# awaelchli/torch-optical-flow

Hardware: AMD Instinct MI355X
Metric: image-pairs/sec + corr-lookup HBM GB/s, RAFT 12-iter @ Sintel 1024×436 (higher is better)
Workload: dtype corr + convs split-fp16 (22-bit operands: fp16 hi + lo, 3 f16 MFMA per product, fp32 accumulate); lookup fp32; 1 GPU; raft-12iter-sintel-436x1024; pairs_per_gpu=8, global_batch=8, iters=12, padded=440x1024, parallelism=pairs sharded over 1 GPU(s), conv_benchmark=True, update_impl=split, hip_graph=True, steps_in_flight=1, full=False

## Files before the change

include/oflow.h:

```cpp
#ifndef OFLOW_H_
#define OFLOW_H_

#ifdef __cplusplus
extern "C" {
#endif

#define OFLOW_ABI_VERSION 3

#define OFLOW_OK 0
#define OFLOW_E_NULL (-1)
#define OFLOW_E_SHAPE (-2)
#define OFLOW_E_LEVELS (-3)
#define OFLOW_E_TINY (-4)
#define OFLOW_E_RADIUS (-5)
#define OFLOW_E_MODE (-6)
#define OFLOW_E_ALIGN (-7)

#define OFLOW_MAX_LEVELS 8
#define OFLOW_MAX_RADIUS 7

#define OFLOW_INTERP_BILINEAR 0
#define OFLOW_INTERP_NEAREST 1
#define OFLOW_INTERP_BICUBIC 2
#define OFLOW_PAD_ZEROS 0
#define OFLOW_PAD_BORDER 1
#define OFLOW_PAD_REFLECTION 2

#define OFLOW_IN_S32 0
#define OFLOW_IN_F32_NORM 1
#define OFLOW_IN_F32 2
#define OFLOW_IN_IMG7S2 3
#define OFLOW_IN_FLOW7 4
#define OFLOW_EPI_FLOW_HEAD 3

int oflow_abi_version(void);
const char* oflow_status_string(int status);

int oflow_corr_pyramid_dims(int H, int W, int num_levels, int* level_h, int* level_w);

int oflow_corr_pyramid_f32(const float* d_fmap1, const float* d_fmap2, int B, int C, int H, int W,
                           int num_levels, float* const* d_levels, void* stream);

int oflow_corr_lookup_f32(const float* const* d_levels, const int* level_h, const int* level_w,
                          int num_levels, const float* d_coords, int B, int H, int W, int radius,
                          float* d_out, void* stream);

long long oflow_corr_tiled_level_floats(int H_l, int W_l);
int oflow_corr_pyramid_tiled_f32(const float* d_fmap1, const float* d_fmap2, int B, int C, int H, int W,
                                 int num_levels, float* const* d_levels, void* stream);
int oflow_corr_pyramid_tiled_s32(const void* d_fmap1_s32, const void* d_fmap2_s32, int B, int C, int H, int W,
                                 int num_levels, float* const* d_levels, void* stream);
int oflow_corr_lookup_tiled_f32(const float* const* d_levels, const int* level_h, const int* level_w,
                                int num_levels, const float* d_coords, int B, int H, int W, int radius,
                                float* d_out, void* stream);
int oflow_corr_untile_f32(const float* d_tiled, float* d_out, long long Q, int H_l, int W_l, void* stream);

int oflow_grid_warp_f32(const float* d_frame, const float* d_flow, int B, int C, int H, int W, int mode,
                        int padding_mode, int align_corners, float* d_out, void* stream);

int oflow_grid_sample_f32(const float* d_input, const float* d_grid, int B, int C, int H, int W, int Ho, int Wo,
                          int mode, int padding_mode, int align_corners, float* d_out, void* stream);

int oflow_corr_otf_prepare_f16(const float* d_fmap1, const float* d_fmap2, int B, int C, int H, int W,
                               int num_levels, void* d_f1h, void* const* d_f2h, float* d_scratch, void* stream);
int oflow_corr_lookup_otf_f16(const void* d_f1h, const void* const* d_f2h, const int* level_h, const int* level_w,
                              int num_levels, const float* d_coords, int B, int C, int H, int W, int radius,
                              float* d_out, void* stream);

int oflow_corr_lookup_otf_backward_f32(const float* d_grad_out, const void* d_f1h, const void* const* d_f2h,
                                       const int* level_h, const int* level_w, int num_levels, const float* d_coords,
                                       int B, int C, int H, int W, int radius, float* d_grad_fmap1,
                                       float* d_grad_fmap2, float* d_scratch, void* stream);

int oflow_bias_act_f32(const float* d_x, long long sx, const float* d_bias, float* d_y0, long long sy0, float* d_y1,
                       long long sy1, int B, int C, int P, int activation, float scale, void* stream);
int oflow_gru_reset_f32(const float* d_zr, long long szr, const float* d_br, const float* d_h, long long sh,
                        float* d_rh, long long srh, int B, int CH, int P, void* stream);
int oflow_gru_blend_f32(const float* d_zr, long long szr, const float* d_bz, const float* d_q, long long sq,
                        const float* d_bq, float* d_h, long long sh, int B, int CH, int P, void* stream);

int oflow_pack_s32_f32(const float* d_x, long long x_batch_stride, int C, int B, int H, int W, int activation,
                       int dst_channel, void* d_y0, long long y0_pixel_stride, void* d_y1, long long y1_pixel_stride,
                       float* d_nhwc, int nhwc_pixel_stride, void* stream);
int oflow_flow_prep_s32(const float* d_coords, int B, int H, int W, void* d_patches, void* d_flow0,
                        long long flow0_pixel_stride, void* d_flow1, long long flow1_pixel_stride, void* stream);

typedef struct oflow_conv_s32_desc {
  unsigned int struct_size;
  int in_format, in_groups;
  const void* d_x;
  long long x_pixel_stride;
  const float *d_in_scale, *d_in_shift;
  const void *d_wpack, *d_wfrag;
  const float *d_wscale, *d_bias;
  int n_pad, N;
  int B, H, W, kh, kw, block_n;
  int epilogue, activation;
  float out_scale;
  void *d_y0, *d_y1;
  long long y0_pixel_stride, y1_pixel_stride;
  float* d_f32;
  long long f32_batch_stride, f32_channel_stride;
  int f32_accumulate;
  float *d_gru_h, *d_gru_z;
  int gru_channels;
  float *d_nhwc, *d_stats;
  const void* d_res;
  long long res_pixel_stride;
  int nhwc_pixel_stride, res_activation, s2d;
  const float* d_addend;
  long long addend_pixel_stride;
  const float* d_fh_weights;
  float* d_fh_partial;
  int fh_slabs;
} oflow_conv_s32_desc;
int oflow_conv_s32(const oflow_conv_s32_desc* desc, void* stream);

int oflow_flow_head_col2im_f32(const float* d_y, const float* d_bias, int B, int H, int W, float* d_coords, void* stream);
int oflow_flow_head_finish_f32(const float* d_partial, int slabs, const float* d_bias, int B, int H, int W,
                               float* d_coords, void* d_flow0, long long flow0_pixel_stride, void* d_flow1,
                               long long flow1_pixel_stride, void* stream);

int oflow_normalize_images_f32(const float* d_x0, const float* d_x1, long long n, float* d_y0, float* d_y1, void* stream);

int oflow_replicate_pad_f32(const float* const* d_src, float* const* d_dst, int count, long long planes, int H, int W,
                            int top, int bottom, int left, int right, void* stream);

int oflow_set_range_flag(unsigned int* d_flag);

int oflow_range_flag_exchange(unsigned int* d_flag, unsigned int* d_out, void* stream);

int oflow_timing_event_create(void** ev);
int oflow_timing_event_destroy(void* ev);
int oflow_timing_event_record(void* ev, void* stream, int external);
int oflow_timing_event_elapsed_ms(void* start, void* end, float* ms);

int oflow_flow_head2_s32(const void* d_x, long long x_pixel_stride, int in_groups, const float* d_weight,
                         const float* d_bias, int B, int H, int W, float* d_coords, void* stream);
int oflow_flow_head2_tiled_s32(const void* d_x, long long x_pixel_stride, int in_groups, const float* d_wr,
                               const float* d_bias, int B, int H, int W, float* d_coords, void* stream);
int oflow_corr_lookup_tiled_nhwc_f32(const float* const* d_levels, const int* level_h, const int* level_w, int num_levels,
                                     const float* d_coords, int B, int H, int W, int radius, float* d_out, int row_floats,
                                     void* stream);
int oflow_corr_lookup_convc1_s32(const float* const* d_levels, const int* level_h, const int* level_w, int num_levels,
                                 const float* d_coords, int B, int H, int W, int radius, const void* d_wpack,
                                 const float* d_wscale, const float* d_bias, void* d_y, long long y_pixel_stride,
                                 void* stream);

int oflow_stem_patches_s32(const float* d_img, int B, int C, int H, int W, void* d_out, int out_groups, void* stream);
int oflow_norm_stats_finalize(const float* d_partials, int B, int tiles, int n_pad, int C, double eps, float* d_alpha,
                              float* d_beta, void* stream);
int oflow_norm_apply_s32(const float* d_x, int C, int B, int H, int W, const float* d_alpha, const float* d_beta,
                         int activation, int res_mode, const void* d_res, long long res_pixel_stride, const float* d_x2,
                         const float* d_alpha2, const float* d_beta2, int res_activation, int s2d, void* d_y,
                         long long y_pixel_stride, void* stream);

int oflow_convex_upsample_f32(const float* d_flow, const float* d_mask, int B, int H, int W, float* d_out, void* stream);
int oflow_convex_upsample_backward_f32(const float* d_grad_out, const float* d_flow, const float* d_mask, int B, int H,
                                       int W, float* d_grad_flow, float* d_grad_mask, float* d_scratch, void* stream);

int oflow_conv2d_backward_input_f32(const float* d_grad_out, const float* d_weight, int B, int Cout, int Cin, int H, int W,
                                    int kh, int kw, float* d_grad_input, void* stream);
int oflow_conv2d_backward_weight_slab_pixels(void);
long long oflow_conv2d_backward_weight_workspace_floats(int B, int Cout, int Cin, int H, int W, int kh, int kw);
int oflow_conv2d_backward_weight_f32(const float* d_grad_out, const float* d_x, int B, int Cout, int Cin, int H, int W,
                                     int kh, int kw, float* d_grad_weight, float* d_grad_bias, float* d_workspace,
                                     void* stream);

int oflow_conv2d_strided_backward_input_f32(const float* d_grad_out, const float* d_weight, int B, int Cout, int Cin, int H,
                                            int W, int kh, int kw, int stride, float* d_grad_input, void* stream);
long long oflow_conv2d_strided_backward_weight_workspace_floats(int B, int Cout, int Cin, int H, int W, int kh, int kw,
                                                                int stride);
int oflow_conv2d_strided_backward_weight_f32(const float* d_grad_out, const float* d_x, int B, int Cout, int Cin, int H,
                                             int W, int kh, int kw, int stride, float* d_grad_weight, float* d_grad_bias,
                                             float* d_workspace, void* stream);
int oflow_conv2d_strided_backward_weight_generic_f32(const float* d_grad_out, const float* d_x, int B, int Cout, int Cin,
                                                     int H, int W, int kh, int kw, int stride, float* d_grad_weight,
                                                     float* d_grad_bias, float* d_workspace, void* stream);

int oflow_instance_norm_backward_f32(const float* d_grad_out, const float* d_x, int planes, int HW, double eps, int relu,
                                     float* d_grad_input, void* stream);
long long oflow_frozen_batch_norm_backward_workspace_floats(int B, int C, int HW);
int oflow_frozen_batch_norm_backward_f32(const float* d_grad_out, const float* d_x, const float* d_weight, const float* d_bias,
                                         const float* d_running_mean, const float* d_running_var, int B, int C, int HW,
                                         double eps, int relu, float* d_grad_input, float* d_grad_weight, float* d_grad_bias,
                                         float* d_workspace, void* stream);

int oflow_batch_norm_chunk_elements(void);
long long oflow_batch_norm_workspace_floats(int B, int C, int HW);
int oflow_batch_norm_forward_f32(const float* d_x, const float* d_weight, const float* d_bias, int B, int C, int HW,
                                 double eps, int relu, float* d_y, float* d_mean, float* d_var, float* d_workspace,
                                 void* stream);
int oflow_batch_norm_backward_f32(const float* d_grad_out, const float* d_x, const float* d_weight, const float* d_bias,
                                  const float* d_mean, const float* d_var, int B, int C, int HW, double eps, int relu,
                                  float* d_grad_input, float* d_grad_weight, float* d_grad_bias, float* d_workspace,
                                  void* stream);

int oflow_corr_lookup_backward_f32(const float* d_grad_out, const float* d_coords, int B, int H, int W, int radius,
                                   float* const* d_grad_levels, const int* level_h, const int* level_w, int num_levels,
                                   void* stream);
int oflow_corr_pyramid_grad_combine_f32(float* const* d_grad_levels, const int* level_h, const int* level_w,
                                        int num_levels, long long Q, void* stream);
int oflow_corr_fmap_grad_f32(const float* d_fmap1, const float* d_fmap2, const float* d_g0, int B, int C, int N,
                             float scale, float* d_grad_f1, float* d_grad_f2, void* stream);

int oflow_grid_warp_backward_f32(const float* d_grad_out, const float* d_frame, const float* d_flow, int B, int C, int H,
                                 int W, int mode, int padding_mode, int align_corners, float* d_grad_frame,
                                 float* d_grad_flow, void* stream);
int oflow_grid_sample_backward_f32(const float* d_grad_out, const float* d_input, const float* d_grid, int B, int C,
                                   int H, int W, int Ho, int Wo, int mode, int padding_mode, int align_corners,
                                   float* d_grad_input, float* d_grad_grid, void* stream);

#define OFLOW_FLOW_STATS_CHUNKS 128
#define OFLOW_FLOW2RGB_BAKER 0
#define OFLOW_FLOW2RGB_HSV 1
#define OFLOW_FLOW2RGB_MEISTER 2
int oflow_flow_stats_f32(const float* d_flow, int B, int H, int W, int clip, float clip_lo, float clip_hi,
                         int invert_y, float* d_partials, void* stream);
int oflow_flow2rgb_f32(const float* d_flow, int B, int H, int W, int method, int clip, float clip_lo, float clip_hi,
                       int invert_y, int have_denom, float denom, const float* d_partials, float* d_rgb, void* stream);
int oflow_flow_pack_f32(const float* d_flow, int B, int H, int W, int channels, int flip_rows, float* d_out,
                        void* stream);

#define OFLOW_FLOW_METRICS_PARTIALS 1024
#define OFLOW_MAX_PREDS 32
#define OFLOW_VALID_NONE 0
#define OFLOW_VALID_F32 1
#define OFLOW_VALID_U8 2
int oflow_flow_error_stats_f32(const float* d_pred, long long pred_sb, long long pred_sc, long long pred_sh,
                               const float* d_target, long long target_sb, long long target_sc, long long target_sh,
                               const void* d_valid, int valid_kind, long long valid_sb, long long valid_sh, int B, int H,
                               int W, float abs_threshold, float rel_threshold, float max_flow, float* d_epe_map,
                               double* d_workspace, double* d_accum, void* stream);
int oflow_sequence_loss_f32(const float* const* d_preds, int n_preds, const float* weights, const float* d_flow_gt,
                            const void* d_valid, int valid_kind, int B, int H, int W, float max_flow,
                            double* d_workspace, float* d_loss, double* d_stats, void* stream);
int oflow_sequence_loss_backward_f32(const float* d_grad_out, const float* const* d_preds, float* const* d_grads,
                                     int n_preds, const float* weights, const float* d_flow_gt, const void* d_valid,
                                     int valid_kind, int B, int H, int W, float max_flow, void* stream);

int oflow_forward_interpolate_f32(const float* d_flow, int B, int H, int W, float* d_out, void* stream);

int oflow_fb_consistency_f32(const float* d_fw, const float* d_bw, int B, int H, int W, float alpha, float beta,
                             unsigned char* d_mask_fw, unsigned char* d_mask_bw, float* d_err_fw, float* d_err_bw,
                             void* stream);

#define OFLOW_SPLAT_SUM 0
#define OFLOW_SPLAT_AVG 1
#define OFLOW_SPLAT_LINEAR 2
#define OFLOW_SPLAT_SOFT 3
#define OFLOW_SPLAT_EPS 1e-7
#define OFLOW_SPLAT_MIN_FRAC_BITS 38
#define OFLOW_SPLAT_MAX_PIXELS (1 << 22)
int oflow_splat_frac_bits(int H, int W);
long long oflow_splat_workspace_bytes(int B, int C, int H, int W);
int oflow_splat_f32(const float* d_frame, const float* d_flow, const float* d_metric, int B, int C, int H, int W,
                    int mode, float* d_out, float* d_weight, void* d_workspace, void* stream);
int oflow_splat_backward_f32(const float* d_grad_out, const float* d_frame, const float* d_flow, const float* d_metric,
                             const float* d_out, const float* d_weight, int B, int C, int H, int W, int mode,
                             float* d_grad_frame, float* d_grad_flow, float* d_grad_metric, void* d_workspace,
                             void* stream);

long long oflow_census_loss_workspace_bytes(int B, int H, int W);
int oflow_census_loss_f32(const float* d_frame0, const float* d_frame1, const void* d_mask, int mask_kind, int B,
                          int C, int H, int W, int patch, float image_range, float* d_s_map, double* d_workspace,
                          float* d_loss, double* d_sum_m, void* stream);
int oflow_census_loss_backward_f32(const float* d_grad_loss, const float* d_frame0, const float* d_frame1,
                                   const void* d_mask, int mask_kind, const float* d_s_map, const double* d_sum_m,
                                   int B, int C, int H, int W, int patch, float image_range, float* d_grad_frame0,
                                   float* d_grad_frame1, void* stream);
// ... 40 lines not shown
```

torch-optical-flow_amd/csrc/conv_s32.hip:

```cpp
#include "oflow_internal.h"

namespace oflow {
namespace {

typedef _Float16 half8 __attribute__((ext_vector_type(8)));
typedef float f32x16 __attribute__((ext_vector_type(16)));
typedef unsigned int u32x4 __attribute__((ext_vector_type(4)));

constexpr int kTY = 4, kTX = 32;

constexpr int kAinGroups = 4;


struct ConvArgs {
  const uint8_t* x;
  long long xps;
  int kg;
  const uint8_t* w;
  int npad;
  const float* wsc;
  const float* bias;
  int N;
  int B, H, W, tiles_x, tiles_y;
  int act;
  float oscale;
  uint8_t* y0;
  long long y0ps;
  uint8_t* y1;
  long long y1ps;
  float* f;
  long long fbs, fcs;
  int faccum;
  float* h;
  float* z;
  int gch;
  const float* add;
  long long addps;
  float* fn;
  int fnps;
  float* stats;
  const uint8_t* res;
  long long resps;
  int res_act;
  int s2d;
  const float* ia;
  const float* ib;
  int ain;
  int cin;
  int wbytes;
  const uint8_t* wf;
  int exp_flags;
  const float* fhw;
  float* fhy;
};
constexpr int kEpiFlowHead = OFLOW_EPI_FLOW_HEAD;
constexpr int kInS32 = OFLOW_IN_S32, kInF32Norm = OFLOW_IN_F32_NORM, kInF32 = OFLOW_IN_F32, kInImg = OFLOW_IN_IMG7S2,
              kInFlow = OFLOW_IN_FLOW7;
constexpr int kImgC = 3, kImgK = 7, kImgRows = (kTY - 1) * 2 + kImgK, kImgCols = (kTX - 1) * 2 + kImgK;
constexpr int kImgHalf = (kImgCols + 1) / 2, kImgPitch = 2 * kImgHalf, kImgPlane = kImgRows * kImgPitch;

__device__ __forceinline__ float sigmoid_hw(float v) {
  return __builtin_amdgcn_rcpf(1.0f + __builtin_amdgcn_exp2f(v * -1.4426950408889634f));
}
__device__ __forceinline__ float tanh_hw(float v) {
  return 1.0f - 2.0f * __builtin_amdgcn_rcpf(__builtin_amdgcn_exp2f(v * 2.8853900817779268f) + 1.0f);
}

__device__ __forceinline__ float act_fn(float v, int act) {
  if (act == 1) return v < 0.f ? 0.f : v;
  if (act == 2) return 1.0f / (1.0f + expf(-v));
  if (act == 3) return tanhf(v);
  return v;
}

__device__ __forceinline__ void split8(const float* v, half8& hi, half8& lo) { split_vec(v, hi, lo); }

__device__ __forceinline__ void store_s32(uint8_t* y, long long ps, long long P, int n, int N, const float* v, float& gm) {
  uint8_t* line = y + P * ps + (long long)(n >> 5) * 128 + ((n & 31) >> 3) * 16;
  if (n + 8 <= N) {
    half8 hi, lo;
    split8(v, hi, lo);
    gm = fmaxf(gm, fmaxf(fmaxf(fmaxf(fabsf(v[0]), fabsf(v[1])), fmaxf(fabsf(v[2]), fabsf(v[3]))),
                         fmaxf(fmaxf(fabsf(v[4]), fabsf(v[5])), fmaxf(fabsf(v[6]), fabsf(v[7])))));
    *reinterpret_cast<half8*>(line) = hi;
    *reinterpret_cast<half8*>(line + 64) = lo;
  } else {
    _Float16* hp = reinterpret_cast<_Float16*>(line);
    _Float16* lp = reinterpret_cast<_Float16*>(line + 64);
#pragma unroll
    for (int j = 0; j < 8; ++j) {
      if (n + j < N) {
        gm = fmaxf(gm, fabsf(v[j]));
        _Float16 h_, l_;
        split_f16(v[j], h_, l_);
        hp[j] = h_;
        lp[j] = l_;
      }
    }
  }
}

typedef __attribute__((address_space(4))) const float cfloat;
template <int T0, int T1>
__device__ __forceinline__ void flow_head_partials(const float* tp, cfloat* w, float* yp, long long plane, bool in) {
  constexpr int NO = 2 * (T1 - T0);
  float acc[2][NO];
#pragma unroll
  for (int j = 0; j < NO; ++j) acc[0][j] = acc[1][j] = 0.f;
  float wn[2][NO];
#pragma unroll
  for (int e = 0; e < 2; ++e)
#pragma unroll
    for (int j = 0; j < NO; ++j) wn[e][j] = w[e * 18 + 2 * T0 + j];
  float2 tn = *reinterpret_cast<const float2*>(tp);
#pragma unroll
  for (int e = 0; e < 2; ++e)
#pragma unroll
    for (int j = 0; j < NO; ++j) asm volatile("" : "+s"(wn[e][j]));
  asm volatile("" : "+v"(tn.x), "+v"(tn.y));
#pragma unroll 2
  for (int c0 = 0; c0 < 64; c0 += 2) {
    float wc[2][NO];
#pragma unroll
    for (int e = 0; e < 2; ++e)
#pragma unroll
      for (int j = 0; j < NO; ++j) wc[e][j] = wn[e][j];
    const float2 t = tn;
    const int c1 = c0 + 2 < 64 ? c0 + 2 : c0;
#pragma unroll
    for (int e = 0; e < 2; ++e)
#pragma unroll
      for (int j = 0; j < NO; ++j) wn[e][j] = w[(c1 + e) * 18 + 2 * T0 + j];
    tn = *reinterpret_cast<const float2*>(tp + c1);
    __builtin_amdgcn_sched_barrier(0);
#pragma unroll
    for (int j = 0; j < NO; ++j) {
      acc[0][j] = fmaf(t.x, wc[0][j], acc[0][j]);
      acc[1][j] = fmaf(t.y, wc[1][j], acc[1][j]);
    }
    __builtin_amdgcn_sched_barrier(0);
#pragma unroll
    for (int e = 0; e < 2; ++e)
#pragma unroll
      for (int j = 0; j < NO; ++j) asm volatile("" : "+s"(wn[e][j]));
    asm volatile("" : "+v"(tn.x), "+v"(tn.y));
  }
  if (in) {
#pragma unroll
    for (int j = 0; j < NO; ++j) yp[(2 * T0 + j) * plane] = acc[0][j] + acc[1][j];
  }
}

template <int KH, int KW, int BN, int WM, int WN, int EPI, int TY = kTY, int AIN = kInS32, bool BREG = false, int BD = 1>
__global__ __launch_bounds__(64 * WM * WN, WM * WN == 8 ? 1 : 2) void conv_s32_kernel(ConvArgs a) {
  constexpr int NTH = 64 * WM * WN;
  constexpr int T = KH * KW;
  constexpr int BM = TY * kTX;
  constexpr int PH = KH / 2, PW = KW / 2;
  constexpr int HY = TY + KH - 1, HX = kTX + KW - 1, NPIX = HY * HX;
  constexpr int AITEMS = NPIX * 8, APER = (AITEMS + NTH - 1) / NTH;
  constexpr int BITEMS = BN * 8, BPER = (BITEMS + NTH - 1) / NTH;
  constexpr int MT = TY / WM;
  constexpr int NT = BN / WN / 32;
  static_assert((WM * WN == 4 || WM * WN == 8) && MT >= 1 && NT >= 1, "bad wave grid");
  static_assert(NTH % 8 == 0, "an A item's 16-B chunk is tid & 7");
  constexpr bool WIN = AIN == kInImg || AIN == kInFlow;
  constexpr int WC = AIN == kInFlow ? 2 : kImgC, WS = AIN == kInFlow ? 1 : 2;
  constexpr int WROWS = (kTY - 1) * WS + kImgK, WCOLS = (kTX - 1) * WS + kImgK;
  constexpr int WHALF = WS == 2 ? (WCOLS + 1) / 2 : WCOLS, WPITCH = WS == 2 ? 2 * WHALF : WCOLS;
  constexpr int WPLANE = WROWS * WPITCH;
  constexpr int WKPAD = AIN == kInFlow ? 128 : 160;
  constexpr int WAPER = WIN ? BM * 4 / NTH : 1;
  static_assert(!WIN || (BM * 4) % NTH == 0, "window items");
  static_assert(AIN != kInImg || (WHALF == kImgHalf && WPITCH == kImgPitch && WPLANE == kImgPlane), "stem window");
  constexpr bool ADB = (T == 1) && !WIN;
  constexpr int RSA = 144, RSB = 144;
  constexpr int A_BYTES = NPIX * RSA, B_BYTES = BN * RSB;
  static_assert(!BREG || (T > 1 && (WM == 1 || WM == 2 || WM == 4) && BN == 32 * WN && AIN == kInS32),
                "register-direct B: T > 1, WM x WN waves of one 32-channel tile each");
  constexpr int MAIN_BYTES = (ADB ? 2 : 1) * A_BYTES + (BREG ? 0 : 2 * B_BYTES);
  constexpr int TS = BN + 4;
  constexpr int EPI_BYTES = BM * TS * 4;
  constexpr int LDS_BYTES = MAIN_BYTES > EPI_BYTES ? MAIN_BYTES : EPI_BYTES;
  constexpr int kImgZero = WC * WPLANE;
  constexpr int IMG_FLOATS = (kImgZero + 1 + 3) & ~3;
  constexpr int AFF_BYTES = AIN == kInF32Norm ? kAinGroups * 32 * 8
                            : WIN ? IMG_FLOATS * 4 + WKPAD * 4
                            : 0;
  static_assert(!WIN || (T == 1 && TY == kTY), "window input: 1x1 geometry over the patch channels, 4-row tiles");
  __shared__ __attribute__((aligned(16))) uint8_t smem[LDS_BYTES + AFF_BYTES];
  __shared__ float2 sSB[BN];
  __shared__ float3 sStat[EPI == 0 ? WM * BN : 1];
  float2* sAff = reinterpret_cast<float2*>(smem + LDS_BYTES);
  float* sImg = reinterpret_cast<float*>(smem + LDS_BYTES);
  int* sKoff = reinterpret_cast<int*>(smem + LDS_BYTES + (WIN ? IMG_FLOATS * 4 : 0));
  uint8_t* sA = smem;
  uint8_t* sB = smem + (ADB ? 2 : 1) * A_BYTES;

  const int tid = threadIdx.x, lane = tid & 63, wave = tid >> 6;
  const int wm = wave / WN, wn = wave % WN;
  const int r = lane & 31, hh = lane >> 5;

  int tile = blockIdx.x;
  const int cblk = blockIdx.y;
  const int tx0 = (tile % a.tiles_x) * kTX;
  tile /= a.tiles_x;
  const int ty0 = (tile % a.tiles_y) * TY;
  const int b = tile / a.tiles_y;
  const int n0 = cblk * BN;
  const long long pix0 = (long long)b * a.H * a.W;

  u32x4 ra[APER];
  const __amdgpu_buffer_rsrc_t rsA = __builtin_amdgcn_make_buffer_rsrc(
      const_cast<uint8_t*>(a.x + pix0 * a.xps), (short)0, (int)((long long)a.H * a.W * a.xps), 0x00020000);
  const __amdgpu_buffer_rsrc_t rsB =
      __builtin_amdgcn_make_buffer_rsrc(const_cast<uint8_t*>(a.w), (short)0, a.wbytes, 0x00020000);
  auto a_off = [&](int s_, int& col) {
    int t_ = tid;
    asm volatile("" : "+v"(t_));
    const int item = (AITEMS % NTH == 0) ? t_ + s_ * NTH : min(t_ + s_ * NTH, AITEMS - 1);
    const int p = item >> 3, c = item & 7;
    const int gy = ty0 - PH + p / HX, gx = tx0 - PW + p % HX;
    const int cy = min(max(gy, 0), a.H - 1), cx = min(max(gx, 0), a.W - 1);
    col = c * 16;
    return (cy * a.W + cx) * (int)a.xps + (AIN == kInF32 ? 0 : c * 16);
  };
  unsigned aok = 0u;
#pragma unroll
  for (int s_ = 0; s_ < APER; ++s_) {
    const int item = (AITEMS % NTH == 0) ? tid + s_ * NTH : min(tid + s_ * NTH, AITEMS - 1);
    const int p = item >> 3;
    const int gy = ty0 - PH + p / HX, gx = tx0 - PW + p % HX;
    const bool ok = static_cast<unsigned>(gy) < static_cast<unsigned>(a.H) && static_cast<unsigned>(gx) < static_cast<unsigned>(a.W);
    aok |= (ok ? 1u : 0u) << s_;
  }
  int boff[BPER];
#pragma unroll
  for (int s_ = 0; s_ < BPER; ++s_) boff[s_] = (n0 + (tid + s_ * NTH) / 8) * 128 + ((tid + s_ * NTH) & 7) * 16;
#define OFLOW_LOAD_A(RA, G)                                                                                          \
  if constexpr (!WIN) _Pragma("unroll") for (int s_ = 0; s_ < APER; ++s_) {                                          \
    int col_;                                                                                                        \
    const int off_ = a_off(s_, col_);                                                                                \
    if constexpr (AIN == kInF32)     \
      RA[s_] = __builtin_amdgcn_raw_buffer_load_b128(rsA, off_ + min((G) * 128 + col_, a.cin * 4 - 16), 0, 0);       \
    else                                                                                                             \
      RA[s_] = __builtin_amdgcn_raw_buffer_load_b128(rsA, off_, (G) * 128, 0);                                       \
  }
#define OFLOW_WRITE_A(RA, BUF, G)                                                                                    \
  float amx_ = 0.f;                                                                                                  \
  float2 af4_[4];                                                                                                    \
  if constexpr (AIN == kInF32Norm) _Pragma("unroll") for (int e_ = 0; e_ < 4; ++e_)                                  \
    af4_[e_] = sAff[(G) * 32 + 4 * (tid & 7) + e_];                                                                  \
  if constexpr (WIN) {                                                                                               \
                                                                                                        \
    _Pragma("unroll") for (int s_ = 0; s_ < WAPER; ++s_) {                                                           \
      const int item = tid + s_ * NTH;                                                                               \
      const int p = item % BM, cp = item / BM;                                                                       \
      const int pb_ = WS * (p >> 5) * WPITCH + (p & 31);                                                             \
      const int4 k0_ = *reinterpret_cast<const int4*>(sKoff + (G) * 32 + 8 * cp);                                    \
      const int4 k1_ = *reinterpret_cast<const int4*>(sKoff + (G) * 32 + 8 * cp + 4);                                \
      const int kov_[8] = {k0_.x, k0_.y, k0_.z, k0_.w, k1_.x, k1_.y, k1_.z, k1_.w};                                  \
      float v8_[8];                                                                                                  \
      _Pragma("unroll") for (int e_ = 0; e_ < 8; ++e_) {                                                             \
        v8_[e_] = sImg[kov_[e_] < 0 ? kImgZero : pb_ + kov_[e_]];                                                    \
        amx_ = fmaxf(amx_, fabsf(v8_[e_]));                                                                          \
      }                                                                                                              \
      half8 h8_, l8_;                                                                                                \
      split_vec(v8_, h8_, l8_);                                                                                      \
      uint8_t* rw_ = sA + (BUF) * A_BYTES + p * RSA;                                                                 \
      *reinterpret_cast<half8*>(rw_ + (cp << 4)) = h8_;                                                              \
      *reinterpret_cast<half8*>(rw_ + ((4 + cp) << 4)) = l8_;                                                        \
    }                                                                                                                \
  } else                                                                                                             \
  _Pragma("unroll") for (int s_ = 0; s_ < APER; ++s_) {                                                              \
    const int item = tid + s_ * NTH;                                                                                 \
                                                     \
    const int p = item >> 3, c = item & 7;                                                                           \
    if (AITEMS % NTH == 0 || item < AITEMS) {                                                                        \
      if constexpr (AIN != kInS32) {                                                                                 \
                   \
        typedef _Float16 half4_ __attribute__((ext_vector_type(4)));                                                 \
        half4_ h4 = {0, 0, 0, 0}, l4 = {0, 0, 0, 0};                                                                 \
        if (((aok >> s_) & 1u) && (AIN != kInF32 || (G) * 32 + 4 * c < a.cin)) {                                     \
          const float* fv = reinterpret_cast<const float*>(&RA[s_]);                                                 \
          float mx_ = 0.f, v4_[4];                                                                                   \
          _Pragma("unroll") for (int e_ = 0; e_ < 4; ++e_) {                                                         \
            float v_ = fv[e_];                                                                                       \
            if constexpr (AIN == kInF32Norm) {                                                                       \
              const float2 af = af4_[e_];                                                                            \
              v_ = v_ * af.x + af.y;                                                                                 \
              v_ = v_ < 0.f ? 0.f : v_;                                                                              \
            }                                                                                                        \
            mx_ = fmaxf(mx_, fabsf(v_));                                                                             \
            v4_[e_] = v_;                                                                                            \
          }                                                                                                          \
          split_vec(v4_, h4, l4);                                                                                    \
          amx_ = fmaxf(amx_, mx_);                                                                                   \
        }                                                                                                            \
        uint8_t* rw_ = sA + (BUF) * A_BYTES + p * RSA + (c & 1) * 8;                                                 \
        *reinterpret_cast<half4_*>(rw_ + ((c >> 1) << 4)) = h4;                                                      \
        *reinterpret_cast<half4_*>(rw_ + ((4 + (c >> 1)) << 4)) = l4;                                                \
      } else {                                                                                                       \
        *reinterpret_cast<u32x4*>(sA + (BUF) * A_BYTES + p * RSA + (c << 4)) =                                       \
            ((aok >> s_) & 1u) ? RA[s_] : u32x4{0u, 0u, 0u, 0u};                                                     \
      }                                                                                                              \
    }                                                                                                                \
  }                                                                                                                  \
  if constexpr (AIN != kInS32) range_guard(amx_);
#define OFLOW_LOAD_B(RB, STEP)                                                                                       \
  _Pragma("unroll") for (int s_ = 0; s_ < BPER; ++s_) {                                                              \
    const int item = tid + s_ * NTH;                                                                                 \
    if (BITEMS % NTH == 0 || item < BITEMS)                                                                          \
      RB[s_] = __builtin_amdgcn_raw_buffer_load_b128(rsB, boff[s_], (STEP) * a.npad * 128, 0);                       \
  }
#define OFLOW_WRITE_B(RB, BUF)                                                                                       \
  _Pragma("unroll") for (int s_ = 0; s_ < BPER; ++s_) {                                                              \
    const int item = tid + s_ * NTH;                                                                                 \
    const int n = item >> 3, c = item & 7;                                                                           \
    if (BITEMS % NTH == 0 || item < BITEMS)                                                                          \
      *reinterpret_cast<u32x4*>(sB + (BUF) * B_BYTES + n * RSB + (c << 4)) = RB[s_];                                 \
  }
#define OFLOW_READ_OPS(AH, AL, BH, BL, I, S_)                                                                        \
  {                                                                                                                  \
    const int ii_ = (I);                                                                                             \
    const int t_ = ii_ % T, ky_ = t_ / KW, kx_ = t_ - ky_ * KW;                                                      \
    const uint8_t* bufA_ = sA + (ADB ? (ii_ & 1) * A_BYTES : 0);                                                     \
    const uint8_t* bufB_ = sB + (ii_ & 1) * B_BYTES;                                                                 \
    const int chi_ = 2 * (S_) + hh, clo_ = 4 + 2 * (S_) + hh;                                                        \
    _Pragma("unroll") for (int mt_ = 0; mt_ < MT; ++mt_) {                                                           \
      const int p_ = (wm * MT + mt_ + ky_) * HX + r + kx_;                                                           \
      const uint8_t* row_ = bufA_ + p_ * RSA;                                                                        \
      AH[mt_] = *reinterpret_cast<const half8*>(row_ + (chi_ << 4));                                                 \
      AL[mt_] = *reinterpret_cast<const half8*>(row_ + (clo_ << 4));                                                 \
    }                                                                                                                \
    _Pragma("unroll") for (int nt_ = 0; nt_ < NT; ++nt_) {                                                           \
      const int n_ = wn * (BN / WN) + nt_ * 32 + r;                                                                  \
      const uint8_t* row_ = bufB_ + n_ * RSB;                                                                        \
      BH[nt_] = *reinterpret_cast<const half8*>(row_ + (chi_ << 4));                                                 \
      BL[nt_] = *reinterpret_cast<const half8*>(row_ + (clo_ << 4));                                                 \
    }                                                                                                                \
  }
#define OFLOW_MFMAS(AH, AL, BH, BL)                                                                                  \
  _Pragma("unroll") for (int mt = 0; mt < MT; ++mt)                                                                  \
    _Pragma("unroll") for (int nt = 0; nt < NT; ++nt) {                                                              \
      acc[mt][nt] = __builtin_amdgcn_mfma_f32_32x32x16_f16(AH[mt], BL[nt], acc[mt][nt], 0, 0, 0);                    \
      acc[mt][nt] = __builtin_amdgcn_mfma_f32_32x32x16_f16(AL[mt], BH[nt], acc[mt][nt], 0, 0, 0);                    \
      acc[mt][nt] = __builtin_amdgcn_mfma_f32_32x32x16_f16(AH[mt], BH[nt], acc[mt][nt], 0, 0, 0);                    \
    }

  f32x16 acc[MT][NT];
#pragma unroll
  for (int i = 0; i < MT; ++i)
#pragma unroll
    for (int j = 0; j < NT; ++j)
#pragma unroll
      for (int e = 0; e < 16; ++e) acc[i][j][e] = 0.f;

  const int S = a.kg * T;
  for (int c = tid; c < BN; c += NTH) {
    const int n = min(n0 + c, a.N - 1);
    sSB[c] = make_float2(a.wsc[n], a.bias ? a.bias[n] : 0.f);
  }
  if constexpr (AIN == kInF32Norm) {
    for (int e = tid; e < a.kg * 32; e += NTH)
      sAff[e] = make_float2(a.ia[(long long)b * a.kg * 32 + e], a.ib[(long long)b * a.kg * 32 + e]);
    __syncthreads();
  }
  if constexpr (AIN == kInImg) {
    const float* img = reinterpret_cast<const float*>(a.x) + (long long)b * kImgC * (2 * a.H) * (2 * a.W);
    const int iy0 = 2 * ty0 - kImgK / 2, ix0 = 2 * tx0 - kImgK / 2;
    constexpr int IMG_N = kImgC * kImgRows * kImgCols, IMG_PER = (IMG_N + NTH - 1) / NTH;
    float iv[IMG_PER];
    int io[IMG_PER];
#pragma unroll
    for (int s_ = 0; s_ < IMG_PER; ++s_) {
      const int e = min(tid + s_ * NTH, IMG_N - 1);
      const int ch = e / (kImgRows * kImgCols), rem = e - ch * (kImgRows * kImgCols);
      const int ry = rem / kImgCols, rx = rem - ry * kImgCols;
      const int iy = iy0 + ry, ix = ix0 + rx;
      const bool in = static_cast<unsigned>(iy) < static_cast<unsigned>(2 * a.H) && static_cast<unsigned>(ix) < static_cast<unsigned>(2 * a.W);
      const int cy = min(max(iy, 0), 2 * a.H - 1), cx = min(max(ix, 0), 2 * a.W - 1);
      const float v = img[((long long)ch * (2 * a.H) + cy) * (2 * a.W) + cx];
      iv[s_] = in ? v : 0.f;
      io[s_] = ch * kImgPlane + ry * kImgPitch + (rx & 1) * kImgHalf + (rx >> 1);
    }
#pragma unroll
    for (int s_ = 0; s_ < IMG_PER; ++s_)
      if (tid + s_ * NTH < IMG_N) sImg[io[s_]] = iv[s_];
  }
  if constexpr (AIN == kInFlow) {
    const float* co = reinterpret_cast<const float*>(a.x) + (long long)b * 2 * a.H * a.W;
    const int iy0 = ty0 - kImgK / 2, ix0 = tx0 - kImgK / 2;
    constexpr int FL_N = 2 * WROWS * WCOLS, FL_PER = (FL_N + NTH - 1) / NTH;
    float iv[FL_PER];
    int io[FL_PER];
#pragma unroll
    for (int s_ = 0; s_ < FL_PER; ++s_) {
      const int e = min(tid + s_ * NTH, FL_N - 1);
      const int ch = e / (WROWS * WCOLS), rem = e - ch * (WROWS * WCOLS);
      const int ry = rem / WCOLS, rx = rem - ry * WCOLS;
      const int iy = iy0 + ry, ix = ix0 + rx;
      const bool in = static_cast<unsigned>(iy) < static_cast<unsigned>(a.H) && static_cast<unsigned>(ix) < static_cast<unsigned>(a.W);
      const int cy = min(max(iy, 0), a.H - 1), cx = min(max(ix, 0), a.W - 1);
      const float v = co[((long long)ch * a.H + cy) * a.W + cx] - static_cast<float>(ch == 0 ? ix : iy);
      iv[s_] = in ? v : 0.f;
      io[s_] = ch * WPLANE + ry * WPITCH + rx;
    }
#pragma unroll
    for (int s_ = 0; s_ < FL_PER; ++s_)
      if (tid + s_ * NTH < FL_N) sImg[io[s_]] = iv[s_];
  }
  if constexpr (WIN) {
    for (int k = tid; k < WKPAD; k += NTH) {
      const int t = k / WC, ch = k - t * WC;
      const int ky = t / kImgK, kx = t - ky * kImgK;
      sKoff[k] = t < kImgK * kImgK
                     ? ch * WPLANE + ky * WPITCH + (WS == 2 ? (kx & 1) * WHALF + (kx >> 1) : kx)
                     : -1;
    }
    if (tid == 0) sImg[kImgZero] = 0.f;
    __syncthreads();
  }
  if constexpr (BREG) {
  const __amdgpu_buffer_rsrc_t rsW =
      __builtin_amdgcn_make_buffer_rsrc(const_cast<uint8_t*>(a.wf), (short)0, a.wbytes, 0x00020000);
  const int wlane = ((n0 >> 5) + wn) * 4096 + lane * 16;
  const int wstep = a.npad * 128;
  constexpr int RING = 2;
  u32x4 bq[RING][4];
  auto load_b = [&](u32x4 (&d)[4], int step) {
#pragma unroll
    for (int e = 0; e < 4; ++e) d[e] = __builtin_amdgcn_raw_buffer_load_b128(rsW, wlane + e * 1024, step * wstep, 0);
  };
#define OFLOW_READ_A(AH, AL, I, S_)                                                                                  \
  {                                                                                                                  \
    const int ii_ = (I);                                                                                             \
    const int t_ = ii_ % T, ky_ = t_ / KW, kx_ = t_ - ky_ * KW;                                                      \
    const int chi_ = 2 * (S_) + hh, clo_ = 4 + 2 * (S_) + hh;                                                        \
    _Pragma("unroll") for (int mt_ = 0; mt_ < MT; ++mt_) {                                                           \
      const int p_ = (wm * MT + mt_ + ky_) * HX + r + kx_;                                                           \
      const uint8_t* row_ = sA + p_ * RSA;                                                                           \
      AH[mt_] = *reinterpret_cast<const half8*>(row_ + (chi_ << 4));                                                 \
      AL[mt_] = *reinterpret_cast<const half8*>(row_ + (clo_ << 4));                                                 \
    }                                                                                                                \
  }
#define OFLOW_MFMAS_R(AH, AL, BC, S_)                                                                                \
  _Pragma("unroll") for (int mt = 0; mt < MT; ++mt) {                                                                \
    const half8 bh_ = __builtin_bit_cast(half8, BC[2 * (S_)]), bl_ = __builtin_bit_cast(half8, BC[2 * (S_) + 1]);    \
    acc[mt][0] = __builtin_amdgcn_mfma_f32_32x32x16_f16(AH[mt], bl_, acc[mt][0], 0, 0, 0);                           \
    acc[mt][0] = __builtin_amdgcn_mfma_f32_32x32x16_f16(AL[mt], bh_, acc[mt][0], 0, 0, 0);                           \
    acc[mt][0] = __builtin_amdgcn_mfma_f32_32x32x16_f16(AH[mt], bh_, acc[mt][0], 0, 0, 0);                           \
  }
#pragma unroll
  for (int q = 0; q < RING; ++q) load_b(bq[q], q < S ? q : S - 1);
  OFLOW_LOAD_A(ra, 0);
  OFLOW_WRITE_A(ra, 0, 0);
  OFLOW_LOAD_A(ra, a.kg > 1 ? 1 : 0);
  __syncthreads();
  constexpr int GPB = (T % RING == 0) ? 1 : RING;
  constexpr bool VSLIDE = KW == 1 && KH > 1 && WM == 1 && !(EPI == 0 && KH == 5);
  if constexpr (VSLIDE) {
    constexpr int NR = MT + KH - 1;
    half8 V[NR][2][2];
    auto rd = [&](int hr, int sub) {
      const uint8_t* row_ = sA + (hr * HX + r) * RSA;
      V[hr][sub][0] = *reinterpret_cast<const half8*>(row_ + ((2 * sub + hh) << 4));
      V[hr][sub][1] = *reinterpret_cast<const half8*>(row_ + ((4 + 2 * sub + hh) << 4));
    };
    auto mf = [&](int ky, int sub, u32x4 (&bc)[4]) {
      const half8 bh_ = __builtin_bit_cast(half8, bc[2 * sub]), bl_ = __builtin_bit_cast(half8, bc[2 * sub + 1]);
#pragma unroll
      for (int mt = 0; mt < MT; ++mt) {
        acc[mt][0] = __builtin_amdgcn_mfma_f32_32x32x16_f16(V[mt + ky][sub][0], bl_, acc[mt][0], 0, 0, 0);
        acc[mt][0] = __builtin_amdgcn_mfma_f32_32x32x16_f16(V[mt + ky][sub][1], bh_, acc[mt][0], 0, 0, 0);
        acc[mt][0] = __builtin_amdgcn_mfma_f32_32x32x16_f16(V[mt + ky][sub][0], bh_, acc[mt][0], 0, 0, 0);
      }
    };
#pragma unroll
    for (int m = 0; m < MT; ++m) rd(m, 0);
    for (int g0 = 0; g0 < a.kg; g0 += GPB) {
#pragma unroll
      for (int j = 0; j < GPB * T; ++j) {
        const int gg = g0 + j / T, t = j % T;
        if (GPB > 1 && j > 0 && t == 0 && gg >= a.kg) break;
        const int i_ = gg * T + t;
        u32x4 (&bc)[4] = bq[j % RING];
        if (t == 0) {
#pragma unroll
          for (int m = 0; m < MT; ++m) rd(m, 1);
        } else {
          rd(t + MT - 1, 1);
        }
        mf(t, 0, bc);
        if (t == T - 1) {
          __syncthreads();
          OFLOW_WRITE_A(ra, 0, gg + 1 < a.kg ? gg + 1 : gg);
          const int g2 = gg + 2 < a.kg ? gg + 2 : a.kg - 1;
          OFLOW_LOAD_A(ra, g2);
          __syncthreads();
#pragma unroll
          for (int m = 0; m < MT; ++m) rd(m, 0);
        } else {
          rd(t + MT, 0);
        }
        mf(t, 1, bc);
        load_b(bc, i_ + RING < S ? i_ + RING : S - 1);
      }
    }
  } else {
  half8 xah[MT], xal[MT], yah[MT], yal[MT];
  OFLOW_READ_A(xah, xal, 0, 0);
  for (int g0 = 0; g0 < a.kg; g0 += GPB) {
#pragma unroll
    for (int j = 0; j < GPB * T; ++j) {
      const int gg = g0 + j / T, t = j % T;
      if (GPB > 1 && j > 0 && t == 0 && gg >= a.kg) break;
      const int i_ = gg * T + t;
      u32x4 (&bc)[4] = bq[j % RING];
      OFLOW_READ_A(yah, yal, i_, 1);
      OFLOW_MFMAS_R(xah, xal, bc, 0);
      if (t == T - 1) {
        __syncthreads();
        OFLOW_WRITE_A(ra, 0, gg + 1 < a.kg ? gg + 1 : gg);
        const int g2 = gg + 2 < a.kg ? gg + 2 : a.kg - 1;
        OFLOW_LOAD_A(ra, g2);
        __syncthreads();
      }
      OFLOW_READ_A(xah, xal, i_ + 1, 0);
      OFLOW_MFMAS_R(yah, yal, bc, 1);
      load_b(bc, i_ + RING < S ? i_ + RING : S - 1);
    }
  }
  }
#undef OFLOW_READ_A
#undef OFLOW_MFMAS_R
  } else {
  u32x4 rbr[BD][BPER];
  u32x4 rar[ADB ? BD : 1][APER];
  OFLOW_LOAD_B(rbr[0], 0);
  OFLOW_LOAD_A(rar[0], 0);
  OFLOW_WRITE_A(rar[0], 0, 0);
// ... 7 lines not shown
  if constexpr (!ADB) { OFLOW_LOAD_A(rar[0], a.kg > 1 ? 1 : 0); }
  __syncthreads();
  half8 xah[MT], xal[MT], xbh[NT], xbl[NT];
  half8 yah[MT], yal[MT], ybh[NT], ybl[NT];
  OFLOW_READ_OPS(xah, xal, xbh, xbl, 0, 0);

  constexpr int GPB2 = (BD > 1 && (T % BD) != 0) ? BD : 1;
  for (int g0 = 0; g0 < a.kg; g0 += GPB2) {
#pragma unroll
    for (int j = 0; j < GPB2 * T; ++j) {
      const int g = g0 + j / T, t = j % T;
      if (GPB2 > 1 && j > 0 && t == 0 && g >= a.kg) break;
      const int i_ = g * T + t;
      u32x4 (&rb)[BPER] = rbr[(j + 1) % BD];
      OFLOW_WRITE_B(rb, (i_ + 1) & 1);
      if constexpr (ADB) { OFLOW_WRITE_A(rar[(j + 1) % BD], (i_ + 1) & 1, i_ + 1 < S ? i_ + 1 : S - 1); }
      {
        const int i2 = i_ + 1 + BD < S ? i_ + 1 + BD : S - 1;
        OFLOW_LOAD_B(rb, i2);
        if constexpr (ADB) { OFLOW_LOAD_A(rar[(j + 1) % BD], i2); }
      }
      OFLOW_READ_OPS(yah, yal, ybh, ybl, i_, 1);
      OFLOW_MFMAS(xah, xal, xbh, xbl);
      if constexpr (!ADB) {
        if (t == T - 1) {
          __syncthreads();
          OFLOW_WRITE_A(rar[0], 0, g + 1 < a.kg ? g + 1 : g);
          const int g2 = g + 2 < a.kg ? g + 2 : a.kg - 1;
          OFLOW_LOAD_A(rar[0], g2);
        }
      }
      __syncthreads();
      OFLOW_READ_OPS(xah, xal, xbh, xbl, i_ + 1, 0);
      OFLOW_MFMAS(yah, yal, ybh, ybl);
    }
  }
  }
#undef OFLOW_MFMAS
#undef OFLOW_READ_OPS
#undef OFLOW_LOAD_A
#undef OFLOW_WRITE_A
#undef OFLOW_LOAD_B
#undef OFLOW_WRITE_B

  constexpr int C8 = BN / 8;
  constexpr int KIT = (BM * C8 + NTH - 1) / NTH;
  constexpr bool GRU = EPI == 1 || EPI == 2;
  const bool has_add = GRU && a.add != nullptr;
  u32x4 ad[GRU ? KIT : 1][2];
  if (has_add) {
#pragma unroll
    for (int k = 0; k < (GRU ? KIT : 0); ++k) {
      const int item = tid + k * NTH;
      const int pl = item / C8, n = n0 + (item - pl * C8) * 8;
      const int y = ty0 + pl / kTX, x = tx0 + (pl % kTX);
      if (item >= BM * C8 || n >= a.N || y >= a.H || x >= a.W) continue;
      const u32x4* ap = reinterpret_cast<const u32x4*>(a.add + (pix0 + (long long)y * a.W + x) * a.addps + n);
      ad[k][0] = ap[0];
      ad[k][1] = ap[1];
    }
  }
  __syncthreads();
  float* sT = reinterpret_cast<float*>(smem);
#pragma unroll
  for (int mt = 0; mt < MT; ++mt)
#pragma unroll
    for (int nt = 0; nt < NT; ++nt) {
      const int nl = wn * (BN / WN) + nt * 32 + r;
      const int pbase = (wm * MT + mt) * kTX;
      if constexpr (EPI == kEpiFlowHead) {
        const float2 sb = sSB[nl];
#pragma unroll
        for (int e = 0; e < 16; ++e) {
          const int m = (e & 3) + 8 * (e >> 2) + 4 * hh;
          const float v = fmaf(acc[mt][nt][e], sb.x, sb.y);
          sT[(pbase + m) * TS + nl] = v < 0.f ? 0.f : v;
        }
      } else {
#pragma unroll
      for (int e = 0; e < 16; ++e) {
        const int m = (e & 3) + 8 * (e >> 2) + 4 * hh;
        sT[(pbase + m) * TS + nl] = acc[mt][nt][e];
      }
      }
    }
  if constexpr (EPI == 0 && TY >= kTY) {
    if (a.stats != nullptr) {
#pragma unroll
      for (int nt = 0; nt < NT; ++nt) {
        const int nl = wn * (BN / WN) + nt * 32 + r;
        const float2 sb = sSB[nl];
        float cnt = 0.f, sum = 0.f, q = 0.f;
        const bool full = ty0 + TY <= a.H && tx0 + kTX <= a.W;
        if (full) {
#pragma unroll
          for (int mt = 0; mt < MT; ++mt)
#pragma unroll
            for (int e = 0; e < 16; ++e) sum += acc[mt][nt][e] * sb.x + sb.y;
          cnt = 16.f * MT;
        } else {
#pragma unroll
          for (int mt = 0; mt < MT; ++mt) {
            const bool yok = ty0 + wm * MT + mt < a.H;
#pragma unroll
            for (int e = 0; e < 16; ++e) {
              const bool ok = yok && tx0 + (e & 3) + 8 * (e >> 2) + 4 * hh < a.W;
              sum += ok ? acc[mt][nt][e] * sb.x + sb.y : 0.f;
              cnt += ok ? 1.f : 0.f;
            }
          }
        }
        const float mean = cnt > 0.f ? sum / cnt : 0.f;
        if (full) {
#pragma unroll
          for (int mt = 0; mt < MT; ++mt)
#pragma unroll
            for (int e = 0; e < 16; ++e) {
              const float d = (acc[mt][nt][e] * sb.x + sb.y) - mean;
              float dd = d * d;
              asm volatile("" : "+v"(dd));
              q += dd;
            }
        } else {
#pragma unroll
          for (int mt = 0; mt < MT; ++mt) {
            const bool yok = ty0 + wm * MT + mt < a.H;
#pragma unroll
            for (int e = 0; e < 16; ++e) {
              const bool ok = yok && tx0 + (e & 3) + 8 * (e >> 2) + 4 * hh < a.W;
              const float d = (acc[mt][nt][e] * sb.x + sb.y) - mean;
              q += ok ? d * d : 0.f;
            }
          }
        }
        const float nb = __shfl_xor(cnt, 32), mb = __shfl_xor(mean, 32), qb = __shfl_xor(q, 32);
        const float n0_ = hh ? nb : cnt, m0_ = hh ? mb : mean, q0_ = hh ? qb : q;
        const float n1_ = hh ? cnt : nb, m1_ = hh ? mean : mb, q1_ = hh ? q : qb;
        const float nn = n0_ + n1_;
        float M = m0_, Q = q0_;
        if (n1_ > 0.f) {
          if (n0_ > 0.f) {
            const float d = m1_ - m0_;
            M = m0_ + d * (n1_ / nn);
            Q = q0_ + q1_ + d * d * (n0_ * n1_ / nn);
          } else {
            M = m1_;
            Q = q1_;
          }
        }
        if (hh == 0) sStat[wm * BN + nl] = make_float3(nn, M, Q);
      }
    }
  }
  __syncthreads();
  if constexpr (EPI == kEpiFlowHead) {
    constexpr int NSLAB = BN / 64, NPART = NTH / 64 / (2 * NSLAB);
    static_assert(BM == 128 && BN % 64 == 0 && NTH == 256 && (NPART == 1 || NPART == 2), "flow-head epilogue: 4 x 32 tiles, 4 waves");
    const int wv = __builtin_amdgcn_readfirstlane(wave);
    const int sl = (wv >> 1) % NSLAB, part = (wv >> 1) / NSLAB;
    const int pl = (wv & 1) * 64 + lane;
    const int y = ty0 + pl / kTX, x = tx0 + (pl % kTX);
    const bool in = y < a.H && x < a.W;
    const int slab = (n0 >> 6) + sl;
    const long long plane = (long long)a.H * a.W;
    cfloat* w2 = (cfloat*)(a.fhw) + slab * (64 * 18);
    float* yp = a.fhy + ((long long)slab * a.B + b) * 18 * plane + (long long)y * a.W + x;
    const float* tp = sT + pl * TS + sl * 64;
    if constexpr (NPART == 1) {
      flow_head_partials<0, 9>(tp, w2, yp, plane, in);
    } else {
      if (part == 0)
        flow_head_partials<0, 5>(tp, w2, yp, plane, in);
      else
        flow_head_partials<5, 9>(tp, w2, yp, plane, in);
    }
    return;
  }
  if (has_add) {
    constexpr bool FIXED_OCT_ADD = NTH % C8 == 0;
    float2 sba[8];
    if constexpr (FIXED_OCT_ADD) {
#pragma unroll
      for (int j = 0; j < 8; ++j) sba[j] = sSB[(tid % C8) * 8 + j];
    }
#pragma unroll
    for (int k = 0; k < (GRU ? KIT : 0); ++k) {
      const int item = tid + k * NTH;
      const int pl = item / C8, nl = (item - pl * C8) * 8, n = n0 + nl;
      const int y = ty0 + pl / kTX, x = tx0 + (pl % kTX);
      if (item >= BM * C8 || n >= a.N || y >= a.H || x >= a.W) continue;
      const float* av = reinterpret_cast<const float*>(&ad[k][0]);
      float4* tp4 = reinterpret_cast<float4*>(&sT[pl * TS + nl]);
      const float4 t0 = tp4[0], t1 = tp4[1];
      float t[8] = {t0.x, t0.y, t0.z, t0.w, t1.x, t1.y, t1.z, t1.w};
#pragma unroll
      for (int j = 0; j < 8; ++j) {
        const float2 sb = FIXED_OCT_ADD ? sba[j] : sSB[nl + j];
        t[j] = (t[j] * sb.x + sb.y) + av[j];
      }
      tp4[0] = make_float4(t[0], t[1], t[2], t[3]);
      tp4[1] = make_float4(t[4], t[5], t[6], t[7]);
    }
  }

  if (a.f != nullptr) {
    for (int item = tid; item < BM * BN; item += NTH) {
      const int nl = item / BM, pl = item - nl * BM;
      const int n = n0 + nl;
      const int y = ty0 + pl / kTX, x = tx0 + (pl % kTX);
      if (n < a.N && y < a.H && x < a.W) {
        const float2 sb = sSB[nl];
        float v = sT[pl * TS + nl] * sb.x + sb.y;
        v = act_fn(v, a.act) * a.oscale;
        float* d = a.f + b * a.fbs + n * a.fcs + (long long)y * a.W + x;
        if (a.faccum)
          *d = *d + v;
        else
          *d = v;
      }
    }
  }
  if constexpr (EPI == 0) {
    if (a.stats != nullptr) {
      if constexpr (TY >= kTY) {
        constexpr int NSUB = TY / kTY, WPS = kTY / MT;
        if (tid < BN * NSUB) {
          const int c = tid % BN, sub = tid / BN, n = n0 + c;
          float N0 = 0.f, M0 = 0.f, Q0 = 0.f;
#pragma unroll
          for (int j = 0; j < WPS; ++j) {
            const float3 t = sStat[(sub * WPS + j) * BN + c];
            const float nn = N0 + t.x;
            if (t.x > 0.f) {
              if (N0 > 0.f) {
                const float d = t.y - M0;
                M0 = M0 + d * (t.x / nn);
                Q0 = Q0 + t.z + d * d * (N0 * t.x / nn);
              } else {
                M0 = t.y;
                Q0 = t.z;
              }
              N0 = nn;
            }
          }
          if (n < a.N && ty0 + sub * kTY < a.H) {
            const int tiles4_y = (a.H + kTY - 1) / kTY;
            const int tile_in_img = (ty0 / kTY + sub) * a.tiles_x + tx0 / kTX;
            float* st = a.stats + (((long long)b * a.tiles_x * tiles4_y + tile_in_img) * a.npad + n) * 3;
            st[0] = N0;
            st[1] = M0;
            st[2] = Q0;
          }
        }
      }
    }
    if (a.y0 == nullptr && a.fn == nullptr) return;
  }

  u32x4 pre[EPI == 0 ? 1 : KIT][EPI == 2 ? 4 : 2];
#pragma unroll
  for (int k = 0; k < (EPI == 0 ? 0 : KIT); ++k) {
    const int item = tid + k * NTH;
    const int pl = item / C8, nl = (item - pl * C8) * 8, n = n0 + nl;
    const int y = ty0 + pl / kTX, x = tx0 + (pl % kTX);
    if (item >= BM * C8 || n >= a.N || y >= a.H || x >= a.W) continue;
    const long long P = pix0 + (long long)y * a.W + x;
    if constexpr (EPI == 1) {
      if (n >= a.gch) {
        const u32x4* hp = reinterpret_cast<const u32x4*>(a.h + P * a.gch + (n - a.gch));
        pre[k][0] = hp[0];
        pre[k][1] = hp[1];
      }
    } else if constexpr (EPI == 2) {
      const u32x4* hp = reinterpret_cast<const u32x4*>(a.h + P * a.gch + n);
      const u32x4* zp = reinterpret_cast<const u32x4*>(a.z + P * a.gch + n);
      pre[k][0] = hp[0];
      pre[k][1] = hp[1];
      pre[k][2] = zp[0];
      pre[k][3] = zp[1];
    }
  }
  const bool hwx = (a.exp_flags & 256) == 0;
  constexpr int UNR = EPI == 0 ? 1 : KIT;
  float gmx = 0.f;
  constexpr bool FIXED_OCT = NTH % C8 == 0;
  float2 sbv[8];
  if constexpr (FIXED_OCT) {
#pragma unroll
    for (int j = 0; j < 8; ++j) sbv[j] = sSB[(tid % C8) * 8 + j];
  }
#pragma unroll UNR
  for (int k = 0; k < KIT; ++k) {
    const int item = tid + k * NTH;
    const int pl = item / C8, c8 = item - pl * C8;
    const int nl = c8 * 8, n = n0 + nl;
    const int y = ty0 + pl / kTX, x = tx0 + (pl % kTX);
    if (item >= BM * C8 || n >= a.N || y >= a.H || x >= a.W) continue;
    const long long P = pix0 + (long long)y * a.W + x;
    const float* pf = reinterpret_cast<const float*>(&pre[EPI == 0 ? 0 : k][0]);
    const float4 t0 = *reinterpret_cast<const float4*>(&sT[pl * TS + nl]);
    const float4 t1 = *reinterpret_cast<const float4*>(&sT[pl * TS + nl + 4]);
    float v[8] = {t0.x, t0.y, t0.z, t0.w, t1.x, t1.y, t1.z, t1.w};
    if (!has_add) {
#pragma unroll
      for (int j = 0; j < 8; ++j) {
        const float2 sb = FIXED_OCT ? sbv[j] : sSB[nl + j];
        v[j] = v[j] * sb.x + sb.y;
      }
    }
    if constexpr (EPI == 0) {
#pragma unroll
      for (int j = 0; j < 8; ++j) v[j] = act_fn(v[j], a.act) * a.oscale;
      if (a.res) {
        const uint8_t* rl = a.res + P * a.resps + (long long)(n >> 5) * 128 + ((n & 31) >> 3) * 16;
        const half8 rh = *reinterpret_cast<const half8*>(rl), rlo = *reinterpret_cast<const half8*>(rl + 64);
#pragma unroll
        for (int j = 0; j < 8; ++j) {
          v[j] = v[j] + (static_cast<float>(rh[j]) + static_cast<float>(rlo[j]));
          if (a.res_act) v[j] = act_fn(v[j], a.res_act);
        }
      }
      if (a.fn) {
        float* fp = a.fn + P * a.fnps + n;
        if (n + 8 <= a.N) {
          *reinterpret_cast<float4*>(fp) = make_float4(v[0], v[1], v[2], v[3]);
          *reinterpret_cast<float4*>(fp + 4) = make_float4(v[4], v[5], v[6], v[7]);
        } else {
#pragma unroll
          for (int j = 0; j < 8; ++j)
            if (n + j < a.N) fp[j] = v[j];
        }
      }
      if (a.y0) {
        long long Pd = P;
        int nd = n;
        if (a.s2d) {
          const int W2 = a.W >> 1, H2 = a.H >> 1;
          Pd = ((long long)b * H2 + (y >> 1)) * W2 + (x >> 1);
          nd = n + ((y & 1) * 2 + (x & 1)) * a.N;
        }
        store_s32(a.y0, a.y0ps, Pd, nd, a.s2d ? 4 * a.N : a.N, v, gmx);
        if (a.y1) store_s32(a.y1, a.y1ps, Pd, nd, a.s2d ? 4 * a.N : a.N, v, gmx);
      }
    } else if constexpr (EPI == 1) {
      if (n < a.gch) {
        float4* zp = reinterpret_cast<float4*>(a.z + P * a.gch + n);
        float zv[8];
#pragma unroll
        for (int j = 0; j < 8; ++j) zv[j] = hwx ? sigmoid_hw(v[j]) : 1.0f / (1.0f + expf(-v[j]));
        zp[0] = make_float4(zv[0], zv[1], zv[2], zv[3]);
        zp[1] = make_float4(zv[4], zv[5], zv[6], zv[7]);
      } else {
        float rh[8];
#pragma unroll
        for (int j = 0; j < 8; ++j) rh[j] = (hwx ? sigmoid_hw(v[j]) : 1.0f / (1.0f + expf(-v[j]))) * pf[j];
        store_s32(a.y0, a.y0ps, P, n - a.gch, a.gch, rh, gmx);
      }
    } else {
      float* hp = a.h + P * a.gch + n;
      float hn[8];
#pragma unroll
      for (int j = 0; j < 8; ++j) {
        const float q = hwx ? tanh_hw(v[j]) : tanhf(v[j]);
        const float z = pf[8 + j];
        hn[j] = (1.0f - z) * pf[j] + z * q;
      }
#pragma unroll
      for (int j = 0; j < 8; ++j) hp[j] = hn[j];
      store_s32(a.y0, a.y0ps, P, n, a.N, hn, gmx);
    }
  }
  range_guard(gmx);
}

inline dim3 conv_grid(const ConvArgs& a, int bn) {
  const int ntiles = a.tiles_x * a.tiles_y * a.B;
  return dim3(ntiles, a.npad / bn);
}

long long g_last_conv_leaf = 0;
template <int KH, int KW, int BN, int WM, int WN, int EPI, int TY, int AIN, bool BREG, int BD>
void record_leaf() {
  static_assert(KH < 16 && KW < 16 && BN < 256 && WM < 16 && WN < 16 && EPI < 16 && TY < 16 && AIN < 16 && BD < 16, "leaf fields");
  g_last_conv_leaf = (long long)KH | (long long)KW << 4 | (long long)BN << 8 | (long long)WM << 16 | (long long)WN << 20 |
                     (long long)EPI << 24 | (long long)TY << 28 | (long long)AIN << 32 | (long long)(BREG ? 1 : 0) << 36 |
                     (long long)BD << 40;
}

template <int KH, int KW, int BN, int WM, int WN, int EPI, int TY, int AIN>
void launch_staged(const ConvArgs& a, dim3 grid, hipStream_t s) {
  record_leaf<KH, KW, BN, WM, WN, EPI, TY, AIN, false, 2>();
  hipLaunchKernelGGL((conv_s32_kernel<KH, KW, BN, WM, WN, EPI, TY, AIN, false, 2>), grid, dim3(64 * WM * WN), 0, s, a);
}

template <int KH, int KW, int BN, int WM, int WN, int EPI, int TY = kTY, bool BREG = false>
int launch_conv(const ConvArgs& a0, hipStream_t s) {
  ConvArgs a = a0;
  if constexpr (BREG) {
    a.tiles_y = (a.H + TY - 1) / TY;
    dim3 grid = conv_grid(a, BN);
    record_leaf<KH, KW, BN, WM, WN, EPI, TY, kInS32, true, 1>();
    hipLaunchKernelGGL((conv_s32_kernel<KH, KW, BN, WM, WN, EPI, TY, kInS32, true>), grid, dim3(64 * WM * WN), 0, s, a);
    return launch_status();
  } else {
  a.tiles_y = (a.H + TY - 1) / TY;
  dim3 grid = conv_grid(a, BN);
  if constexpr (KH == 3 && KW == 3 && EPI == 0) {
    if (a.ain == kInF32Norm) {
      launch_staged<KH, KW, BN, WM, WN, EPI, TY, kInF32Norm>(a, grid, s);
      return launch_status();
    }
  }
  if constexpr (KH == 1 && KW == 1 && EPI == 0 && BN == 64 && TY == kTY) {
    if (a.ain == kInImg) {
      launch_staged<KH, KW, BN, WM, WN, EPI, TY, kInImg>(a, grid, s);
      return launch_status();
    }
  }
  if constexpr (KH == 1 && KW == 1 && EPI == 0 && BN == 128 && TY == kTY) {
    if (a.ain == kInFlow) {
      launch_staged<KH, KW, BN, WM, WN, EPI, TY, kInFlow>(a, grid, s);
      return launch_status();
    }
  }
  if constexpr (KH == 1 && KW == 1 && EPI == 0 && BN == 128) {
    if (a.ain == kInF32) {
      launch_staged<KH, KW, BN, WM, WN, EPI, TY, kInF32>(a, grid, s);
      return launch_status();
    }
  }
  if (a.ain != kInS32) return OFLOW_E_MODE;
  launch_staged<KH, KW, BN, WM, WN, EPI, TY, kInS32>(a, grid, s);
  return launch_status();
  }
}

int g_small_grid_px = 16384;
int g_stats_8row = 1;
int g_conv_exp_flags = 0;
int g_bn64_8row = 0;
inline bool small_grid(const ConvArgs& a, int bn) {
  return (long long)a.B * a.H * a.W < g_small_grid_px && a.stats == nullptr && a.ain == kInS32 && a.npad % 64 == 0 &&
         bn >= 64;
}

inline bool use_breg(const ConvArgs& a, int bn, int taps) {
  return a.wf != nullptr && (bn == 128 || bn == 64 || bn == 32) && taps > 1 && a.ain == kInS32 && a.stats == nullptr &&
         !small_grid(a, bn);
}

template <int KH, int KW, int EPI>
int launch_bn(const ConvArgs& a, int bn, hipStream_t s) {
  if (small_grid(a, bn)) return launch_conv<KH, KW, 64, 2, 2, EPI, 2>(a, s);
  if constexpr (KH * KW > 1 && KH * KW != 4)
    if (use_breg(a, bn, KH * KW)) {
      if (bn == 128) return launch_conv<KH, KW, 128, 1, 4, EPI, kTY, true>(a, s);
      if constexpr (KH == 3 && KW == 3) {
        if (bn == 64) return launch_conv<KH, KW, 64, 2, 2, EPI, kTY, true>(a, s);
        return launch_conv<KH, KW, 32, 4, 1, EPI, kTY, true>(a, s);
      }
    }
  switch (bn) {
    case 128: return launch_conv<KH, KW, 128, 2, 2, EPI>(a, s);
    case 96: return launch_conv<KH, KW, 96, 4, 1, EPI>(a, s);
    case 64:
      if constexpr (KH * KW > 1)
        if (a.stats == nullptr ? g_bn64_8row != 0 : g_stats_8row != 0) return launch_conv<KH, KW, 64, 4, 1, EPI, 8>(a, s);
      return launch_conv<KH, KW, 64, 2, 2, EPI>(a, s);
    case 32: return launch_conv<KH, KW, 32, 4, 1, EPI>(a, s);
    default: return OFLOW_E_SHAPE;
  }
}

int dispatch_conv(const ConvArgs& a, int kh, int kw, int block_n, int epilogue, hipStream_t s) {
  const int key = kh * 16 + kw;
  switch (epilogue) {
    case 0:
      switch (key) {
        case 0x11: return launch_bn<1, 1, 0>(a, block_n, s);
        case 0x22: return launch_bn<2, 2, 0>(a, block_n, s);
        case 0x33: return launch_bn<3, 3, 0>(a, block_n, s);
        case 0x15: return launch_bn<1, 5, 0>(a, block_n, s);
        case 0x51: return launch_bn<5, 1, 0>(a, block_n, s);
        default: return OFLOW_E_SHAPE;
      }
    case 1:
      if (block_n != 128) return OFLOW_E_SHAPE;
      if (small_grid(a, block_n)) {
        if (key == 0x15) return launch_conv<1, 5, 64, 2, 2, 1, 2>(a, s);
        if (key == 0x51) return launch_conv<5, 1, 64, 2, 2, 1, 2>(a, s);
      }
      if (use_breg(a, block_n, kh * kw)) {
        if (key == 0x15) return launch_conv<1, 5, 128, 1, 4, 1, kTY, true>(a, s);
        if (key == 0x51) return launch_conv<5, 1, 128, 1, 4, 1, kTY, true>(a, s);
      }
      if (key == 0x15) return launch_conv<1, 5, 128, 2, 2, 1>(a, s);
      if (key == 0x51) return launch_conv<5, 1, 128, 2, 2, 1>(a, s);
      return OFLOW_E_SHAPE;
    case kEpiFlowHead:
      if (key != 0x33) return OFLOW_E_SHAPE;
      if (block_n == 64) return launch_conv<3, 3, 64, 2, 2, kEpiFlowHead>(a, s);
      if (block_n == 128) return a.wf != nullptr ? launch_conv<3, 3, 128, 1, 4, kEpiFlowHead, kTY, true>(a, s) : OFLOW_E_MODE;
      return OFLOW_E_SHAPE;
    default:
      if (block_n != 128) return OFLOW_E_SHAPE;
      if (small_grid(a, block_n)) {
        if (key == 0x15) return launch_conv<1, 5, 64, 2, 2, 2, 2>(a, s);
        if (key == 0x51) return launch_conv<5, 1, 64, 2, 2, 2, 2>(a, s);
      }
      if (use_breg(a, block_n, kh * kw)) {
        if (key == 0x15) return launch_conv<1, 5, 128, 1, 4, 2, kTY, true>(a, s);
        if (key == 0x51) return launch_conv<5, 1, 128, 1, 4, 2, kTY, true>(a, s);
      }
      if (key == 0x15) return launch_conv<1, 5, 128, 2, 2, 2>(a, s);
      if (key == 0x51) return launch_conv<5, 1, 128, 2, 2, 2>(a, s);
      return OFLOW_E_SHAPE;
  }
}

int conv_args_from_desc(const oflow_conv_s32_desc& d, ConvArgs& a) {
  const bool fh = d.epilogue == kEpiFlowHead;
  if (fh) {
    if (!d.d_fh_weights || !d.d_fh_partial) return OFLOW_E_NULL;
    if (d.N != 256 || d.n_pad != 256 || d.fh_slabs != d.N / 64 || d.kh != 3 || d.kw != 3 ||
        (d.block_n != 64 && d.block_n != 128))
      return OFLOW_E_SHAPE;
    if (d.in_format != kInS32 || d.activation != 1 || d.out_scale != 1.0f || d.d_y0 || d.d_y1 || d.d_f32 || d.d_gru_h ||
        d.d_gru_z || d.d_nhwc || d.d_stats || d.d_res || d.s2d || d.d_addend)
      return OFLOW_E_MODE;
    if ((d.x_pixel_stride & 127) || ((uintptr_t)d.d_fh_weights & 3) || ((uintptr_t)d.d_fh_partial & 3)) return OFLOW_E_ALIGN;
  }
  const bool gru = d.epilogue == 1 || d.epilogue == 2;
  if (!d.d_x || !d.d_wpack || !d.d_wscale) return OFLOW_E_NULL;
  if (d.B <= 0 || d.H <= 0 || d.W <= 0 || d.N <= 0 || d.in_groups <= 0 || d.n_pad < d.N || d.n_pad % d.block_n)
    return OFLOW_E_SHAPE;
  if (d.activation < 0 || d.activation > 3 ||
      (!fh && (d.res_activation < 0 || d.res_activation > 3 || d.epilogue < 0 || d.epilogue > 2)))
    return OFLOW_E_MODE;
  if ((d.x_pixel_stride & 15) || ((uintptr_t)d.d_x & 15) || ((uintptr_t)d.d_wpack & 15)) return OFLOW_E_ALIGN;
  if (d.epilogue == 0 && !d.d_y0 && !d.d_f32 && !d.d_nhwc && !d.d_stats) return OFLOW_E_NULL;
  if (gru && (!d.d_y0 || !d.d_gru_h || !d.d_gru_z || d.gru_channels <= 0 || d.gru_channels % 8)) return OFLOW_E_NULL;
  if (gru && (((uintptr_t)d.d_gru_h & 15) || ((uintptr_t)d.d_gru_z & 15))) return OFLOW_E_ALIGN;
  if (d.epilogue == 1 && d.N != 2 * d.gru_channels) return OFLOW_E_SHAPE;
  if (d.epilogue == 2 && d.N != d.gru_channels) return OFLOW_E_SHAPE;
  if (gru && (d.d_nhwc || d.d_stats || d.d_res || d.s2d)) return OFLOW_E_MODE;
  if (d.s2d && ((d.H | d.W) & 1 || d.N % 8)) return OFLOW_E_SHAPE;
  if (d.d_nhwc && (d.nhwc_pixel_stride < d.N || ((uintptr_t)d.d_nhwc & 15) || (d.nhwc_pixel_stride & 3))) return OFLOW_E_ALIGN;
  if ((d.d_y0 && ((d.y0_pixel_stride & 127) || ((uintptr_t)d.d_y0 & 15))) ||
      (d.d_y1 && ((d.y1_pixel_stride & 127) || ((uintptr_t)d.d_y1 & 15))) ||
      (d.d_res && ((d.res_pixel_stride & 127) || ((uintptr_t)d.d_res & 15))))
    return OFLOW_E_ALIGN;
  a = ConvArgs{};
  a.x = static_cast<const uint8_t*>(d.d_x);
  a.xps = d.x_pixel_stride;
  a.kg = d.in_groups;
  a.w = static_cast<const uint8_t*>(d.d_wpack);
  a.npad = d.n_pad;
  a.wsc = d.d_wscale;
  a.bias = d.d_bias;
  a.N = d.N;
  a.B = d.B;
  a.H = d.H;
  a.W = d.W;
  a.tiles_x = (d.W + kTX - 1) / kTX;
  a.tiles_y = (d.H + kTY - 1) / kTY;
  a.act = d.activation;
  a.oscale = d.out_scale;
  a.cin = d.in_groups * 32;
  a.exp_flags = g_conv_exp_flags;
  a.y0 = static_cast<uint8_t*>(d.d_y0);
  a.y0ps = d.y0_pixel_stride;
  a.y1 = static_cast<uint8_t*>(d.d_y1);
  a.y1ps = d.y1_pixel_stride;
  a.f = d.d_f32;
  a.fbs = d.f32_batch_stride;
  a.fcs = d.f32_channel_stride;
  a.faccum = d.f32_accumulate;
  a.h = d.d_gru_h;
  a.z = d.d_gru_z;
  a.gch = d.gru_channels;
  a.fn = d.d_nhwc;
  a.fnps = d.nhwc_pixel_stride;
  a.stats = d.d_stats;
  a.res = static_cast<const uint8_t*>(d.d_res);
  a.resps = d.res_pixel_stride;
  a.res_act = d.res_activation;
  a.s2d = d.s2d;
  const long long wbytes = (long long)d.in_groups * d.kh * d.kw * d.n_pad * 128;
  if (wbytes >= (1ll << 31) || (long long)d.H * d.W * d.x_pixel_stride >= (1ll << 31)) return OFLOW_E_SHAPE;
  a.wbytes = static_cast<int>(wbytes);
  if (d.d_wfrag) {
    if ((uintptr_t)d.d_wfrag & 15) return OFLOW_E_ALIGN;
    if (d.n_pad % 32) return OFLOW_E_SHAPE;
    a.wf = static_cast<const uint8_t*>(d.d_wfrag);
  }
  if (fh) {
    a.fhw = d.d_fh_weights;
    a.fhy = d.d_fh_partial;
    return OFLOW_OK;
  }
  if (d.in_format < kInS32 || d.in_format > kInFlow) return OFLOW_E_MODE;
  a.ain = d.in_format;
  if (d.in_format == kInFlow) {
    if (d.kh != 1 || d.kw != 1 || d.epilogue != 0 || d.block_n != 128 || d.in_groups != (kImgK * kImgK * 2 + 31) / 32)
      return OFLOW_E_MODE;
    if ((long long)2 * d.B * d.H * d.W >= (1ll << 31) || d.d_addend) return OFLOW_E_SHAPE;
    return OFLOW_OK;
  }
  if (d.in_format == kInImg) {
    if (d.kh != 1 || d.kw != 1 || d.epilogue != 0 || d.block_n != 64 || d.in_groups != (kImgK * kImgK * kImgC + 31) / 32)
      return OFLOW_E_MODE;
    if ((long long)kImgC * 4 * d.H * d.W >= (1ll << 31)) return OFLOW_E_SHAPE;
    if (d.d_addend) return OFLOW_E_MODE;
    return OFLOW_OK;
  }
  if (d.in_format != kInF32 && (d.x_pixel_stride & 127)) return OFLOW_E_ALIGN;
  if (d.in_format == kInF32Norm && d.x_pixel_stride != (long long)d.in_groups * 128) return OFLOW_E_SHAPE;
  if (d.in_format == kInF32) {
    const long long cin = d.x_pixel_stride / 4;
    if ((d.x_pixel_stride & 15) || cin > (long long)d.in_groups * 32 || cin <= (long long)(d.in_groups - 1) * 32)
      return OFLOW_E_SHAPE;
    a.cin = static_cast<int>(cin);
  }
  if (d.in_format == kInF32Norm) {
    if (!d.d_in_scale || !d.d_in_shift) return OFLOW_E_NULL;
    if (d.kh != 3 || d.kw != 3 || d.epilogue != 0 || d.in_groups > kAinGroups) return OFLOW_E_MODE;
    a.ia = d.d_in_scale;
    a.ib = d.d_in_shift;
  } else if (d.in_format == kInF32) {
    if (d.kh != 1 || d.kw != 1 || d.epilogue != 0 || d.block_n != 128) return OFLOW_E_MODE;
  }
  if (d.d_addend) {
    if (d.epilogue == 0) return OFLOW_E_MODE;
    if (d.N % 8) return OFLOW_E_SHAPE;
    if (((uintptr_t)d.d_addend & 15) || (d.addend_pixel_stride & 3) || d.addend_pixel_stride < d.N) return OFLOW_E_ALIGN;
    a.add = d.d_addend;
    a.addps = d.addend_pixel_stride;
  }
  return OFLOW_OK;
}

}
OFLOW_RANGE_FLAG_SETTER(conv)
}

using namespace oflow;

extern "C" int oflow_conv_s32(const oflow_conv_s32_desc* desc, void* stream) {
  if (!desc) return OFLOW_E_NULL;
  if (desc->struct_size != sizeof(oflow_conv_s32_desc)) return OFLOW_E_MODE;
  ConvArgs a;
  const int st = conv_args_from_desc(*desc, a);
  if (st != OFLOW_OK) return st;
  return dispatch_conv(a, desc->kh, desc->kw, desc->block_n, desc->epilogue, static_cast<hipStream_t>(stream));
}

extern "C" void oflow_exp_set_small_grid_px(int pixels) { oflow::g_small_grid_px = pixels; }
extern "C" void oflow_exp_set_stats_8row(int on) { oflow::g_stats_8row = on; }
extern "C" void oflow_exp_set_conv_flags(int flags) { oflow::g_conv_exp_flags = flags; }
extern "C" void oflow_exp_set_bn64_8row(int on) { oflow::g_bn64_8row = on; }
extern "C" long long oflow_exp_last_conv_leaf(void) { return oflow::g_last_conv_leaf; }
```

torch-optical-flow_amd/csrc/upsample.hip:

```cpp
#include "oflow_internal.h"

namespace oflow {
namespace {

constexpr int kUX = 32;

__global__ __launch_bounds__(256) void convex_upsample_kernel(const float* __restrict__ flow,
                                                              const float* __restrict__ mask, int H, int W,
                                                              float* __restrict__ out) {
  __shared__ float sM[9][8][kUX + 1];
  __shared__ float sF[2][3][kUX + 2];
  const int tid = threadIdx.x;
  const int xb = blockIdx.x, y = blockIdx.y, n = blockIdx.z;
  const int x0 = xb * kUX;
  const long long HW = (long long)H * W;
  const float* fl = flow + (long long)n * 2 * HW;
  const float* mk = mask + (long long)n * 576 * HW + (long long)y * W;
  for (int e = tid; e < 2 * 3 * (kUX + 2); e += 256) {
    const int c = e / (3 * (kUX + 2)), rem = e - c * 3 * (kUX + 2);
    const int dy = rem / (kUX + 2), dx = rem - dy * (kUX + 2);
    const int yy = y + dy - 1, xx = x0 + dx - 1;
    float v = 0.f;
    if (yy >= 0 && yy < H && xx >= 0 && xx < W) v = 8.0f * fl[c * HW + (long long)yy * W + xx];
    sF[c][dy][dx] = v;
  }
  const int xo = tid >> 3, j = tid & 7;
  const bool live = x0 + xo < W;
  for (int i = 0; i < 8; ++i) {
    __syncthreads();
    for (int e = tid; e < 9 * 8 * kUX; e += 256) {
      const int row = e / kUX, xl = e - row * kUX;
      const int k = row >> 3, jj = row & 7;
      float v = 0.f;
      if (x0 + xl < W) v = mk[(long long)(k * 64 + i * 8 + jj) * HW + x0 + xl];
      sM[k][jj][xl] = v;
    }
    __syncthreads();
    if (live) {
      float m[9];
      float mx = sM[0][j][xo];
#pragma unroll
      for (int k = 0; k < 9; ++k) {
        m[k] = sM[k][j][xo];
        mx = fmaxf(mx, m[k]);
      }
      float s = 0.f;
#pragma unroll
      for (int k = 0; k < 9; ++k) {
        m[k] = expf(m[k] - mx);
        s += m[k];
      }
      float o0 = 0.f, o1 = 0.f;
#pragma unroll
      for (int k = 0; k < 9; ++k) {
        const float w = m[k] / s;
        const int dy = k / 3, dx = k % 3;
        o0 += w * sF[0][dy][xo + dx];
        o1 += w * sF[1][dy][xo + dx];
      }
      const long long W8 = 8LL * W, H8W8 = 64LL * HW;
      float* op = out + (long long)n * 2 * H8W8 + (long long)(8 * y + i) * W8 + 8LL * (x0 + xo) + j;
      op[0] = o0;
      op[H8W8] = o1;
    }
  }
}

}
}

using namespace oflow;

extern "C" int oflow_convex_upsample_f32(const float* d_flow, const float* d_mask, int B, int H, int W, float* d_out,
                                         void* stream) {
  if (!d_flow || !d_mask || !d_out) return OFLOW_E_NULL;
  if (B <= 0 || H <= 0 || W <= 0 || B > 65535 || H > 65535) return OFLOW_E_SHAPE;
  dim3 grid((W + kUX - 1) / kUX, H, B);
  hipLaunchKernelGGL(convex_upsample_kernel, grid, dim3(256), 0, static_cast<hipStream_t>(stream), d_flow, d_mask, H,
                     W, d_out);
  return launch_status();
}
```

torch-optical-flow_amd/methods/raft/model/extractor.py:

```python
from __future__ import annotations

import os

from typing import Optional, List, Sequence, Tuple, Union

import torch
import torch.nn as nn
from torch import Tensor

from optical_flow import _native

from .update import CONV_BLOCKS, parse_block_overrides


def _norm_layer(norm_fn: str, planes: int, groups: int) -> nn.Module:
    if norm_fn == "group":
        return nn.GroupNorm(num_groups=groups, num_channels=planes)
    if norm_fn == "batch":
        return nn.BatchNorm2d(planes)
    if norm_fn == "instance":
        return nn.InstanceNorm2d(planes)
    if norm_fn == "none":
        return nn.Sequential()
    raise ValueError(f"unknown norm_fn {norm_fn!r}")
# ... 124 lines not shown
                    nn.init.constant_(m.weight, 1)
                if m.bias is not None:
                    nn.init.constant_(m.bias, 0)

    def _make_layer(self, dim: int, stride: int = 1) -> nn.Module:
        blocks = (ResidualBlock(self.in_planes, dim, self.norm_fn, stride=stride), ResidualBlock(dim, dim, self.norm_fn, 1))
        self.in_planes = dim
        return nn.Sequential(*blocks)

    def forward(self, x: Union[Tensor, Sequence[Tensor]]) -> Union[Tensor, Tuple[Tensor, ...]]:
        is_list = isinstance(x, (tuple, list))
        if is_list:
            batch_dim = x[0].shape[0]
            x = torch.cat(list(x), dim=0)
        impl = self.encoder_backward_impl
        if impl not in ENCODER_BACKWARD_IMPLS:
            raise ValueError(f"encoder_backward_impl must be 'aten' or 'native', got {impl!r}")
        bn = self.batch_norm_impl
        if bn not in BATCH_NORM_IMPLS:
            raise ValueError(f"batch_norm_impl must be 'aten' or 'native', got {bn!r}")
        for layer in (self.layer1, self.layer2, self.layer3):
            for blk in layer:
                blk.encoder_backward_impl, blk.batch_norm_impl = impl, bn
        if impl != "aten" or bn != "aten":
            x = enc_norm_act(self.norm1, enc_conv(self.conv1, x, impl), True, impl, bn)
        else:
            x = self.relu1(self.norm1(self.conv1(x)))
        x = self.layer3(self.layer2(self.layer1(x)))
        x = enc_conv(self.conv2, x, impl)
        if self.training and self.dropout is not None:
            x = self.dropout(x)
        if is_list:
            return torch.split(x, [batch_dim, batch_dim], dim=0)
        return x




def _s2d_weight(w: Tensor) -> Tensor:
    n, c = w.shape[:2]
    out = torch.zeros((n, 4, c, 2, 2), device=w.device, dtype=w.dtype)
    for kyp in range(2):
        for a in range(2):
            ky = 2 * kyp + a - 1
            if not 0 <= ky <= 2:
                continue
            for kxp in range(2):
                for b in range(2):
                    kx = 2 * kxp + b - 1
                    if 0 <= kx <= 2:
                        out[:, a * 2 + b, :, kyp, kxp] = w[:, :, ky, kx]
    return out.reshape(n, 4 * c, 2, 2)


def _fold_bn(conv: nn.Conv2d, bn: nn.Module):
    w = conv.weight.detach().double()
    b = conv.bias.detach().double() if conv.bias is not None else torch.zeros(w.shape[0], device=w.device, dtype=w.dtype)
    alpha = bn.weight.detach().double() / torch.sqrt(bn.running_var.detach().double() + bn.eps)
    beta = bn.bias.detach().double() - bn.running_mean.detach().double() * alpha
    return (w * alpha.view(-1, 1, 1, 1)).float(), (b * alpha + beta).float()


_ENC_BN_OVERRIDE = {int(k): v for k, v in
                    parse_block_overrides("OFLOW_ENC_BN", {str(b) for b in CONV_BLOCKS}).items()}


class SplitEncoder:

    def __init__(self, enc: BasicEncoder) -> None:
        if enc.norm_fn not in ("instance", "batch"):
            raise RuntimeError(f"SplitEncoder: norm_fn {enc.norm_fn!r} not supported")
        if enc.norm_fn == "batch" and enc.training:
            raise RuntimeError("SplitEncoder: batch norm needs eval mode (running statistics)")
        self.enc = enc
        self.inorm = enc.norm_fn == "instance"
        from .update import cached_pack, tensor_key

        key = tuple(tensor_key(q) for q in enc.parameters()) + tuple(tensor_key(q) for q in enc.buffers())
        self.w = cached_pack(enc, key, lambda: self._pack(enc))

    def _cw(self, conv: nn.Conv2d, norm, **kw):
        if self.inorm or norm is None:
            w, b = conv.weight, conv.bias
        else:
            w, b = _fold_bn(conv, norm)
        if kw.pop("s2d", False):
            w = _s2d_weight(w.detach().float())
        n = w.shape[0]
        return _native.ConvWeights(w, b, ((n + 31) // 32) * 32, **kw)

    def _pack(self, enc: BasicEncoder):
        W = {"stem": self._cw(enc.conv1, enc.norm1, patches=True)}
        for li, layer in enumerate((enc.layer1, enc.layer2, enc.layer3)):
            for bi, blk in enumerate(layer):
                s2 = blk.downsample is not None
                W[f"{li}.{bi}.conv1"] = self._cw(blk.conv1, blk.norm1, s2d=s2)
                W[f"{li}.{bi}.conv2"] = self._cw(blk.conv2, blk.norm2)
                if s2:
                    W[f"{li}.{bi}.down"] = self._cw(blk.downsample[0], blk.downsample[1])
        W["head"] = _native.ConvWeights(enc.conv2.weight, enc.conv2.bias, ((enc.conv2.out_channels + 31) // 32) * 32)
        return W

    @staticmethod
    def _bn(n: int) -> int:
        bn = {64: 64, 96: 96, 128: 128}.get(n, 128 if n % 128 == 0 else 64 if n % 64 == 0 else 32)
        return _ENC_BN_OVERRIDE.get(bn, bn)

    def _conv_norm(self, x, cw, shape, act, out=None, res=None, s2d=False, raw_only=False):
        b, h, w = shape
        bn = self._bn(cw.n)
        V = _native.S32Slice
        dev = x.device
        if self.inorm:
            raw = torch.empty((b * h * w, cw.n), device=dev, dtype=torch.float32)
            tiles = _native.conv_tiles(h, w)
            part = torch.empty((b, tiles, cw.n_pad, 3), device=dev, dtype=torch.float32)
            _native.conv_s32(x, cw, bn, nhwc=raw, stats=part)
            alpha, beta = _native.norm_stats(part, b, tiles, cw.n_pad, cw.n, 1e-5)
            if raw_only:
                return raw, alpha, beta
            if out is None:
                out = _native.s32_empty(b, h // 2 if s2d else h, w // 2 if s2d else w, (cw.n * (4 if s2d else 1) + 31) // 32, dev)
            if isinstance(res, _native.NhwcNormIn):
                _native.norm_apply(raw, (b, cw.n, h, w), alpha, beta, act, V(out), res_raw=(res.raw, res.scale, res.shift),
                                   res_act="relu", s2d=s2d, res_raw_relu=True)
            elif isinstance(res, tuple):
                _native.norm_apply(raw, (b, cw.n, h, w), alpha, beta, act, V(out), res_raw=res, res_act="relu", s2d=s2d)
            else:
                _native.norm_apply(raw, (b, cw.n, h, w), alpha, beta, act, V(out), res=res, res_act="relu" if res is not None else "none", s2d=s2d)
            return out
        if raw_only:
            out = _native.s32_empty(b, h, w, (cw.n + 31) // 32, dev)
            _native.conv_s32(x, cw, bn, y0=V(out))
            return out
        if out is None:
            out = _native.s32_empty(b, h // 2 if s2d else h, w // 2 if s2d else w, (cw.n * (4 if s2d else 1) + 31) // 32, dev)
        _native.conv_s32(x, cw, bn, act=act, y0=V(out), res=res, res_act="relu" if res is not None else "none", s2d=s2d)
        return out

    def _conv1(self, x, cw, shape):
        if self.inorm:
            raw, alpha, beta = self._conv_norm(x, cw, shape, "relu", raw_only=True)
            return _native.NhwcNormIn(raw, *shape, alpha, beta)
        return _native.S32Slice(self._conv_norm(x, cw, shape, "relu"))

    def stem_patches(self, x: Tensor) -> Tensor:
        x = x.float().contiguous()
        n, _, hh, ww = x.shape
        patches = _native.s32_empty(n, hh // 2, ww // 2, self.w["stem"].kg, x.device)
        _native.stem_patches(x, patches)
        return patches

    def __call__(self, x: Union[Tensor, Sequence[Tensor]], patches: Optional[Tensor] = None,
                 split_out: bool = False, stem_from_image: bool = False) -> Union[Tensor, Tuple[Tensor, ...]]:
        is_list = isinstance(x, (tuple, list))
        if is_list:
            batch_dim = x[0].shape[0]
            n, _, hh, ww = x[0].shape
            n *= len(x)
            if patches is None or tuple(patches.shape[:4]) != (n, hh // 2, ww // 2, self.w["stem"].kg):
                x = torch.cat(list(x), dim=0)
        if not isinstance(x, (tuple, list)):
            x = x.float().contiguous()
            n, _, hh, ww = x.shape
            dev = x.device
        else:
            dev = x[0].device
        if hh % 8 or ww % 8:
            raise RuntimeError("SplitEncoder: H and W must be multiples of 8")
        V = _native.S32Slice
        h, w = hh // 2, ww // 2
        if stem_from_image:
            if isinstance(x, (tuple, list)):
                x = torch.cat([t.float() for t in x], dim=0)
            stem_in = _native.ImgIn(x.float().contiguous())
            self.patches = None
        else:
            if patches is None or tuple(patches.shape[:4]) != (n, h, w, self.w["stem"].kg):
                patches = _native.s32_empty(n, h, w, self.w["stem"].kg, dev)
                _native.stem_patches(x, patches)
            self.patches = patches
            stem_in = V(patches)
        cur = (self._conv1(stem_in, self.w["stem"], (n, h, w)) if self.inorm
               else self._conv_norm(stem_in, self.w["stem"], (n, h, w), "relu"))
        layers = (self.enc.layer1, self.enc.layer2, self.enc.layer3)
        for li, layer in enumerate(layers):
            for bi, blk in enumerate(layer):
                last_of_stage = bi == len(layer) - 1
                out_s2d = last_of_stage and li + 1 < len(layers)
                pre = f"{li}.{bi}."
                if blk.downsample is None:
                    x_in = cur if isinstance(cur, _native.NhwcNormIn) else V(cur)
                    t = self._conv1(x_in, self.w[pre + "conv1"], (n, h, w))
                    cur = self._conv_norm(t, self.w[pre + "conv2"], (n, h, w), "relu", res=x_in, s2d=out_s2d)
                else:
                    h, w = h // 2, w // 2
                    t = self._conv1(V(cur), self.w[pre + "conv1"], (n, h, w))
                    cin = self.w[pre + "down"].kg
                    d = self._conv_norm(V(cur, 0, cin), self.w[pre + "down"], (n, h, w), "none", raw_only=True)
                    res = d if self.inorm else V(d)
                    cur = self._conv_norm(t, self.w[pre + "conv2"], (n, h, w), "relu", res=res, s2d=out_s2d)
                if out_s2d:
                    pass
        head = self.w["head"]
        if split_out:
            out = _native.s32_empty(n, h, w, (head.n + 31) // 32, dev)
            _native.conv_s32(V(cur), head, self._bn(head.n), y0=V(out))
        else:
            out = torch.empty((n, head.n, h, w), device=dev, dtype=torch.float32)
            _native.conv_s32(V(cur), head, self._bn(head.n), f32=out)
        if is_list:
            return torch.split(out, [batch_dim, batch_dim], dim=0)
        return out
```

torch-optical-flow_amd/methods/raft/model/raft.py:

```python
from __future__ import annotations

import os
from typing import Any, Dict, List, Optional, Tuple, Union

import torch
import torch.nn as nn
import torch.nn.functional as F
from torch import Tensor

from optical_flow import _native
from optical_flow.metrics import AverageEndPointError, OutlierRatio

from .corr import AlternateCorrBlock, CorrBlock
from .extractor import BasicEncoder, SplitEncoder
from .update import BasicUpdateBlock, FusedUpdate, SplitUpdate, _side_stream, capture_active
from .utils import InputPadder, coords_grid, upflow8

NATIVE_NORMALIZE = True
EARLY_LANE_INIT = True


class HParams(dict):

    def __getattr__(self, key: str) -> Any:
        try:
            return self[key]
        except KeyError as e:
            raise AttributeError(key) from e


def strip_module(state_dict: Dict[str, Tensor]) -> Dict[str, Tensor]:
    return {(k[7:] if k.startswith("module.") else k): v for k, v in state_dict.items()}


def _drop_weight_cache(module: nn.Module, _incompatible) -> None:
    module.__dict__.pop("_split_weights", None)


class RAFT(nn.Module):
    def __init__(
        self,
        hidden_dim: int = 128,
        context_dim: int = 128,
        corr_levels: int = 4,
        corr_radius: int = 4,
        iters: int = 12,
        iters_val: int = 24,
        gamma: float = 0.8,
        dropout: float = 0.0,
        lr: float = 0.00002,
        wdecay: float = 0.00005,
        epsilon: float = 1e-8,
        alternate_corr: bool = False,
    ) -> None:
        super().__init__()
        self.hparams = HParams(
            hidden_dim=hidden_dim,
            context_dim=context_dim,
            corr_levels=corr_levels,
            corr_radius=corr_radius,
            iters=iters,
            iters_val=iters_val,
            gamma=gamma,
            dropout=dropout,
            lr=lr,
            wdecay=wdecay,
            epsilon=epsilon,
            alternate_corr=alternate_corr,
        )
        self.fnet = BasicEncoder(output_dim=256, norm_fn="instance", dropout=dropout)
        self.cnet = BasicEncoder(output_dim=hidden_dim + context_dim, norm_fn="batch", dropout=dropout)
        self.update_block = BasicUpdateBlock(corr_levels=corr_levels, corr_radius=corr_radius, hidden_dim=hidden_dim)
        self.epe_train = AverageEndPointError()
        self.epe_val = AverageEndPointError()
        self.f1_val = OutlierRatio(abs_threshold=3.0, rel_threshold=0.05)
        self.last_train_metrics: Dict[str, float] = {}
        self.update_impl = "split"
        self.fused_update = True
        self.encoder_impl = "split"
        self.upsample_impl = "native"
        self.conv_backward_impl = "aten"
        self.encoder_backward_impl = "aten"
        self.batch_norm_impl = "aten"
        self.encoder_streams = True
        self.fnet_streams = True
        self.pair_lanes = 2
        self.pair_lookup = "joined"
        self.lookup_fusion = True
        self.split_corr = True
        self.stem_from_image = True
        self.range_guard = "deferred"
        self._range_pending = []
        self.last_range_snapshot = None
        for m in (self.fnet, self.cnet, self.update_block):
            m.register_load_state_dict_post_hook(_drop_weight_cache)

    def invalidate_weight_caches(self) -> None:
        for m in (self.fnet, self.cnet, self.update_block):
            _drop_weight_cache(m, None)

    @classmethod
    def load_from_checkpoint(cls, checkpoint_path: Union[str, os.PathLike], map_location=None, **kwargs) -> "RAFT":
        ckpt = torch.load(checkpoint_path, map_location=map_location or "cpu", weights_only=True)
        hp = {}
        if isinstance(ckpt, dict) and "state_dict" in ckpt:
            hp = dict(ckpt.get("hyper_parameters", {}) or {})
            sd = ckpt["state_dict"]
        else:
            sd = ckpt
        hp.update(kwargs)
        model = cls(**{k: v for k, v in hp.items() if k in cls.__init__.__code__.co_varnames})
        sd = {k: v for k, v in strip_module(sd).items() if not k.startswith(("epe_", "f1_"))}
        model.load_state_dict(sd)
        return model

    def freeze_bn(self) -> None:
        for m in self.modules():
            if isinstance(m, nn.BatchNorm2d):
                m.eval()

    def training_step(self, batch: Tuple[Tensor, Tensor, Tensor, Tensor], batch_idx: int = 0) -> Tensor:
        img0, img1, flow, valid = batch
        flow_predictions = self(img0, img1, iters=self.hparams.iters)
        loss, metrics = sequence_loss(flow_predictions, flow, valid, gamma=self.hparams.gamma)
        self.epe_train.update(flow_predictions[-1].detach(), flow, valid)
        self.last_train_metrics = metrics
        return loss

    def unsupervised_step(self, batch: Tuple[Tensor, Tensor], batch_idx: int = 0, w_census: float = 1.0,
                          w_smooth: float = 1.0, smooth_order: int = 1, w_ssim: float = 0.0,
                          w_charbonnier: float = 0.0, ssim_window: int = 3, ssim_sigma: Optional[float] = None) -> Tensor:
        from optical_flow import fb_consistency

        img0, img1 = batch
        preds_fw, preds_bw = self.forward_bidirectional(img0, img1, iters=self.hparams.iters)
        with torch.no_grad():
            occ_fw, occ_bw = fb_consistency(preds_fw[-1], preds_bw[-1], both=True)
        kw = dict(gamma=self.hparams.gamma, w_census=w_census, w_smooth=w_smooth, smooth_order=smooth_order,
                  w_ssim=w_ssim, w_charbonnier=w_charbonnier, ssim_window=ssim_window, ssim_sigma=ssim_sigma)
        return (unsupervised_sequence_loss(preds_fw, img0, img1, mask=~occ_fw, **kw)
                + unsupervised_sequence_loss(preds_bw, img1, img0, mask=~occ_bw, **kw))

    def validation_step(self, batch: Tuple[Tensor, Tensor, Tensor, Tensor], batch_idx: int = 0, stage: str = "sintel") -> None:
        img0, img1, flow_gt, valid = batch
        padder = InputPadder(img0.shape, mode=stage)
        img0, img1 = padder.pad(img0, img1)
        _, flow_pr = self(img0, img1, iters=self.hparams.iters_val, test_mode=True)
        flow_pr = padder.unpad(flow_pr)
        self.epe_val.update(flow_pr, flow_gt, valid)
        self.f1_val.update(flow_pr, flow_gt, valid)

    @staticmethod
    def initialize_flow(img: Tensor) -> Tuple[Tensor, Tensor]:
        n, _, h, w = img.shape
        coords0 = coords_grid(n, h // 8, w // 8, device=img.device)
        return coords0, coords0.clone()

    @staticmethod
    def upsample_flow(flow: Tensor, mask: Tensor, impl: str = "native") -> Tensor:
        if impl not in ("native", "aten"):
            raise ValueError(f"upsample_impl must be 'native' or 'aten', got {impl!r}")
        grad = torch.is_grad_enabled() and (flow.requires_grad or mask.requires_grad)
        if flow.is_cuda and (not grad or impl == "native"):
            return _native.convex_upsample(flow, mask)
        n, _, h, w = flow.shape
        mask = torch.softmax(mask.view(n, 1, 9, 8, 8, h, w), dim=2)
        up_flow = F.unfold(8 * flow, [3, 3], padding=1).view(n, 2, 9, 1, 1, h, w)
        up_flow = torch.sum(mask * up_flow, dim=2).permute(0, 1, 4, 2, 5, 3)
        return up_flow.reshape(n, 2, 8 * h, 8 * w)

    def _lane_cuts(self, b: int):
        n = min(self.pair_lanes, b)
        edges = [(b * i) // n for i in range(n + 1)]
        return list(zip(edges[:-1], edges[1:]))

    def _lane_runners(self, cnet_out: Tensor, hdim: int, lanes, on=None) -> list:
        runners = []
        for i, ((b0, b1), st) in enumerate(zip(self._lane_cuts(cnet_out.shape[0]), lanes)):
            with torch.cuda.stream(on if on is not None else st):
                slot = 0 if i == 0 else 200 + i
                runners.append(SplitUpdate(self.update_block, cnet_out[b0:b1], hdim, side_slot=slot, fuse_c1=self.lookup_fusion,
                                           flow_head_pixels=cnet_out.shape[0] * cnet_out.shape[2] * cnet_out.shape[3],
                                           side_owner=st))
        return runners

    def _lanes_for(self, dev, b: int):
        main = torch.cuda.current_stream(dev)
        return [main] + [_side_stream(dev, 100 + i) for i in range(1, min(self.pair_lanes, b))]

    def _split_update_lanes(self, corr_fn, cnet_out: Tensor, coords0: Tensor, coords1: Tensor, iters: int, hdim: int,
                            test_mode: bool, runners=None) -> List[Tensor]:
        b = cnet_out.shape[0]
        dev = cnet_out.device
        cuts = self._lane_cuts(b)
        main = torch.cuda.current_stream(dev)
        lanes = self._lanes_for(dev, b)
        SplitUpdate._weights(self.update_block)
        init_main = getattr(self, "lane_init_on_main", False) or runners is not None
        if not init_main:
            for st in lanes[1:]:
                st.wait_stream(main)
        if runners is None:
            runners = self._lane_runners(cnet_out, hdim, lanes, on=main if init_main else None)
        if init_main:
            for st in lanes[1:]:
                st.wait_stream(main)
        joined = self.pair_lookup == "joined" and not runners[0].fusable(corr_fn)
        hw = cnet_out.shape[2] * cnet_out.shape[3]
        if joined:
            rows = torch.empty((b * hw, runners[0].corr_ch), device=dev, dtype=torch.float32)
            h, w = cnet_out.shape[2:]
            ins = [_native.F32In(rows[b0 * hw : b1 * hw], b1 - b0, h, w) for b0, b1 in cuts]
        else:
            parts = [corr_fn.batch_slice(b0, b1) for b0, b1 in cuts]
        outs = []
        for itr in range(iters):
            last = itr == iters - 1
            need = not test_mode or last
            mask = torch.empty((b, 576, *cnet_out.shape[2:]), device=dev, dtype=torch.float32) if need else None
            if joined:
                for st in lanes[1:]:
                    main.wait_stream(st)
                corr_fn.lookup_nhwc(coords1, rows)
            if joined or need:
                for st in lanes[1:]:
                    st.wait_stream(main)
            for i, ((b0, b1), st) in enumerate(zip(cuts, lanes)):
                with torch.cuda.stream(st):
                    c1 = coords1[b0:b1]
                    corr_in = ins[i] if joined else runners[i].lookup(parts[i], c1)
                    runners[i].update(corr_in, c1, need, mask_out=mask[b0:b1] if need else None)
            if need:
                for st in lanes[1:]:
                    main.wait_stream(st)
                outs.append(self.upsample_flow(coords1 - coords0, mask))
        for st in lanes[1:]:
            main.wait_stream(st)
        return outs

    def check_range(self, device=None) -> None:
        pend, self._range_pending = self._range_pending, []
        bad = False
        for snap in pend:
            bad |= snap.overflowed()
        if bad:
            raise RuntimeError(f"RAFT forward: in an earlier forward {_native.RANGE_ERROR}")
        if device is not None:
            _native.range_flag_raise_if_set(device, all_streams=True)

    def forward(
        self,
        image0: Tensor,
        image1: Tensor,
        iters: int = 12,
        flow_init: Optional[Tensor] = None,
        upsample: bool = True,
        test_mode: bool = False,
    ) -> Union[Tensor, Tuple[Tensor, Tensor], List[Tensor]]:
        return self._guarded(image0, lambda: self._forward(image0, image1, iters, flow_init, test_mode))

    def forward_bidirectional(
        self,
        image0: Tensor,
        image1: Tensor,
        iters: int = 12,
        flow_init: Optional[Tuple[Optional[Tensor], Optional[Tensor]]] = None,
        test_mode: bool = False,
    ):
        n = image0.shape[0]
        init = None
        if flow_init is not None:
            if not isinstance(flow_init, (tuple, list)) or len(flow_init) != 2:
                raise TypeError("forward_bidirectional: flow_init must be None or a pair (init_fw, init_bw), either of "
                                "which may be None")
            init_fw, init_bw = flow_init
            if init_fw is not None or init_bw is not None:
                ref = init_fw if init_fw is not None else init_bw
                init = torch.cat([torch.zeros_like(ref) if t is None else t for t in (init_fw, init_bw)], dim=0)
        if self.fnet.training and self.fnet.dropout is not None:
            stacked0, stacked1 = torch.cat([image0, image1], dim=0), torch.cat([image1, image0], dim=0)
            out = self._guarded(image0, lambda: self._forward(stacked0, stacked1, iters, init, test_mode))
        else:
            out = self._guarded(image0, lambda: self._forward(image0, image1, iters, init, test_mode, both=True))
        if test_mode:
            low, up = out
            return (low[:n], up[:n]), (low[n:], up[n:])
        return [p[:n] for p in out], [p[n:] for p in out]

    def _guarded(self, image0: Tensor, run):
        guard = self.range_guard in ("sync", "deferred") and image0.is_cuda and not torch.is_grad_enabled()
        capturing = image0.is_cuda and capture_active(image0.device)
        if guard and not capturing:
            self._range_before(image0.device)
        out = run()
        if guard and not capturing:
            self._range_after(image0.device)
        return out

    def _range_before(self, dev) -> None:
        _native.range_flag(dev)
        if self.range_guard != "deferred":
            return
        bad = False
        while self._range_pending and self._range_pending[0].done():
            bad |= self._range_pending.pop(0).overflowed()
        if bad:
            raise RuntimeError(f"RAFT forward: in an earlier forward {_native.RANGE_ERROR}")

    def _range_after(self, dev) -> None:
        snap = _native.RangeSnapshot(torch.device(dev)).take()
        self.last_range_snapshot = snap
        if self.range_guard == "sync":
            if snap.overflowed():
                raise RuntimeError(f"RAFT forward: {_native.RANGE_ERROR}")
        else:
            self._range_pending.append(snap)

    def _encode(self, image0: Tensor, image1: Tensor, hdim: int, both: bool):
        if (NATIVE_NORMALIZE and image0.is_cuda and image1.is_cuda and image0.dtype == image1.dtype == torch.float32
                and image0.shape == image1.shape
                and not (torch.is_grad_enabled() and (image0.requires_grad or image1.requires_grad))):
            image0, image1 = _native.normalize_images(image0, image1)
        else:
            image0 = (2 * (image0 / 255.0) - 1.0).contiguous()
            image1 = (2 * (image1 / 255.0) - 1.0).contiguous()
        first = torch.cat([image0, image1], dim=0) if both else image0

        def sides(a, b):
            return (torch.cat([a, b], dim=0), torch.cat([b, a], dim=0)) if both else (a, b)

        split_enc = (
            image0.is_cuda
            and not torch.is_grad_enabled()
            and self.encoder_impl == "split"
            and (not self.fnet.training or self.fnet.dropout is None)
        )
        fnet = SplitEncoder(self.fnet) if split_enc else self.fnet
        cnet = SplitEncoder(self.cnet) if split_enc and not self.cnet.training else self.cnet
        block = AlternateCorrBlock if self.hparams.get("alternate_corr", False) else CorrBlock
        pre_runners = None
        if split_enc and isinstance(cnet, SplitEncoder):
            main = torch.cuda.current_stream(image0.device)
            side = _side_stream(image0.device) if self.encoder_streams else None
            ni = image0.shape[0]
            nb = first.shape[0]
            side2 = (_side_stream(image0.device, 1) if side is not None and self.fnet_streams
                     and block is CorrBlock and self.split_corr else None)
            sfi = self.stem_from_image
            patches = None if sfi or not both else fnet.stem_patches(first)
            if side2 is not None:
                side2.wait_stream(main)
                with torch.cuda.stream(side2):
                    f2s = fnet(image1, patches=None if patches is None else patches[ni:], split_out=True,
                               stem_from_image=sfi)
                if not both:
                    patches = None if sfi else fnet.stem_patches(image0)
            elif not both:
                patches = None if sfi else fnet.stem_patches(torch.cat([image0, image1], dim=0))
            cpatches = None if patches is None else patches[:nb]
            early = (EARLY_LANE_INIT and side is not None and self.fused_update and self.update_impl == "split"
                     and self.pair_lanes > 1 and nb > 1 and block is CorrBlock and self.split_corr)
            lanes = self._lanes_for(image0.device, nb) if early else None
            if side is not None:
                side.wait_stream(main)
                with torch.cuda.stream(side):
                    cnet_out = cnet(first, patches=cpatches, stem_from_image=sfi)
                    if early:
                        SplitUpdate._weights(self.update_block)
                        pre_runners = self._lane_runners(cnet_out, hdim, lanes, on=side)
            if block is CorrBlock and self.split_corr:
                if side2 is not None:
                    f1s = fnet(image0, patches=patches[:ni] if both and patches is not None else patches, split_out=True,
                               stem_from_image=sfi)
                    main.wait_stream(side2)
                else:
                    f1s, f2s = fnet([image0, image1], patches=patches, split_out=True, stem_from_image=sfi)
                corr_fn = CorrBlock.from_split_features(*sides(f1s, f2s), radius=self.hparams.corr_radius)
            else:
                fmap1, fmap2 = fnet([image0, image1], patches=patches, stem_from_image=sfi)
                corr_fn = block(*sides(fmap1.float(), fmap2.float()), radius=self.hparams.corr_radius)
            if side is not None:
                main.wait_stream(side)
            else:
                cnet_out = cnet(first, patches=cpatches, stem_from_image=sfi)
        else:
            fmap1, fmap2 = fnet([image0, image1])
            corr_fn = block(*sides(fmap1.float(), fmap2.float()), radius=self.hparams.corr_radius)
            cnet_out = cnet(first)
        return corr_fn, cnet_out, pre_runners, first

    def _forward(self, image0: Tensor, image1: Tensor, iters: int, flow_init: Optional[Tensor], test_mode: bool,
                 both: bool = False):
        if self.conv_backward_impl not in ("aten", "native"):
            raise ValueError(f"conv_backward_impl must be 'aten' or 'native', got {self.conv_backward_impl!r}")
        if self.encoder_backward_impl not in ("aten", "native"):
            raise ValueError(f"encoder_backward_impl must be 'aten' or 'native', got {self.encoder_backward_impl!r}")
        if self.batch_norm_impl not in ("aten", "native"):
            raise ValueError(f"batch_norm_impl must be 'aten' or 'native', got {self.batch_norm_impl!r}")
        self.fnet.encoder_backward_impl = self.cnet.encoder_backward_impl = self.encoder_backward_impl
        self.fnet.batch_norm_impl = self.cnet.batch_norm_impl = self.batch_norm_impl
        hdim, cdim = self.hparams.hidden_dim, self.hparams.context_dim
        corr_fn, cnet_out, pre_runners, first = self._encode(image0, image1, hdim, both)
        coords0, coords1 = self.initialize_flow(first)
        if flow_init is not None:
            coords1 = coords1 + flow_init

        gpu_inference = cnet_out.is_cuda and not torch.is_grad_enabled() and self.fused_update
        impl = self.update_impl if gpu_inference else "module"
        flow_predictions = []
        flow_up = None
        if impl == "split" and self.pair_lanes > 1 and cnet_out.shape[0] > 1 and hasattr(corr_fn, "lookup_nhwc"):
            coords1 = coords1.contiguous()
            flow_predictions = self._split_update_lanes(corr_fn, cnet_out, coords0, coords1, iters, hdim, test_mode,
                                                        runners=pre_runners)
            if test_mode:
                return coords1 - coords0, flow_predictions[-1]
            return flow_predictions
        if impl == "split":
            runner = SplitUpdate(self.update_block, cnet_out, hdim, fuse_c1=self.lookup_fusion)
            coords1 = coords1.contiguous()
            for itr in range(iters):
                last = itr == iters - 1
                up_mask = runner.step(corr_fn, coords1, need_mask=not test_mode or last)
                if test_mode and not last:
                    continue
                flow_up = self.upsample_flow(coords1 - coords0, up_mask)
                flow_predictions.append(flow_up)
            if test_mode:
                return coords1 - coords0, flow_up
            return flow_predictions

        self.update_block.conv_backward_impl = self.conv_backward_impl
        net, inp = torch.split(cnet_out, [hdim, cdim], dim=1)
        net = torch.tanh(net)
        inp = torch.relu(inp)
        runner = FusedUpdate(self.update_block, net, inp) if impl == "fused" else None
        for itr in range(iters):
            coords1 = coords1.detach()
            corr = corr_fn(coords1)
            flow = coords1 - coords0
            last = itr == iters - 1
            if runner is not None:
                net, up_mask, delta_flow = runner.step(corr, flow, need_mask=not test_mode or last)
            else:
                net, up_mask, delta_flow = self.update_block(net, inp, corr, flow)
            coords1 = coords1 + delta_flow
            if test_mode and not last:
                continue
            if up_mask is None:
                flow_up = upflow8(coords1 - coords0)
            else:
                flow_up = self.upsample_flow(coords1 - coords0, up_mask, self.upsample_impl)
            flow_predictions.append(flow_up)

        if test_mode:
            return coords1 - coords0, flow_up
        return flow_predictions


def sequence_loss(
    flow_preds: List[Tensor],
    flow_gt: Tensor,
    valid: Tensor,
    gamma: float = 0.8,
    max_flow: float = 400.0,
) -> Tuple[Tensor, Dict[str, float]]:
    n = len(flow_preds)
    weights = [gamma ** (n - i - 1) for i in range(n)]
    if flow_gt.is_cuda:
        loss, stats = _native.ops().sequence_loss(list(flow_preds), flow_gt, valid, weights, float(max_flow))
        s = stats.cpu()
        px = (s[1:4] / s[0]).float().tolist()
        return loss, {"1px": px[0], "3px": px[1], "5px": px[2]}
    return sequence_loss_torch(flow_preds, flow_gt, valid, weights, max_flow)


def sequence_loss_torch(flow_preds, flow_gt: Tensor, valid: Tensor, weights, max_flow: float):
    mag = torch.sum(flow_gt**2, dim=1).sqrt()
    mask = (valid.reshape(mag.shape) >= 0.5) & (mag < max_flow)
    loss = 0.0
    for w, pred in zip(weights, flow_preds):
        loss = loss + w * (mask[:, None] * (pred - flow_gt).abs()).mean()
    epe = torch.sum((flow_preds[-1].detach() - flow_gt) ** 2, dim=1).sqrt()[mask]
    px = torch.stack([(epe < t).float().mean() for t in (1, 3, 5)]).tolist()
    return loss, {"1px": px[0], "3px": px[1], "5px": px[2]}


def unsupervised_sequence_loss(
    flow_preds: List[Tensor],
    image0: Tensor,
    image1: Tensor,
    mask: Optional[Tensor] = None,
    gamma: float = 0.8,
    w_census: float = 1.0,
    w_smooth: float = 1.0,
    smooth_order: int = 1,
    w_ssim: float = 0.0,
    w_charbonnier: float = 0.0,
    ssim_window: int = 3,
    ssim_sigma: Optional[float] = None,
) -> Tensor:
    from optical_flow import census_loss, charbonnier_loss, normalize, smoothness_loss, ssim_loss, warp, warp_grid

    n = len(flow_preds)
    loss = 0.0
    for i, flow in enumerate(flow_preds):
        if flow.is_cuda:
            warped = warp(image1, normalize(flow), align_corners=True)
        else:
            grid = warp_grid(normalize(flow).permute(0, 2, 3, 1))
            warped = F.grid_sample(image1, grid.to(image1.dtype), mode="bilinear", padding_mode="border", align_corners=True)
        term = w_census * census_loss(image0, warped, mask) + w_smooth * smoothness_loss(flow, image0, order=smooth_order)
        if w_ssim != 0:
            term = term + w_ssim * ssim_loss(image0, warped, mask, window=ssim_window, sigma=ssim_sigma)
        if w_charbonnier != 0:
            term = term + w_charbonnier * charbonnier_loss(image0, warped, mask)
        loss = loss + gamma ** (n - 1 - i) * term
    return loss
```

torch-optical-flow_amd/methods/raft/model/update.py:

```python
from __future__ import annotations

import contextlib
import os
import threading
from typing import Optional, Tuple

import torch
import torch.nn as nn
import torch.nn.functional as F
from torch import Tensor

from optical_flow import _native



CONV_BN = {"c2": 96, "f1": 128, "f2": 64, "mo": 128, "gru": 128, "fh1": 64}
CONV_BN_SIDE = dict(CONV_BN, c2=64, fh1=128)
CONV_BLOCKS = (32, 64, 96, 128)


def parse_block_overrides(var: str, keys) -> dict:
    spec = os.environ.get(var, "")
    out = {}
    for kv in filter(None, (s.strip() for s in spec.split(","))):
# ... 187 lines not shown
        if need_mask:
            m = _native.bias_act_(self._conv(net, blk.mask[0]), blk.mask[0].bias, "relu")
            mask = _native.bias_act_(self._conv(m, blk.mask[2]), blk.mask[2].bias, "none", scale=0.25)
        return net, mask, delta_flow


class FusedLookup:

    __slots__ = ("pyr", "coords", "radius")

    def __init__(self, pyr, coords: Tensor, radius: int) -> None:
        self.pyr, self.coords, self.radius = pyr, coords, radius


_SIDE_STREAMS = {}


def _side_stream(device: torch.device, slot: int = 0) -> "torch.cuda.Stream":
    dev = torch.device(device)
    owner = torch.cuda.current_stream(dev).stream_id
    key = (dev.index, owner, slot)
    if key not in _SIDE_STREAMS:
        _SIDE_STREAMS[key] = torch.cuda.Stream(device=device)
    return _SIDE_STREAMS[key]


_CAPTURE = threading.local()


@contextlib.contextmanager
def capturing(device: torch.device):
    depth = _CAPTURE.__dict__.setdefault("depth", {})
    idx = torch.device(device).index
    depth[idx] = depth.get(idx, 0) + 1
    try:
        yield
    finally:
        depth[idx] -= 1


def capture_active(device: Optional[torch.device] = None) -> bool:
    idx = torch.device(device).index if device is not None else torch.cuda.current_device()
    if _CAPTURE.__dict__.get("depth", {}).get(idx, 0) > 0:
        return True
    return torch.cuda.is_current_stream_capturing()


def _module_device(module: nn.Module) -> Optional[torch.device]:
    for p in module.parameters():
        return p.device
    return None


def cached_pack(module: nn.Module, key, build):
    dev = _module_device(module)
    on_gpu = dev is not None and dev.type == "cuda"
    cache = module.__dict__.get("_split_weights")
    if cache is not None and cache[0] == key:
        if cache[2] is not None and on_gpu and not capture_active(dev):
            torch.cuda.current_stream(dev).wait_event(cache[2])
        return cache[1]
    if on_gpu:
        with torch.cuda.device(dev):
            w = build()
            ev = torch.cuda.Event()
            ev.record(torch.cuda.current_stream(dev))
    else:
        w, ev = build(), None
    module.__dict__["_split_weights"] = (key, w, ev)
    return w


def tensor_key(q: Tensor):
    return (q.data_ptr(), -1 if q.is_inference() else q._version)


def _weights_key(block: nn.Module):
    return tuple(tensor_key(q) for q in block.parameters())


class SplitUpdate:

    def __init__(self, block: BasicUpdateBlock, cnet_out: Tensor, hdim: int, side_slot: int = 0,
                 fuse_c1: bool = True, flow_head_pixels: Optional[int] = None, side_owner=None) -> None:
        b, c, h, w = cnet_out.shape
        enc, gru = block.encoder, block.gru
        cdim = c - hdim
        if (hdim, cdim, enc.conv.out_channels, gru.convz1.in_channels) != (128, 128, 126, 384):
            raise RuntimeError("SplitUpdate: supports the RAFT (large) update block only")
        dev = cnet_out.device
        self.block, self.shape = block, (b, h, w)
        px = b * h * w if flow_head_pixels is None else int(flow_head_pixels)
        self.flow_head_fma = px < _native.FLOW_HEAD2_MAX_PIXELS
        self.f1_from_flow = px >= CONVF1_FROM_FLOW_MIN_PIXELS
        S = _native.s32_empty
        self.hx = S(b, h, w, 8, dev)
        self.rhx = S(b, h, w, 8, dev)
        levels, radius = block.corr_levels, block.corr_radius
        self.corr_ch = levels * (2 * radius + 1) ** 2
        self.corr_f32 = None
        self.c1 = S(b, h, w, 8, dev)
        self.cf = S(b, h, w, 8, dev)
        self.pm = None if self.f1_from_flow else S(b, h, w, 4, dev)
        self.f1 = S(b, h, w, 4, dev)
        self.fh = S(b, h, w, 8, dev)
        self.flow_head_mode = getattr(block, "flow_head_mode", FLOW_HEAD_MODE)
        self.fused_head = self.flow_head_mode == "fused" and not self.flow_head_fma
        self.fhy = _native.flow_head_partial_empty(b, h, w, dev) if self.fused_head else None
        self.flow_for = None
        self.hm = torch.empty((b * h * w, hdim), device=dev, dtype=torch.float32)
        self.z = torch.empty_like(self.hm)
        V = _native.S32Slice
        _native.pack_s32(cnet_out[:, :hdim], "tanh", V(self.hx, 0, 4), nhwc=self.hm)
        inp = S(b, h, w, 4, dev)
        _native.pack_s32(cnet_out[:, hdim:], "relu", V(inp))
        self.w = self._weights(block)
        self.gx = []
        for tag in ("1", "2"):
            gx = torch.empty((b * h * w, 3 * hdim), device=dev, dtype=torch.float32)
            _native.conv_s32(V(inp), self.w["inp" + tag], 128, nhwc=gx)
            self.gx.append(gx)
        self.fuse_c1 = fuse_c1 and "c1L" in self.w
        self.streams = getattr(block, "split_streams", True)
        self.side_stream = None
        if self.streams:
            if side_owner is None:
                self.side_stream = _side_stream(dev, side_slot)
            else:
                with torch.cuda.stream(side_owner):
                    self.side_stream = _side_stream(dev, side_slot)

    @staticmethod
    def _weights(block: BasicUpdateBlock):
        return cached_pack(block, _weights_key(block), lambda: SplitUpdate._pack(block))

    @staticmethod
    def _pack(block: BasicUpdateBlock):
        enc, gru, fh = block.encoder, block.gru, block.flow_head
        CW = _native.ConvWeights
        w = {
            "c1": CW(enc.convc1.weight, enc.convc1.bias, 256),
            "c2": CW(enc.convc2.weight, enc.convc2.bias, 192),
            "f1": CW(enc.convf1.weight, enc.convf1.bias, 128, patches=True),
            "f2": CW(enc.convf2.weight, enc.convf2.bias, 64),
            "mo": CW(enc.conv.weight, enc.conv.bias, 128),
            "fh1": CW(fh.conv1.weight, fh.conv1.bias, 256),
            "fh2": CW(fh.conv2.weight, fh.conv2.bias, 32),
            "fh2_bias": fh.conv2.bias.detach().float().contiguous(),
            "fh2_f32": (fh.conv2.weight.detach().float().contiguous(), fh.conv2.bias.detach().float().contiguous()),
            "fh2_tiled": (_native.flow_head2_tiled_weights(fh.conv2.weight), fh.conv2.bias.detach().float().contiguous()),
            "fh2_fused": _native.flow_head_fused_weights(fh.conv2.weight),
            "m1": CW(block.mask[0].weight, block.mask[0].bias, 256),
            "m2": CW(block.mask[2].weight, block.mask[2].bias, 576),
        }
        if block.corr_radius in (3, 4):
            w["c1L"] = _native.convc1_level_weights(enc.convc1, block.corr_levels, block.corr_radius)
        for tag in ("1", "2"):
            cz, cr, cq = (getattr(gru, f"conv{g}{tag}") for g in "zrq")
            hmf = lambda wt: torch.cat([wt[:, :128], wt[:, 256:]], dim=1)
            w["zr" + tag] = CW(hmf(torch.cat([cz.weight, cr.weight])), None, 256)
            w["q" + tag] = CW(hmf(cq.weight), None, 128)
            w["inp" + tag] = CW(torch.cat([cz.weight, cr.weight, cq.weight])[:, 128:256],
                                torch.cat([cz.bias, cr.bias, cq.bias]), 384)
        return w

    def step(self, corr_fn, coords1: Tensor, need_mask: bool, mask_out: Optional[Tensor] = None) -> Optional[Tensor]:
        return self.update(self.lookup(corr_fn, coords1), coords1, need_mask, mask_out)

    def lookup_rows(self, coords1: Tensor) -> Tensor:
        if self.corr_f32 is None:
            b, h, wd = self.shape
            self.corr_f32 = torch.empty((b * h * wd, self.corr_ch), device=coords1.device, dtype=torch.float32)
        return self.corr_f32

    def fusable(self, corr_fn) -> bool:
        return self.fuse_c1 and getattr(corr_fn, "_tiled", None) is not None and corr_fn.radius in (3, 4)

    def lookup(self, corr_fn, coords1: Tensor):
        if self.fusable(corr_fn):
            return FusedLookup(corr_fn._tiled, coords1, corr_fn.radius)
        b, h, wd = self.shape
        corr_fn.lookup_nhwc(coords1, self.lookup_rows(coords1))
        return _native.F32In(self.corr_f32, b, h, wd)

    def _convc1(self, corr_in) -> None:
        if isinstance(corr_in, FusedLookup):
            _native.corr_lookup_convc1(corr_in.pyr, corr_in.coords, corr_in.radius, self.w["c1L"], _native.S32Slice(self.c1))
        else:
            _native.conv_s32(corr_in, self.w["c1"], 128, "relu", y0=_native.S32Slice(self.c1))

    def update(self, corr_in, coords1: Tensor, need_mask: bool, mask_out: Optional[Tensor] = None) -> Optional[Tensor]:
        V, conv, w = _native.S32Slice, _native.conv_s32, self.w
        main = torch.cuda.current_stream(coords1.device)
        side = self.side_stream if self.streams else None
        bns = CONV_BN_SIDE if side is not None else CONV_BN
        f1_in = V(self.pm) if self.pm is not None else _native.FlowIn(coords1)
        fused = self.fused_head and coords1.is_contiguous()
        flow_key = (coords1.data_ptr(), tuple(coords1.shape))
        prep = self.pm is not None or not fused or self.flow_for != flow_key
        self.flow_for = None
        if side is not None:
            side.wait_stream(main)
            with torch.cuda.stream(side):
                if prep:
                    _native.flow_prep(coords1, self.pm, (V(self.hx), 254), (V(self.rhx), 254))
                conv(f1_in, w["f1"], bns["f1"], "relu", y0=V(self.f1))
                conv(V(self.f1), w["f2"], bns["f2"], "relu", y0=V(self.cf, 6, 2))
            self._convc1(corr_in)
            conv(V(self.c1), w["c2"], bns["c2"], "relu", y0=V(self.cf, 0, 6))
            main.wait_stream(side)
        else:
            if prep:
                _native.flow_prep(coords1, self.pm, (V(self.hx), 254), (V(self.rhx), 254))
            self._convc1(corr_in)
            conv(V(self.c1), w["c2"], bns["c2"], "relu", y0=V(self.cf, 0, 6))
            conv(f1_in, w["f1"], bns["f1"], "relu", y0=V(self.f1))
            conv(V(self.f1), w["f2"], bns["f2"], "relu", y0=V(self.cf, 6, 2))
        conv(V(self.cf), w["mo"], bns["mo"], "relu", y0=V(self.hx, 4, 4), y1=V(self.rhx, 4, 4))
        for tag, gx in zip(("1", "2"), self.gx):
            conv(V(self.hx), w["zr" + tag], bns["gru"], epilogue=1, y0=V(self.rhx, 0, 4), gru_h=self.hm, gru_z=self.z,
                 addend=gx[:, :256])
            conv(V(self.rhx), w["q" + tag], bns["gru"], epilogue=2, y0=V(self.hx, 0, 4), gru_h=self.hm, gru_z=self.z,
                 addend=gx[:, 256:])
        net = V(self.hx, 0, 4)
        if fused:
            _native.conv_s32_flow_head(net, w["fh1"], bns["fh1"], w["fh2_fused"], self.fhy)
            _native.flow_head_finish(self.fhy, w["fh2_bias"], coords1, (V(self.hx), 254), (V(self.rhx), 254))
            self.flow_for = flow_key
            return self._mask(net, coords1, mask_out) if need_mask else None
        conv(net, w["fh1"], bns["fh1"], "relu", y0=V(self.fh))
        if self.flow_head_fma and coords1.is_contiguous():
            _native.flow_head2(V(self.fh), *w["fh2_f32"], coords1)
        elif self.flow_head_mode == "tiled" and coords1.is_contiguous():
            _native.flow_head2_tiled(V(self.fh), *w["fh2_tiled"], coords1)
        else:
            conv(V(self.fh), w["fh2"], 32, f32=coords1, f32_accumulate=True)
        return self._mask(net, coords1, mask_out) if need_mask else None

    def _mask(self, net, coords1: Tensor, mask_out: Optional[Tensor]) -> Tensor:
        V, conv, w = _native.S32Slice, _native.conv_s32, self.w
        b, h, wd = self.shape
        mask = mask_out if mask_out is not None else torch.empty((b, 576, h, wd), device=coords1.device, dtype=torch.float32)
        conv(net, w["m1"], 128, "relu", y0=V(self.fh))
        conv(V(self.fh), w["m2"], 64, out_scale=0.25, f32=mask)
        return mask
```

torch-optical-flow_amd/optical_flow/_native.py:

```python
from __future__ import annotations

import ctypes
import os
from typing import List, Optional, Sequence

import torch

from . import _ops

_LIB_PATH = os.environ.get(
    "OFLOW_LIB", os.path.join(os.path.dirname(os.path.abspath(__file__)), "_lib", "liboflow_hip.so")
)
ABI_VERSION = 3
MAX_LEVELS = 8
MAX_RADIUS = 7
FLOW_HEAD2_MAX_PIXELS = 16384
E_TINY = -4

INTERP = {"bilinear": 0, "nearest": 1, "bicubic": 2}
PADDING = {"zeros": 0, "border": 1, "reflection": 2}

class ConvS32Desc(ctypes.Structure):
    _P, _I, _L = ctypes.c_void_p, ctypes.c_int, ctypes.c_longlong
    _fields_ = [
        ("struct_size", ctypes.c_uint),
        ("in_format", _I), ("in_groups", _I), ("d_x", _P), ("x_pixel_stride", _L), ("d_in_scale", _P), ("d_in_shift", _P),
        ("d_wpack", _P), ("d_wfrag", _P), ("d_wscale", _P), ("d_bias", _P), ("n_pad", _I), ("N", _I),
        ("B", _I), ("H", _I), ("W", _I), ("kh", _I), ("kw", _I), ("block_n", _I),
        ("epilogue", _I), ("activation", _I), ("out_scale", ctypes.c_float),
        ("d_y0", _P), ("d_y1", _P), ("y0_pixel_stride", _L), ("y1_pixel_stride", _L),
        ("d_f32", _P), ("f32_batch_stride", _L), ("f32_channel_stride", _L), ("f32_accumulate", _I),
        ("d_gru_h", _P), ("d_gru_z", _P), ("gru_channels", _I),
        ("d_nhwc", _P), ("d_stats", _P), ("d_res", _P), ("res_pixel_stride", _L),
        ("nhwc_pixel_stride", _I), ("res_activation", _I), ("s2d", _I), ("d_addend", _P), ("addend_pixel_stride", _L),
        ("d_fh_weights", _P), ("d_fh_partial", _P), ("fh_slabs", _I),
    ]


def _signatures():
    P, I, F, L, D = ctypes.c_void_p, ctypes.c_int, ctypes.c_float, ctypes.c_longlong, ctypes.c_double
    IP, PP, FP = ctypes.POINTER(I), ctypes.POINTER(P), ctypes.POINTER(F)
    strided_wgrad = (I, [P, P, I, I, I, I, I, I, I, I, P, P, P, P])
    return {
        "oflow_abi_version": (I, []),
        "oflow_status_string": (ctypes.c_char_p, [I]),
        "oflow_corr_pyramid_dims": (I, [I, I, I, IP, IP]),
        "oflow_corr_pyramid_f32": (I, [P, P, I, I, I, I, I, PP, P]),
        "oflow_corr_lookup_f32": (I, [PP, IP, IP, I, P, I, I, I, I, P, P]),
        "oflow_corr_tiled_level_floats": (L, [I, I]),
        "oflow_corr_pyramid_tiled_f32": (I, [P, P, I, I, I, I, I, PP, P]),
        "oflow_corr_lookup_tiled_f32": (I, [PP, IP, IP, I, P, I, I, I, I, P, P]),
        "oflow_corr_untile_f32": (I, [P, P, L, I, I, P]),
        "oflow_grid_warp_f32": (I, [P, P, I, I, I, I, I, I, I, P, P]),
        "oflow_grid_sample_f32": (I, [P, P, I, I, I, I, I, I, I, I, I, P, P]),
        "oflow_corr_otf_prepare_f16": (I, [P, P, I, I, I, I, I, P, PP, P, P]),
        "oflow_corr_lookup_otf_f16": (I, [P, PP, IP, IP, I, P, I, I, I, I, I, P, P]),
        "oflow_bias_act_f32": (I, [P, L, P, P, L, P, L, I, I, I, I, F, P]),
        "oflow_gru_reset_f32": (I, [P, L, P, P, L, P, L, I, I, I, P]),
        "oflow_gru_blend_f32": (I, [P, L, P, P, L, P, P, L, I, I, I, P]),
        "oflow_conv_s32": (I, [ctypes.POINTER(ConvS32Desc), P]),
        "oflow_pack_s32_f32": (I, [P, L, I, I, I, I, I, I, P, L, P, L, P, I, P]),
        "oflow_flow_prep_s32": (I, [P, I, I, I, P, P, L, P, L, P]),
        "oflow_stem_patches_s32": (I, [P, I, I, I, I, P, I, P]),
        "oflow_norm_stats_finalize": (I, [P, I, I, I, I, D, P, P, P]),
        "oflow_norm_apply_s32": (I, [P, I, I, I, I, P, P, I, I, P, L, P, P, P, I, I, P, L, P]),
        "oflow_convex_upsample_f32": (I, [P, P, I, I, I, P, P]),
        "oflow_corr_lookup_tiled_nhwc_f32": (I, [PP, IP, IP, I, P, I, I, I, I, P, I, P]),
        "oflow_corr_lookup_backward_f32": (I, [P, P, I, I, I, I, PP, IP, IP, I, P]),
        "oflow_corr_pyramid_grad_combine_f32": (I, [PP, IP, IP, I, L, P]),
        "oflow_flow_stats_f32": (I, [P, I, I, I, I, F, F, I, P, P]),
        "oflow_flow2rgb_f32": (I, [P, I, I, I, I, I, F, F, I, I, F, P, P, P]),
        "oflow_flow_pack_f32": (I, [P, I, I, I, I, I, P, P]),
        "oflow_corr_lookup_convc1_s32": (I, [PP, IP, IP, I, P, I, I, I, I, P, P, P, P, L, P]),
        "oflow_corr_pyramid_tiled_s32": (I, [P, P, I, I, I, I, I, PP, P]),
        "oflow_flow_head2_s32": (I, [P, L, I, P, P, I, I, I, P, P]),
        "oflow_flow_head2_tiled_s32": (I, [P, L, I, P, P, I, I, I, P, P]),
        "oflow_normalize_images_f32": (I, [P, P, L, P, P, P]),
        "oflow_replicate_pad_f32": (I, [P, P, I, L, I, I, I, I, I, I, P]),
        "oflow_corr_fmap_grad_f32": (I, [P, P, P, I, I, I, F, P, P, P]),
        "oflow_grid_warp_backward_f32": (I, [P, P, P, I, I, I, I, I, I, I, P, P, P]),
        "oflow_grid_sample_backward_f32": (I, [P, P, P, I, I, I, I, I, I, I, I, I, P, P, P]),
        "oflow_set_range_flag": (I, [P]),
        "oflow_range_flag_exchange": (I, [P, P, P]),
        "oflow_flow_head_col2im_f32": (I, [P, P, I, I, I, P, P]),
        "oflow_flow_head_finish_f32": (I, [P, I, P, I, I, I, P, P, L, P, L, P]),
        "oflow_timing_event_create": (I, [PP]),
        "oflow_timing_event_destroy": (I, [P]),
        "oflow_timing_event_record": (I, [P, P, I]),
        "oflow_timing_event_elapsed_ms": (I, [P, P, FP]),
        "oflow_flow_error_stats_f32": (I, [P, L, L, L, P, L, L, L, P, I, L, L, I, I, I, F, F, F, P, P, P, P]),
        "oflow_sequence_loss_f32": (I, [PP, I, FP, P, P, I, I, I, I, F, P, P, P, P]),
        "oflow_sequence_loss_backward_f32": (I, [P, PP, PP, I, FP, P, P, I, I, I, I, F, P]),
        "oflow_convex_upsample_backward_f32": (I, [P, P, P, I, I, I, P, P, P, P]),
        "oflow_corr_lookup_otf_backward_f32": (I, [P, P, PP, IP, IP, I, P, I, I, I, I, I, P, P, P, P]),
        "oflow_forward_interpolate_f32": (I, [P, I, I, I, P, P]),
        "oflow_augment_stats_u8": (I, [P, P, P, I, I, I, I, P, P]),
        "oflow_augment_dense_f32": (I, [P, P, P, P, P, I, I, I, I, I, P, P, P, P, P]),
        "oflow_augment_sparse_flow_f32": (I, [P, P, P, I, I, I, I, I, P, P, P]),
        "oflow_conv2d_backward_input_f32": (I, [P, P, I, I, I, I, I, I, I, P, P]),
        "oflow_conv2d_backward_weight_slab_pixels": (I, []),
        "oflow_conv2d_backward_weight_workspace_floats": (L, [I, I, I, I, I, I, I]),
        "oflow_conv2d_backward_weight_f32": (I, [P, P, I, I, I, I, I, I, I, P, P, P, P]),
        "oflow_conv2d_strided_backward_input_f32": (I, [P, P, I, I, I, I, I, I, I, I, P, P]),
        "oflow_conv2d_strided_backward_weight_workspace_floats": (L, [I, I, I, I, I, I, I, I]),
        "oflow_conv2d_strided_backward_weight_f32": strided_wgrad,
        "oflow_conv2d_strided_backward_weight_generic_f32": strided_wgrad,
        "oflow_instance_norm_backward_f32": (I, [P, P, I, I, D, I, P, P]),
        "oflow_frozen_batch_norm_backward_workspace_floats": (L, [I, I, I]),
        "oflow_frozen_batch_norm_backward_f32": (I, [P, P, P, P, P, P, I, I, I, D, I, P, P, P, P, P]),
        "oflow_batch_norm_chunk_elements": (I, []),
        "oflow_batch_norm_workspace_floats": (L, [I, I, I]),
        "oflow_batch_norm_forward_f32": (I, [P, P, P, I, I, I, D, I, P, P, P, P, P]),
        "oflow_batch_norm_backward_f32": (I, [P, P, P, P, P, P, I, I, I, D, I, P, P, P, P, P]),
        "oflow_fb_consistency_f32": (I, [P, P, I, I, I, F, F, P, P, P, P, P]),
        "oflow_splat_frac_bits": (I, [I, I]),
        "oflow_splat_workspace_bytes": (L, [I, I, I, I]),
        "oflow_splat_f32": (I, [P, P, P, I, I, I, I, I, P, P, P, P]),
        "oflow_splat_backward_f32": (I, [P, P, P, P, P, P, I, I, I, I, I, P, P, P, P, P]),
        "oflow_census_loss_workspace_bytes": (L, [I, I, I]),
        "oflow_census_loss_f32": (I, [P, P, P, I, I, I, I, I, I, F, P, P, P, P, P]),
        "oflow_census_loss_backward_f32": (I, [P, P, P, P, I, P, P, I, I, I, I, I, F, P, P, P]),
        "oflow_smoothness_loss_workspace_bytes": (L, [I, I, I]),
        "oflow_smoothness_loss_f32": (I, [P, P, I, I, I, I, I, F, F, P, P, P]),
        "oflow_smoothness_loss_backward_f32": (I, [P, P, P, I, I, I, I, I, F, F, P, P]),
        "oflow_ssim_loss_workspace_bytes": (L, [I, I, I]),
        "oflow_ssim_loss_f32": (I, [P, P, P, I, I, I, I, I, I, FP, F, F, P, P, P, P, P]),
        "oflow_ssim_loss_backward_f32": (I, [P, P, P, P, I, P, I, I, I, I, I, FP, F, F, P, P, P]),
        "oflow_charbonnier_loss_f32": (I, [P, P, P, I, I, I, I, I, F, F, F, P, P, P, P]),
        "oflow_charbonnier_loss_backward_f32": (I, [P, P, P, P, I, P, I, I, I, I, F, F, F, P, P, P]),
    }


_SIGNATURES = _signatures()
SYMBOLS = tuple(_SIGNATURES)


_lib = None
_recorder = None
_flops = None


def set_flop_counter(counter):
    global _flops
    _flops = counter


def _count(exec_f16: int, useful: int, fma: int = 0) -> None:
    _flops["exec_f16"] = _flops.get("exec_f16", 0) + exec_f16
    _flops["useful"] = _flops.get("useful", 0) + useful
    _flops["fma_f32"] = _flops.get("fma_f32", 0) + fma


def set_event_recorder(recorder):
    global _recorder
    _recorder = recorder


class TimingEvent:

    __slots__ = ("ev",)

    def __init__(self):
        ev = ctypes.c_void_p()
        _check(load().oflow_timing_event_create(ctypes.byref(ev)), "timing_event_create")
        self.ev = ev

    def record(self, stream: "torch.cuda.Stream") -> None:
        _check(load().oflow_timing_event_record(self.ev, ctypes.c_void_p(stream.cuda_stream), 1), "timing_event_record")

    def elapsed_time(self, end: "TimingEvent") -> float:
        ms = ctypes.c_float()
        _check(load().oflow_timing_event_elapsed_ms(self.ev, end.ev, ctypes.byref(ms)), "timing_event_elapsed_ms")
        return float(ms.value)

    def __del__(self):
        try:
            if _lib is not None and self.ev:
                _lib.oflow_timing_event_destroy(self.ev)
        except Exception:
            pass


_TIMED_DEFAULT = ("corr_lookup", "corr_lookup_convc1", "corr_pyramid", "corr_lookup_otf", "corr_otf_prepare", "grid_warp")


class _Timed:
    __slots__ = ("what", "stream", "ev0")

    def __init__(self, what: str, device: torch.device):
        self.what = what
        on = _recorder is not None and (what in _TIMED_DEFAULT or _recorder.get("*", False))
        self.stream = torch.cuda.current_stream(device) if on else None
        self.ev0 = None

    def __enter__(self):
        if self.stream is not None:
            self.ev0 = TimingEvent() if _recorder.get("_native") else torch.cuda.Event(enable_timing=True)
            self.ev0.record(self.stream)
        return self

    def __exit__(self, *exc):
        if self.stream is not None and exc[0] is None and _recorder is not None:
            ev1 = TimingEvent() if _recorder.get("_native") else torch.cuda.Event(enable_timing=True)
            ev1.record(self.stream)
            _recorder.setdefault(self.what, []).append((self.ev0, ev1))
        return False


def library_path() -> str:
    return _LIB_PATH


def load() -> ctypes.CDLL:
    global _lib
    if _lib is not None:
        return _lib
    if not os.path.exists(_LIB_PATH):
        raise RuntimeError(
            f"liboflow_hip.so not found at {_LIB_PATH}: build it with `make -C torch-optical-flow_amd/csrc` "
            "(or __graft_entry__.build()); the MI355X path has no CPU fallback"
        )
    lib = ctypes.CDLL(_LIB_PATH)
    for name, (restype, argtypes) in _SIGNATURES.items():
        fn = getattr(lib, name)
        fn.restype, fn.argtypes = restype, argtypes
    v = lib.oflow_abi_version()
    if v != ABI_VERSION:
        raise RuntimeError(f"liboflow_hip.so ABI version {v}, expected {ABI_VERSION}: rebuild the library")
    _ops.load()
    _lib = lib
    return lib


def ops():
    if _lib is None:
        load()
    return torch.ops.oflow


def _run(what: str, device: torch.device, op, *args):
    if _recorder is None:
        return op(*args)
    with _Timed(what, device):
        return op(*args)


def _tensor(t, name: str, what: str) -> torch.Tensor:
    if not isinstance(t, torch.Tensor):
        raise TypeError(f"{what}: {name} must be a torch.Tensor")
    return t


def _no_grad_input(t: torch.Tensor, name: str, what: str) -> None:
    if t.requires_grad and torch.is_grad_enabled():
        raise RuntimeError(
            f"{what}: {name} requires grad; this layout is inference-only (no backward): use CorrBlock's canonical "
            "pyramid (corr_pyramid / corr_lookup have autograd), or run under torch.no_grad()"
        )


def _check(status: int, what: str) -> None:
    if status == 0:
        return
    msg = load().oflow_status_string(status).decode()
    if status == E_TINY:
        raise ValueError(f"{what}: {msg}")
    raise RuntimeError(f"{what} failed ({status}): {msg}")


def _gpu_f32(t: torch.Tensor, name: str, what: str) -> torch.Tensor:
    if not isinstance(t, torch.Tensor):
        raise TypeError(f"{what}: {name} must be a torch.Tensor")
    if t.device.type != "cuda":
        raise RuntimeError(
            f"{what}: {name} is on {t.device}; this MI355X build runs only on ROCm GPU tensors (no CPU fallback)"
        )
    if t.requires_grad and torch.is_grad_enabled():
        raise RuntimeError(
            f"{what}: {name} requires grad; this entry point is an inference layout with no autograd formula: use "
            "CorrBlock / optical_flow.warp (native backward kernels), or run under torch.no_grad() / "
            "torch.inference_mode(), or detach the input"
        )
# ... 328 lines not shown
               "kernels represent exactly; the output is not valid (OFLOW_CHECK=1 names the convolution)")


def range_flag_raise_if_set(device: torch.device, what: str = "RAFT forward", all_streams: bool = False) -> None:
    device = torch.device(device)
    if all_streams:
        torch.cuda.synchronize(device)
    if RangeSnapshot(device).take().overflowed():
        raise RuntimeError(f"{what}: {RANGE_ERROR}")


CHECK_RANGE = os.environ.get("OFLOW_CHECK", "0") not in ("", "0")
F16_MAX = 65504.0
CONV_BREG = True
CONV_BREG64 = False
CONV_BREG32 = False


def _range_check(x, what: str) -> None:
    if isinstance(x, S32Slice):
        v = x.t[:, :, :, x.g0 : x.g0 + x.ng, 0]
    elif isinstance(x, NhwcNormIn):
        b, h, w = x.bhw
        c = x.raw.shape[1]
        v = torch.relu(x.raw.view(b, h * w, c) * x.scale.view(b, 1, c) + x.shift.view(b, 1, c))
    else:
        v = x.raw
    m = float(v.abs().amax().float()) if v.numel() else 0.0
    if not m <= F16_MAX:
        raise RuntimeError(
            f"{what}: input max |x| = {m:g} is outside the fp16 range (65504) of the split-fp16 operands (OFLOW_CHECK)"
        )


def _chan_view(t: torch.Tensor, what: str):
    if t.device.type != "cuda" or t.dtype != torch.float32 or t.dim() != 4:
        raise RuntimeError(f"{what}: expected a 4-D fp32 ROCm tensor, got {t.dtype} {tuple(t.shape)} on {t.device}")
    b, c, h, w = t.shape
    if t.stride(3) != 1 or t.stride(2) != w or t.stride(1) != h * w:
        raise RuntimeError(f"{what}: the (C, H, W) part must be contiguous")
    return t.data_ptr(), t.stride(0), c, h * w


def bias_act_(x: torch.Tensor, bias, act: str = "relu", scale: float = 1.0, out=None, out2=None) -> torch.Tensor:
    px, sx, c, p = _chan_view(x, "bias_act")
    y = x if out is None else out
    py, sy, cy, py_ = _chan_view(y, "bias_act out")
    p2, s2 = (0, 0)
    if out2 is not None:
        p2, s2, c2, _ = _chan_view(out2, "bias_act out2")
        if c2 != c:
            raise RuntimeError("bias_act: out2 channel count differs")
    if cy != c or py_ != p or y.shape[0] != x.shape[0]:
        raise RuntimeError("bias_act: output shape differs from input")
    if bias is not None and (bias.numel() != c or bias.dtype != torch.float32 or not bias.is_contiguous()):
        raise RuntimeError("bias_act: bias must be a contiguous fp32 vector of C elements")
    with torch.cuda.device(x.device):
        _check(
            load().oflow_bias_act_f32(
                px, sx, bias.data_ptr() if bias is not None else None, py, sy, p2 or None, s2, x.shape[0], c, p,
                ACT[act], float(scale), _stream(x.device)
            ),
            "bias_act",
        )
    return y


def gru_reset(zr: torch.Tensor, br: torch.Tensor, h: torch.Tensor, rh: torch.Tensor) -> None:
    pz, sz, c2, p = _chan_view(zr, "gru_reset zr")
    ph, sh, ch, p1 = _chan_view(h, "gru_reset h")
    pr, sr, cr, p2 = _chan_view(rh, "gru_reset rh")
    if c2 != 2 * ch or cr != ch or p1 != p or p2 != p or br.numel() != ch:
        raise RuntimeError("gru_reset: inconsistent shapes")
    with torch.cuda.device(h.device):
        _check(load().oflow_gru_reset_f32(pz, sz, br.data_ptr(), ph, sh, pr, sr, h.shape[0], ch, p, _stream(h.device)), "gru_reset")


def gru_blend_(zr: torch.Tensor, bz: torch.Tensor, q: torch.Tensor, bq: torch.Tensor, h: torch.Tensor) -> None:
    pz, sz, c2, p = _chan_view(zr, "gru_blend zr")
    pq, sq, cq, p1 = _chan_view(q, "gru_blend q")
    ph, sh, ch, p2 = _chan_view(h, "gru_blend h")
    if c2 != 2 * ch or cq != ch or p1 != p or p2 != p or bz.numel() != ch or bq.numel() != ch:
        raise RuntimeError("gru_blend: inconsistent shapes")
    with torch.cuda.device(h.device):
        _check(
            load().oflow_gru_blend_f32(pz, sz, bz.data_ptr(), pq, sq, bq.data_ptr(), ph, sh, h.shape[0], ch, p, _stream(h.device)),
            "gru_blend",
        )




class S32Slice:

    __slots__ = ("t", "g0", "ng")

    def __init__(self, t: torch.Tensor, g0: int = 0, ng: int = -1):
        if t.dtype != torch.float16 or t.dim() != 6 or tuple(t.shape[-2:]) != (2, 32) or not t.is_contiguous():
            raise RuntimeError(f"S32 tensor must be contiguous fp16 (B, H, W, G, 2, 32), got {t.dtype} {tuple(t.shape)}")
        self.t, self.g0 = t, int(g0)
        self.ng = int(t.shape[3]) - self.g0 if ng < 0 else int(ng)
        if self.g0 < 0 or self.g0 + self.ng > t.shape[3]:
            raise RuntimeError("S32Slice: group range outside the tensor")

    @property
    def ptr(self) -> int:
        return self.t.data_ptr() + self.g0 * 128

    @property
    def ps(self) -> int:
        return int(self.t.shape[3]) * 128

    def channel_ptr(self, c: int) -> int:
        return self.ptr + (c // 32) * 128 + (c % 32) * 2

    @property
    def bhw(self):
        return tuple(int(v) for v in self.t.shape[:3])

    @property
    def device(self):
        return self.t.device


class F32In:

    __slots__ = ("raw", "bhw")
    in_format = 2

    def __init__(self, raw: torch.Tensor, b: int, h: int, w: int):
        if raw.dtype != torch.float32 or not raw.is_contiguous() or raw.shape[0] != b * h * w or raw.shape[1] % 4:
            raise RuntimeError("F32In: raw must be contiguous fp32 [B*H*W, C], C % 4 == 0")
        self.raw, self.bhw = raw, (int(b), int(h), int(w))

    @property
    def ptr(self) -> int:
        return self.raw.data_ptr()

    @property
    def ps(self) -> int:
        return int(self.raw.shape[1]) * 4

    @property
    def ng(self) -> int:
        return (int(self.raw.shape[1]) + 31) // 32

    @property
    def device(self):
        return self.raw.device


class ImgIn:

    __slots__ = ("raw", "bhw")
    in_format = 3

    def __init__(self, img: torch.Tensor):
        if img.dtype != torch.float32 or img.dim() != 4 or img.shape[1] != 3 or not img.is_contiguous():
            raise RuntimeError("ImgIn: the image must be contiguous fp32 (B, 3, H, W)")
        b, _, hh, ww = img.shape
        if hh % 2 or ww % 2:
            raise RuntimeError("ImgIn: H and W must be even")
        self.raw, self.bhw = img, (int(b), int(hh) // 2, int(ww) // 2)

    @property
    def ptr(self) -> int:
        return self.raw.data_ptr()

    @property
    def ps(self) -> int:
        return 0

    @property
    def ng(self) -> int:
        return 5

    @property
    def device(self):
        return self.raw.device


class FlowIn:

    __slots__ = ("raw", "bhw")
    in_format = 4

    def __init__(self, coords: torch.Tensor):
        if coords.dtype != torch.float32 or coords.dim() != 4 or coords.shape[1] != 2 or not coords.is_contiguous():
            raise RuntimeError("FlowIn: coords must be contiguous fp32 (B, 2, H, W)")
        b, _, hh, ww = coords.shape
        self.raw, self.bhw = coords, (int(b), int(hh), int(ww))

    @property
    def ptr(self) -> int:
        return self.raw.data_ptr()

    @property
    def ps(self) -> int:
        return 0

    @property
    def ng(self) -> int:
        return 4

    @property
    def device(self):
        return self.raw.device


class NhwcNormIn:

    __slots__ = ("raw", "bhw", "scale", "shift")
    in_format = 1

    def __init__(self, raw: torch.Tensor, b: int, h: int, w: int, scale: torch.Tensor, shift: torch.Tensor):
        c = raw.shape[1]
        if raw.dtype != torch.float32 or not raw.is_contiguous() or raw.shape[0] != b * h * w or c % 32:
            raise RuntimeError("NhwcNormIn: raw must be contiguous fp32 [B*H*W, C], C % 32 == 0")
        for t in (scale, shift):
            if t.dtype != torch.float32 or not t.is_contiguous() or t.numel() != b * c:
                raise RuntimeError("NhwcNormIn: scale / shift must be contiguous fp32 [B, C]")
        self.raw, self.bhw, self.scale, self.shift = raw, (int(b), int(h), int(w)), scale, shift

    @property
    def ptr(self) -> int:
        return self.raw.data_ptr()

    @property
    def ps(self) -> int:
        return int(self.raw.shape[1]) * 4

    @property
    def ng(self) -> int:
        return int(self.raw.shape[1]) // 32

    @property
    def device(self):
        return self.raw.device


def s32_empty(b: int, h: int, w: int, groups: int, device, zero: bool = False) -> torch.Tensor:
    f = torch.zeros if zero else torch.empty
    return f((b, h, w, groups, 2, 32), device=device, dtype=torch.float16)


def s32_from_f32(x: torch.Tensor, groups: int = -1) -> torch.Tensor:
    b, c, h, w = x.shape
    g = (c + 31) // 32 if groups < 0 else groups
    v = torch.zeros((b, h, w, g * 32), device=x.device, dtype=torch.float32)
    v[..., :c] = x.permute(0, 2, 3, 1)
    hi = v.half()
    lo = (v - hi.float()).half()
    return torch.stack([hi.view(b, h, w, g, 32), lo.view(b, h, w, g, 32)], dim=4).contiguous()


def s32_to_f32(t: torch.Tensor, channels: int = -1) -> torch.Tensor:
    b, h, w, g = t.shape[:4]
    v = (t[:, :, :, :, 0].float() + t[:, :, :, :, 1].float()).reshape(b, h, w, g * 32)
    c = g * 32 if channels < 0 else channels
    return v[..., :c].permute(0, 3, 1, 2).contiguous()


class ConvWeights:

    __slots__ = ("pack", "wscale", "bias", "n", "n_pad", "kh", "kw", "kg", "layout", "cin", "_frag")

    def __init__(self, weight: torch.Tensor, bias, n_pad: int, patches: bool = False):
        w = weight.detach().float()
        if patches:
            n, c, kh, kw = w.shape
            w = w.permute(0, 2, 3, 1).reshape(n, kh * kw * c, 1, 1)
        n, c, kh, kw = w.shape
        if n_pad < n:
            raise RuntimeError("ConvWeights: n_pad < out channels")
        amax = w.abs().amax(dim=(1, 2, 3))
        e = torch.where(amax > 0, torch.ceil(torch.log2(amax)), torch.zeros_like(amax)).clamp(-100, 100)
        scale = torch.exp2(14.0 - e)
        ws = w * scale.view(-1, 1, 1, 1)
        kg = (c + 31) // 32
        t = kh * kw
        full = torch.zeros((n_pad, kg * 32, t), device=w.device, dtype=torch.float32)
        full[:n, :c] = ws.reshape(n, c, t)
        full = full.view(n_pad, kg, 32, t).permute(1, 3, 0, 2).contiguous()
        hi = full.half()
        lo = (full - hi.float()).half()
        self.pack = torch.stack([hi, lo], dim=3).contiguous()
        inv = torch.ones(n_pad, device=w.device, dtype=torch.float32)
        inv[:n] = 1.0 / scale
        self.wscale = inv
        self.bias = None if bias is None else bias.detach().float().contiguous()
        self.n, self.n_pad, self.kh, self.kw, self.kg = n, n_pad, kh, kw, kg
        self.cin = c
        self.layout = "conv"
        self._frag = None
        if t > 1 and n_pad % 32 == 0:
            self.frag()

    def frag(self) -> torch.Tensor:
        if self._frag is None:
            if self.layout != "conv" or self.n_pad % 32:
                raise RuntimeError("ConvWeights.frag: needs a conv-layout pack with n_pad a multiple of 32")
            kg, t = self.pack.shape[:2]
            f = self.pack.reshape(kg, t, self.n_pad // 32, 32, 2, 2, 2, 8)
            self._frag = f.permute(0, 1, 2, 5, 4, 6, 3, 7).contiguous()
        return self._frag


def convc1_level_weights(conv: torch.nn.Conv2d, num_levels: int, radius: int) -> "ConvWeights":
    kk = (2 * radius + 1) ** 2
    g = (kk + 31) // 32
    w = conv.weight.detach().float()
    if tuple(w.shape[1:]) != (num_levels * kk, 1, 1):
        raise RuntimeError(f"convc1_level_weights: expected a 1x1 conv over {num_levels * kk} channels, got {tuple(w.shape)}")
    wp = w.new_zeros((w.shape[0], num_levels * g * 32, 1, 1))
    for l in range(num_levels):
        wp[:, l * g * 32 : l * g * 32 + kk] = w[:, l * kk : (l + 1) * kk]
    cw = ConvWeights(wp, conv.bias, w.shape[0])
    lg = cw.pack.shape[0]
    frag = cw.pack.reshape(lg, 4, 2, 32, 2, 2, 2, 8)
    cw.pack = frag.permute(0, 1, 2, 5, 4, 6, 3, 7).contiguous()
    cw.layout = "convc1_frag"
    cw.cin = num_levels * kk
    return cw


def corr_lookup_convc1(pyr: "TiledPyramid", coords: torch.Tensor, radius: int, cw: "ConvWeights", y: "S32Slice") -> None:
    what = "corr_lookup_convc1"
    co = _gpu_f32(coords, "coords", what)
    b, two, h, w = co.shape
    if two != 2 or b * h * w != pyr.queries:
        raise RuntimeError(f"{what}: coords (B, 2, H, W) must cover the pyramid's {pyr.queries} queries")
    kk = (2 * radius + 1) ** 2
    if (cw.layout != "convc1_frag" or cw.n != 256 or cw.n_pad != 256 or cw.kh * cw.kw != 1
            or cw.kg != len(pyr.levels) * ((kk + 31) // 32)):
        raise RuntimeError(f"{what}: weights must be convc1_level_weights of this pyramid / radius")
    if y.ng != 8 or y.bhw != (b, h, w) or y.device != co.device:
        raise RuntimeError(f"{what}: destination must be an 8-group S32 slice of shape ({b}, {h}, {w})")
    n = len(pyr.levels)
    ptrs = (ctypes.c_void_p * MAX_LEVELS)(*[t.data_ptr() for t in pyr.levels])
    hs = (ctypes.c_int * MAX_LEVELS)(*[d[0] for d in pyr.dims])
    ws = (ctypes.c_int * MAX_LEVELS)(*[d[1] for d in pyr.dims])
    if _flops is not None:
        _count(3 * 2 * b * h * w * 256 * cw.kg * 32, 2 * b * h * w * 256 * cw.cin)
    with torch.cuda.device(co.device), _Timed(what, co.device):
        _check(
            load().oflow_corr_lookup_convc1_s32(
                ptrs, hs, ws, n, co.data_ptr(), b, h, w, int(radius), cw.pack.data_ptr(), cw.wscale.data_ptr(),
                cw.bias.data_ptr() if cw.bias is not None else None, y.ptr, y.ps, _stream(co.device),
            ),
            what,
        )


def conv_tiles(h: int, w: int) -> int:
    return ((h + 3) // 4) * ((w + 31) // 32)


def _conv_desc(x, cw: ConvWeights, block_n: int) -> ConvS32Desc:
    b, h, w = x.bhw
    return ConvS32Desc(
        struct_size=ctypes.sizeof(ConvS32Desc), in_format=getattr(x, "in_format", 0), in_groups=cw.kg, d_x=x.ptr,
        x_pixel_stride=x.ps, d_wpack=cw.pack.data_ptr(), d_wscale=cw.wscale.data_ptr(),
        d_bias=cw.bias.data_ptr() if cw.bias is not None else None, n_pad=cw.n_pad, N=cw.n, B=b, H=h, W=w, kh=cw.kh,
        kw=cw.kw, block_n=int(block_n),
    )


def conv_s32(x: S32Slice, cw: ConvWeights, block_n: int, act: str = "none", out_scale: float = 1.0, y0=None, y1=None,
             f32=None, f32_accumulate: bool = False, epilogue: int = 0, gru_h=None, gru_z=None, nhwc=None, stats=None,
             res=None, res_act: str = "none", s2d: bool = False, addend=None) -> None:
    what = "conv_s32"
    if CHECK_RANGE:
        _range_check(x, f"{what} {cw.kh}x{cw.kw}")
    if x.ng != cw.kg:
        raise RuntimeError(f"{what}: input has {x.ng} groups, weights expect {cw.kg}")
    b, h, w = x.bhw
    d = _conv_desc(x, cw, block_n)
    d.epilogue, d.activation, d.res_activation, d.s2d = int(epilogue), ACT[act], ACT[res_act], int(bool(s2d))
    d.out_scale = float(out_scale)
    hw_out = (h // 2, w // 2) if s2d else (h, w)
    for dst in (y0, y1):
        if dst is not None and (tuple(dst.t.shape[:3]) != (b, *hw_out) or dst.t.device != x.device):
            raise RuntimeError(f"{what}: destination shape/device mismatch")
    if y0 is not None:
        d.d_y0, d.y0_pixel_stride = y0.ptr, y0.ps
    if y1 is not None:
        d.d_y1, d.y1_pixel_stride = y1.ptr, y1.ps
    if res is not None:
        if tuple(res.t.shape[:3]) != (b, h, w) or res.ng * 32 < cw.n:
            raise RuntimeError(f"{what}: residual shape mismatch")
        d.d_res, d.res_pixel_stride = res.ptr, res.ps
    if f32 is not None:
        if f32.dtype != torch.float32 or f32.dim() != 4 or tuple(f32.shape[2:]) != (h, w) or f32.shape[0] != b:
            raise RuntimeError(f"{what}: fp32 destination must be (B, C, H, W) fp32")
        if f32.stride(3) != 1 or f32.stride(2) != w or f32.shape[1] < cw.n and epilogue == 0:
            raise RuntimeError(f"{what}: fp32 destination planes must be contiguous with >= N channels")
        d.d_f32, d.f32_batch_stride, d.f32_channel_stride = f32.data_ptr(), f32.stride(0), f32.stride(1)
        d.f32_accumulate = int(bool(f32_accumulate))
    if nhwc is not None:
        if nhwc.dtype != torch.float32 or not nhwc.is_contiguous() or nhwc.numel() != b * h * w * cw.n:
            raise RuntimeError(f"{what}: nhwc destination must be contiguous fp32 [P, {cw.n}]")
        d.d_nhwc, d.nhwc_pixel_stride = nhwc.data_ptr(), cw.n
    if stats is not None:
        if stats.dtype != torch.float32 or stats.numel() < b * conv_tiles(h, w) * cw.n_pad * 3:
            raise RuntimeError(f"{what}: stats partials buffer too small")
        d.d_stats = stats.data_ptr()
    if epilogue:
        gch = cw.n // 2 if epilogue == 1 else cw.n
        for tt in (gru_h, gru_z):
            if tt is None or tt.dtype != torch.float32 or not tt.is_contiguous() or tt.numel() != b * h * w * gch:
                raise RuntimeError(f"{what}: GRU state tensors must be contiguous fp32 [P, {gch}]")
        d.d_gru_h, d.d_gru_z, d.gru_channels = gru_h.data_ptr(), gru_z.data_ptr(), gch
    if addend is not None:
        if (not epilogue or addend.dtype != torch.float32 or addend.dim() != 2 or addend.stride(1) != 1
                or addend.shape[0] != b * h * w or addend.shape[1] < cw.n or addend.stride(0) % 4
                or addend.data_ptr() % 16 or addend.device != x.device):
            raise RuntimeError(f"{what}: addend must be a GRU-epilogue fp32 [P, >= {cw.n}] view with 16-B aligned rows")
        d.d_addend, d.addend_pixel_stride = addend.data_ptr(), addend.stride(0)
    if d.in_format == NhwcNormIn.in_format:
        d.d_in_scale, d.d_in_shift = x.scale.data_ptr(), x.shift.data_ptr()
    if (CONV_BREG and (d.block_n == 128 or (CONV_BREG64 and d.block_n == 64) or (CONV_BREG32 and d.block_n == 32))
            and cw.kh * cw.kw > 1 and d.in_format == 0 and cw.layout == "conv"):
        d.d_wfrag = cw.frag().data_ptr()
    if _flops is not None:
        taps, p_out = cw.kh * cw.kw, b * h * w
        n_exec = -(-cw.n_pad // d.block_n) * d.block_n
        _count(3 * 2 * p_out * n_exec * cw.kg * 32 * taps, 2 * p_out * cw.n * cw.cin * taps)
    with torch.cuda.device(x.device), _Timed(f"conv{cw.kh}x{cw.kw}", x.device):
        _check(load().oflow_conv_s32(ctypes.byref(d), _stream(x.device)), what)


def flow_head2(x: "S32Slice", weight: torch.Tensor, bias: torch.Tensor, coords: torch.Tensor) -> None:
    what = "flow_head2"
    b, h, w = x.bhw
    if weight.dtype != torch.float32 or not weight.is_contiguous() or tuple(weight.shape) != (2, x.ng * 32, 3, 3):
        raise RuntimeError(f"{what}: weight must be contiguous fp32 (2, {x.ng * 32}, 3, 3)")
    if bias is None or bias.dtype != torch.float32 or tuple(bias.shape) != (2,):
        raise RuntimeError(f"{what}: bias must be fp32 (2,)")
    if coords.dtype != torch.float32 or not coords.is_contiguous() or tuple(coords.shape) != (b, 2, h, w):
        raise RuntimeError(f"{what}: coords must be contiguous fp32 ({b}, 2, {h}, {w})")
    if _flops is not None:
        fl = 2 * b * h * w * 2 * x.ng * 32 * 9
        _count(0, fl, fl)
    with torch.cuda.device(coords.device), _Timed("conv3x3", coords.device):
        _check(load().oflow_flow_head2_s32(x.ptr, x.ps, x.ng, weight.data_ptr(), bias.data_ptr(), b, h, w,
                                           coords.data_ptr(), _stream(coords.device)), what)


def flow_head2_tiled_weights(weight: torch.Tensor) -> torch.Tensor:
    o, c = weight.shape[:2]
    if o != 2 or c % 32 or tuple(weight.shape[2:]) != (3, 3):
        raise RuntimeError("flow_head2_tiled_weights: weight must be (2, C, 3, 3) with C a multiple of 32")
    w = weight.detach().float().reshape(2, c // 32, 8, 4, 3, 3)
    return w.permute(1, 2, 4, 5, 0, 3).contiguous()


def flow_head2_tiled(x: "S32Slice", wr: torch.Tensor, bias: torch.Tensor, coords: torch.Tensor) -> None:
    what = "flow_head2_tiled"
    b, h, w = x.bhw
    if wr.dtype != torch.float32 or not wr.is_contiguous() or wr.numel() != 2 * x.ng * 32 * 9 or wr.data_ptr() % 16:
        raise RuntimeError(f"{what}: wr must be flow_head2_tiled_weights of a (2, {x.ng * 32}, 3, 3) weight")
    if bias is None or bias.dtype != torch.float32 or tuple(bias.shape) != (2,):
        raise RuntimeError(f"{what}: bias must be fp32 (2,)")
    if coords.dtype != torch.float32 or not coords.is_contiguous() or tuple(coords.shape) != (b, 2, h, w):
        raise RuntimeError(f"{what}: coords must be contiguous fp32 ({b}, 2, {h}, {w})")
    if _flops is not None:
        fl = 2 * b * h * w * 2 * x.ng * 32 * 9
        _count(0, fl, fl)
    with torch.cuda.device(coords.device), _Timed("conv3x3", coords.device):
        _check(load().oflow_flow_head2_tiled_s32(x.ptr, x.ps, x.ng, wr.data_ptr(), bias.data_ptr(), b, h, w,
                                                 coords.data_ptr(), _stream(coords.device)), what)


def flow_head_col2im(y: torch.Tensor, bias: torch.Tensor, coords: torch.Tensor) -> None:
    what = "flow_head_col2im"
    b, _, h, w = coords.shape
    if coords.dtype != torch.float32 or not coords.is_contiguous() or coords.shape[1] != 2 or coords.device.type != "cuda":
        raise RuntimeError(f"{what}: coords must be contiguous fp32 (B, 2, H, W) on the GPU")
    if y.dtype != torch.float32 or not y.is_contiguous() or tuple(y.shape) != (b, 18, h, w) or y.device != coords.device:
        raise RuntimeError(f"{what}: y must be contiguous fp32 ({b}, 18, {h}, {w})")
    if bias is None or bias.dtype != torch.float32 or tuple(bias.shape) != (2,) or bias.device != coords.device:
        raise RuntimeError(f"{what}: bias must be fp32 (2,) on the coords' device")
    with torch.cuda.device(coords.device), _Timed("flow_head_col2im", coords.device):
        _check(load().oflow_flow_head_col2im_f32(y.data_ptr(), bias.data_ptr(), b, h, w, coords.data_ptr(),
                                                 _stream(coords.device)), what)


FLOW_HEAD_SLABS = 4


def flow_head_fused_weights(weight: torch.Tensor) -> torch.Tensor:
    if tuple(weight.shape) != (2, 64 * FLOW_HEAD_SLABS, 3, 3):
        raise RuntimeError(f"flow_head_fused_weights: weight must be (2, {64 * FLOW_HEAD_SLABS}, 3, 3)")
    return weight.detach().float().permute(1, 2, 3, 0).reshape(FLOW_HEAD_SLABS, 64, 18).contiguous()


def flow_head_partial_empty(b: int, h: int, w: int, device) -> torch.Tensor:
    return torch.empty((FLOW_HEAD_SLABS, b, 18, h, w), device=device, dtype=torch.float32)


def conv_s32_flow_head(x: "S32Slice", cw: "ConvWeights", block_n: int, w2r: torch.Tensor, partial) -> None:
    what = "conv_s32_flow_head"
    if x.ng != cw.kg:
        raise RuntimeError(f"{what}: input has {x.ng} groups, weights expect {cw.kg}")
    b, h, w = x.bhw
    dev = x.device
    if (w2r.dtype != torch.float32 or not w2r.is_contiguous() or tuple(w2r.shape[1:]) != (64, 18) or w2r.device != dev):
        raise RuntimeError(f"{what}: w2r must be flow_head_fused_weights(conv2.weight) on the input's device")
    d = _conv_desc(x, cw, block_n)
    d.epilogue, d.activation, d.out_scale = 3, ACT["relu"], 1.0
    d.d_fh_weights = w2r.data_ptr()
    if partial is not None:
        if (partial.dtype != torch.float32 or not partial.is_contiguous() or partial.dim() != 5
                or tuple(partial.shape[1:]) != (b, 18, h, w) or partial.device != dev):
            raise RuntimeError(f"{what}: partial must be contiguous fp32 (slabs, {b}, 18, {h}, {w}) on the input's device")
        d.fh_slabs, d.d_fh_partial = int(partial.shape[0]), partial.data_ptr()
    if w2r.shape[0] != FLOW_HEAD_SLABS:
        d.fh_slabs = -1
    if d.block_n == 128 and cw.layout == "conv":
        d.d_wfrag = cw.frag().data_ptr()
    if _flops is not None:
        n_exec = -(-cw.n_pad // d.block_n) * d.block_n
        _count(3 * 2 * b * h * w * n_exec * cw.kg * 32 * 9, 2 * b * h * w * cw.n * cw.cin * 9)
        fl = 2 * b * h * w * 2 * cw.n * 9
        _count(0, fl, fl)
    with torch.cuda.device(dev), _Timed("conv3x3", dev):
        _check(load().oflow_conv_s32(ctypes.byref(d), _stream(dev)), what)


def flow_head_finish(partial: torch.Tensor, bias: torch.Tensor, coords: torch.Tensor, flow0=None, flow1=None) -> None:
    what = "flow_head_finish"
    if (coords.dtype != torch.float32 or coords.dim() != 4 or coords.shape[1] != 2 or not coords.is_contiguous()
            or coords.device.type != "cuda"):
        raise RuntimeError(f"{what}: coords must be contiguous fp32 (B, 2, H, W) on the GPU")
    b, _, h, w = coords.shape
    if (partial.dtype != torch.float32 or not partial.is_contiguous() or partial.dim() != 5
            or tuple(partial.shape[1:]) != (b, 18, h, w) or partial.device != coords.device):
        raise RuntimeError(f"{what}: partial must be contiguous fp32 (slabs, {b}, 18, {h}, {w})")
    if bias is None or bias.dtype != torch.float32 or tuple(bias.shape) != (2,) or bias.device != coords.device:
        raise RuntimeError(f"{what}: bias must be fp32 (2,) on the coords' device")
    for fl in (flow0, flow1):
        if fl is not None and (fl[0].bhw != (b, h, w) or fl[0].device != coords.device):
            raise RuntimeError(f"{what}: flow destination shape/device mismatch")
    f0 = (flow0[0].channel_ptr(flow0[1]), flow0[0].ps) if flow0 is not None else (None, 0)
    f1 = (flow1[0].channel_ptr(flow1[1]), flow1[0].ps) if flow1 is not None else (None, 0)
    with torch.cuda.device(coords.device), _Timed("flow_head_finish", coords.device):
        _check(load().oflow_flow_head_finish_f32(partial.data_ptr(), int(partial.shape[0]), bias.data_ptr(), b, h, w,
                                                 coords.data_ptr(), f0[0], f0[1], f1[0], f1[1],
                                                 _stream(coords.device)), what)


def stem_patches(img: torch.Tensor, out: torch.Tensor) -> torch.Tensor:
    x = _gpu_f32(img, "image", "stem_patches")
    b, c, h, w = x.shape
    if out.dtype != torch.float16 or tuple(out.shape[:3]) != (b, (h + 1) // 2, (w + 1) // 2):
        raise RuntimeError("stem_patches: output must be S32 (B, ceil(H/2), ceil(W/2), G, 2, 32)")
    with torch.cuda.device(x.device), _Timed("stem_patches", x.device):
        _check(load().oflow_stem_patches_s32(x.data_ptr(), b, c, h, w, out.data_ptr(), int(out.shape[3]), _stream(x.device)), "stem_patches")
    return out


def norm_stats(partials: torch.Tensor, b: int, tiles: int, n_pad: int, c: int, eps: float):
    alpha = torch.empty((b, c), device=partials.device, dtype=torch.float32)
    beta = torch.empty_like(alpha)
    with torch.cuda.device(partials.device):
        _check(
            load().oflow_norm_stats_finalize(partials.data_ptr(), b, tiles, n_pad, c, float(eps), alpha.data_ptr(), beta.data_ptr(), _stream(partials.device)),
            "norm_stats",
        )
    return alpha, beta


def norm_apply(x: torch.Tensor, shape, alpha, beta, act: str, y: S32Slice, res=None, res_raw=None, res_act: str = "none",
               s2d: bool = False, res_raw_relu: bool = False) -> None:
    b, c, h, w = shape
    mode, rp, rps = 0, None, 0
    x2 = a2 = b2 = None
    if res is not None:
        mode, rp, rps = 1, res.ptr, res.ps
    elif res_raw is not None:
        mode = 3 if res_raw_relu else 2
        x2, a2, b2 = (t.data_ptr() for t in res_raw)
# ... 92 lines not shown
```

Before: 465.6 image-pairs/s.

## Fuse convex upsampling into mask conv epilogue and image scaling into stem

Adds an upsample epilogue to the 1x1 mask conv. It applies softmax over the 9 mask taps and the convex combination of 8x flow neighbours in registers and writes the full-resolution flow directly. This removes the 576-channel fp32 mask tensor write and re-read and the separate upsample kernel for every iteration that needs output. The stem conv can also apply the /255 image normalization while it loads the image, which removes a separate normalize pass. In exchange, weights are padded from 576 to 768 columns, adding some wasted MFMA work.

```diff
diff --git a/include/oflow.h b/include/oflow.h
--- a/include/oflow.h
+++ b/include/oflow.h
@@ -116,6 +116,16 @@
 } oflow_conv_s32_desc;
 int oflow_conv_s32(const oflow_conv_s32_desc* desc, void* stream);
 
+#define OFLOW_EPI_UPSAMPLE 4
+typedef struct oflow_conv_s32_ext_desc {
+  unsigned int struct_size;
+  int img_scale255;
+  const float *d_up_coords0, *d_up_coords1;
+  float* d_up_out;
+  long long up_batch_stride;
+} oflow_conv_s32_ext_desc;
+int oflow_conv_s32_ext(const oflow_conv_s32_desc* desc, const oflow_conv_s32_ext_desc* ext, void* stream);
+
 int oflow_flow_head_col2im_f32(const float* d_y, const float* d_bias, int B, int H, int W, float* d_coords, void* stream);
 int oflow_flow_head_finish_f32(const float* d_partial, int slabs, const float* d_bias, int B, int H, int W,
                                float* d_coords, void* d_flow0, long long flow0_pixel_stride, void* d_flow1,
diff --git a/torch-optical-flow_amd/csrc/conv_s32.hip b/torch-optical-flow_amd/csrc/conv_s32.hip
--- a/torch-optical-flow_amd/csrc/conv_s32.hip
+++ b/torch-optical-flow_amd/csrc/conv_s32.hip
@@ -1,3 +1,4 @@
+#include "convex_upsample.h"
 #include "oflow_internal.h"
 
 namespace oflow {
@@ -52,8 +53,15 @@
   int exp_flags;
   const float* fhw;
   float* fhy;
+  const float* upc0;
+  const float* upc1;
+  float* upo;
+  long long upbs;
+  int img255;
 };
 constexpr int kEpiFlowHead = OFLOW_EPI_FLOW_HEAD;
+constexpr int kEpiUp = OFLOW_EPI_UPSAMPLE;
+constexpr int kUpRows = kTY + 2, kUpPitch = kTX + 2;
 constexpr int kInS32 = OFLOW_IN_S32, kInF32Norm = OFLOW_IN_F32_NORM, kInF32 = OFLOW_IN_F32, kInImg = OFLOW_IN_IMG7S2,
               kInFlow = OFLOW_IN_FLOW7;
 constexpr int kImgC = 3, kImgK = 7, kImgRows = (kTY - 1) * 2 + kImgK, kImgCols = (kTX - 1) * 2 + kImgK;
@@ -191,6 +199,7 @@
   __shared__ __attribute__((aligned(16))) uint8_t smem[LDS_BYTES + AFF_BYTES];
   __shared__ float2 sSB[BN];
   __shared__ float3 sStat[EPI == 0 ? WM * BN : 1];
+  __shared__ float sUpF[EPI == kEpiUp ? 2 * kUpRows * kUpPitch : 1];
   float2* sAff = reinterpret_cast<float2*>(smem + LDS_BYTES);
   float* sImg = reinterpret_cast<float*>(smem + LDS_BYTES);
   int* sKoff = reinterpret_cast<int*>(smem + LDS_BYTES + (WIN ? IMG_FLOATS * 4 : 0));
@@ -202,7 +211,14 @@
   const int r = lane & 31, hh = lane >> 5;
 
   int tile = blockIdx.x;
-  const int cblk = blockIdx.y;
+  int cblk_ = blockIdx.y;
+  if constexpr (EPI == kEpiUp) {
+    const int id = blockIdx.x, slot = id >> 3;
+    cblk_ = slot & 7;
+    tile = (slot >> 3) * 8 + (id & 7);
+    if (tile >= a.tiles_x * a.tiles_y * a.B) return;
+  }
+  const int cblk = cblk_;
   const int tx0 = (tile % a.tiles_x) * kTX;
   tile /= a.tiles_x;
   const int ty0 = (tile % a.tiles_y) * TY;
@@ -372,6 +388,8 @@
     constexpr int IMG_N = kImgC * kImgRows * kImgCols, IMG_PER = (IMG_N + NTH - 1) / NTH;
     float iv[IMG_PER];
     int io[IMG_PER];
+    unsigned inm = 0u;
+    static_assert(IMG_PER <= 32, "in-image mask");
 #pragma unroll
     for (int s_ = 0; s_ < IMG_PER; ++s_) {
       const int e = min(tid + s_ * NTH, IMG_N - 1);
@@ -381,12 +399,19 @@
       const bool in = static_cast<unsigned>(iy) < static_cast<unsigned>(2 * a.H) && static_cast<unsigned>(ix) < static_cast<unsigned>(2 * a.W);
       const int cy = min(max(iy, 0), 2 * a.H - 1), cx = min(max(ix, 0), 2 * a.W - 1);
       const float v = img[((long long)ch * (2 * a.H) + cy) * (2 * a.W) + cx];
-      iv[s_] = in ? v : 0.f;
+      iv[s_] = v;
+      inm |= (in ? 1u : 0u) << s_;
       io[s_] = ch * kImgPlane + ry * kImgPitch + (rx & 1) * kImgHalf + (rx >> 1);
     }
-#pragma unroll
-    for (int s_ = 0; s_ < IMG_PER; ++s_)
-      if (tid + s_ * NTH < IMG_N) sImg[io[s_]] = iv[s_];
+    if (a.img255) {
+#pragma unroll
+      for (int s_ = 0; s_ < IMG_PER; ++s_)
+        if (tid + s_ * NTH < IMG_N) sImg[io[s_]] = ((inm >> s_) & 1u) ? 2.0f * (iv[s_] / 255.0f) - 1.0f : 0.f;
+    } else {
+#pragma unroll
+      for (int s_ = 0; s_ < IMG_PER; ++s_)
+        if (tid + s_ * NTH < IMG_N) sImg[io[s_]] = ((inm >> s_) & 1u) ? iv[s_] : 0.f;
+    }
   }
   if constexpr (AIN == kInFlow) {
     const float* co = reinterpret_cast<const float*>(a.x) + (long long)b * 2 * a.H * a.W;
@@ -700,7 +725,50 @@
       }
     }
   }
+  if constexpr (EPI == kEpiUp) {
+    const long long HW = (long long)a.H * a.W;
+    for (int e = tid; e < 2 * kUpRows * kUpPitch; e += NTH) {
+      const int c = e / (kUpRows * kUpPitch), rem = e - c * (kUpRows * kUpPitch);
+      const int dy = rem / kUpPitch, dx = rem - dy * kUpPitch;
+      const int yy = ty0 + dy - 1, xx = tx0 + dx - 1;
+      float v = 0.f;
+      if (yy >= 0 && yy < a.H && xx >= 0 && xx < a.W) {
+        const long long o = ((long long)b * 2 + c) * HW + (long long)yy * a.W + xx;
+        const float fl = a.upc1[o] - a.upc0[o];
+        v = 8.0f * fl;
+      }
+      sUpF[e] = v;
+    }
+  }
   __syncthreads();
+  if constexpr (EPI == kEpiUp) {
+    static_assert(EPI != kEpiUp || (BM == 128 && NTH == 256 && BN >= 72), "upsampling epilogue: 4 x 32 tiles, 4 waves");
+    const int xo = tid >> 3, j = tid & 7;
+    const int x = tx0 + xo;
+    if (x < a.W) {
+      float2 sb9[9];
+#pragma unroll
+      for (int k = 0; k < 9; ++k) sb9[k] = sSB[k * 8 + j];
+      const long long W8 = 8LL * a.W, H8W8 = 64LL * a.H * a.W;
+      for (int rr = 0; rr < kTY; ++rr) {
+        const int y = ty0 + rr;
+        if (y >= a.H) break;
+        float m[9];
+#pragma unroll
+        for (int k = 0; k < 9; ++k) {
+          float v = sT[(rr * kTX + xo) * TS + k * 8 + j] * sb9[k].x + sb9[k].y;
+          v = act_fn(v, a.act) * a.oscale;
+          m[k] = v;
+        }
+        float o0, o1;
+        convex_upsample_px(m, &sUpF[rr * kUpPitch + xo], &sUpF[(kUpRows + rr) * kUpPitch + xo], kUpPitch, o0, o1);
+        float* op = a.upo + b * a.upbs + (long long)(8 * y + cblk) * W8 + 8LL * x + j;
+        op[0] = o0;
+        op[H8W8] = o1;
+      }
+    }
+    return;
+  }
   if constexpr (EPI == kEpiFlowHead) {
     constexpr int NSLAB = BN / 64, NPART = NTH / 64 / (2 * NSLAB);
     static_assert(BM == 128 && BN % 64 == 0 && NTH == 256 && (NPART == 1 || NPART == 2), "flow-head epilogue: 4 x 32 tiles, 4 waves");
@@ -953,6 +1021,7 @@
   } else {
   a.tiles_y = (a.H + TY - 1) / TY;
   dim3 grid = conv_grid(a, BN);
+  if constexpr (EPI == kEpiUp) grid = dim3((a.tiles_x * a.tiles_y * a.B + 7) / 8 * 64);
   if constexpr (KH == 3 && KW == 3 && EPI == 0) {
     if (a.ain == kInF32Norm) {
       launch_staged<KH, KW, BN, WM, WN, EPI, TY, kInF32Norm>(a, grid, s);
@@ -1050,6 +1119,9 @@
       if (block_n == 64) return launch_conv<3, 3, 64, 2, 2, kEpiFlowHead>(a, s);
       if (block_n == 128) return a.wf != nullptr ? launch_conv<3, 3, 128, 1, 4, kEpiFlowHead, kTY, true>(a, s) : OFLOW_E_MODE;
       return OFLOW_E_SHAPE;
+    case kEpiUp:
+      if (key != 0x11 || block_n != 96) return OFLOW_E_SHAPE;
+      return launch_conv<1, 1, 96, 4, 1, kEpiUp>(a, s);
     default:
       if (block_n != 128) return OFLOW_E_SHAPE;
       if (small_grid(a, block_n)) {
@@ -1203,6 +1275,40 @@
   return dispatch_conv(a, desc->kh, desc->kw, desc->block_n, desc->epilogue, static_cast<hipStream_t>(stream));
 }
 
+extern "C" int oflow_conv_s32_ext(const oflow_conv_s32_desc* desc, const oflow_conv_s32_ext_desc* ext, void* stream) {
+  if (!desc || !ext) return OFLOW_E_NULL;
+  if (desc->struct_size != sizeof(oflow_conv_s32_desc) || ext->struct_size != sizeof(oflow_conv_s32_ext_desc))
+    return OFLOW_E_MODE;
+  oflow_conv_s32_desc d = *desc;
+  const bool up = d.epilogue == kEpiUp;
+  if (up) {
+    if (!ext->d_up_coords0 || !ext->d_up_coords1 || !ext->d_up_out) return OFLOW_E_NULL;
+    if (d.kh != 1 || d.kw != 1 || d.block_n != 96 || d.n_pad != 768 || d.N != 768 || d.H <= 0 || d.W <= 0 ||
+        ext->up_batch_stride < 128ll * d.H * d.W)
+      return OFLOW_E_SHAPE;
+    if (d.in_format != kInS32 || d.activation != 0 || d.d_y0 || d.d_y1 || d.d_f32 || d.d_gru_h || d.d_gru_z || d.d_nhwc ||
+        d.d_stats || d.d_res || d.s2d || d.d_addend || ext->img_scale255)
+      return OFLOW_E_MODE;
+    if (((uintptr_t)ext->d_up_coords0 & 3) || ((uintptr_t)ext->d_up_coords1 & 3) || ((uintptr_t)ext->d_up_out & 3))
+      return OFLOW_E_ALIGN;
+    d.epilogue = 0;
+    d.d_f32 = ext->d_up_out;
+  }
+  if (ext->img_scale255 && d.in_format != kInImg) return OFLOW_E_MODE;
+  ConvArgs a;
+  const int st = conv_args_from_desc(d, a);
+  if (st != OFLOW_OK) return st;
+  if (up) {
+    a.f = nullptr;
+    a.upc0 = ext->d_up_coords0;
+    a.upc1 = ext->d_up_coords1;
+    a.upo = ext->d_up_out;
+    a.upbs = ext->up_batch_stride;
+  }
+  a.img255 = ext->img_scale255 ? 1 : 0;
+  return dispatch_conv(a, desc->kh, desc->kw, desc->block_n, desc->epilogue, static_cast<hipStream_t>(stream));
+}
+
 extern "C" void oflow_exp_set_small_grid_px(int pixels) { oflow::g_small_grid_px = pixels; }
 extern "C" void oflow_exp_set_stats_8row(int on) { oflow::g_stats_8row = on; }
 extern "C" void oflow_exp_set_conv_flags(int flags) { oflow::g_conv_exp_flags = flags; }
diff --git a/torch-optical-flow_amd/csrc/convex_upsample.h b/torch-optical-flow_amd/csrc/convex_upsample.h
--- /dev/null
+++ b/torch-optical-flow_amd/csrc/convex_upsample.h
@@ -0,0 +1,32 @@
+#ifndef OFLOW_CONVEX_UPSAMPLE_H_
+#define OFLOW_CONVEX_UPSAMPLE_H_
+
+#include <hip/hip_runtime.h>
+
+namespace oflow {
+
+__device__ __forceinline__ void convex_upsample_px(float (&m)[9], const float* f0, const float* f1, int pitch, float& o0,
+                                                   float& o1) {
+  float mx = m[0];
+#pragma unroll
+  for (int k = 0; k < 9; ++k) mx = fmaxf(mx, m[k]);
+  float s = 0.f;
+#pragma unroll
+  for (int k = 0; k < 9; ++k) {
+    m[k] = expf(m[k] - mx);
+    s += m[k];
+  }
+  o0 = 0.f;
+  o1 = 0.f;
+#pragma unroll
+  for (int k = 0; k < 9; ++k) {
+    const float w = m[k] / s;
+    const int dy = k / 3, dx = k % 3;
+    o0 = fmaf(w, f0[dy * pitch + dx], o0);
+    o1 = fmaf(w, f1[dy * pitch + dx], o1);
+  }
+}
+
+}
+
+#endif
diff --git a/torch-optical-flow_amd/csrc/upsample.hip b/torch-optical-flow_amd/csrc/upsample.hip
--- a/torch-optical-flow_amd/csrc/upsample.hip
+++ b/torch-optical-flow_amd/csrc/upsample.hip
@@ -1,3 +1,4 @@
+#include "convex_upsample.h"
 #include "oflow_internal.h"
 
 namespace oflow {
@@ -38,26 +39,10 @@
     __syncthreads();
     if (live) {
       float m[9];
-      float mx = sM[0][j][xo];
 #pragma unroll
-      for (int k = 0; k < 9; ++k) {
-        m[k] = sM[k][j][xo];
-        mx = fmaxf(mx, m[k]);
-      }
-      float s = 0.f;
-#pragma unroll
-      for (int k = 0; k < 9; ++k) {
-        m[k] = expf(m[k] - mx);
-        s += m[k];
-      }
-      float o0 = 0.f, o1 = 0.f;
-#pragma unroll
-      for (int k = 0; k < 9; ++k) {
-        const float w = m[k] / s;
-        const int dy = k / 3, dx = k % 3;
-        o0 += w * sF[0][dy][xo + dx];
-        o1 += w * sF[1][dy][xo + dx];
-      }
+      for (int k = 0; k < 9; ++k) m[k] = sM[k][j][xo];
+      float o0, o1;
+      convex_upsample_px(m, &sF[0][0][xo], &sF[1][0][xo], kUX + 2, o0, o1);
       const long long W8 = 8LL * W, H8W8 = 64LL * HW;
       float* op = out + (long long)n * 2 * H8W8 + (long long)(8 * y + i) * W8 + 8LL * (x0 + xo) + j;
       op[0] = o0;
diff --git a/torch-optical-flow_amd/methods/raft/model/extractor.py b/torch-optical-flow_amd/methods/raft/model/extractor.py
--- a/torch-optical-flow_amd/methods/raft/model/extractor.py
+++ b/torch-optical-flow_amd/methods/raft/model/extractor.py
@@ -300,7 +300,10 @@
         return patches
 
     def __call__(self, x: Union[Tensor, Sequence[Tensor]], patches: Optional[Tensor] = None,
-                 split_out: bool = False, stem_from_image: bool = False) -> Union[Tensor, Tuple[Tensor, ...]]:
+                 split_out: bool = False, stem_from_image: bool = False,
+                 scale255: bool = False) -> Union[Tensor, Tuple[Tensor, ...]]:
+        if scale255 and not stem_from_image:
+            raise RuntimeError("SplitEncoder: scale255 needs stem_from_image")
         is_list = isinstance(x, (tuple, list))
         if is_list:
             batch_dim = x[0].shape[0]
@@ -321,7 +324,7 @@
         if stem_from_image:
             if isinstance(x, (tuple, list)):
                 x = torch.cat([t.float() for t in x], dim=0)
-            stem_in = _native.ImgIn(x.float().contiguous())
+            stem_in = _native.ImgIn(x.float().contiguous(), scale255=scale255)
             self.patches = None
         else:
             if patches is None or tuple(patches.shape[:4]) != (n, h, w, self.w["stem"].kg):
diff --git a/torch-optical-flow_amd/methods/raft/model/raft.py b/torch-optical-flow_amd/methods/raft/model/raft.py
--- a/torch-optical-flow_amd/methods/raft/model/raft.py
+++ b/torch-optical-flow_amd/methods/raft/model/raft.py
@@ -89,6 +89,8 @@
         self.lookup_fusion = True
         self.split_corr = True
         self.stem_from_image = True
+        self.stem_scale_fusion = True
+        self.upsample_fusion = True
         self.range_guard = "deferred"
         self._range_pending = []
         self.last_range_snapshot = None
@@ -169,6 +171,9 @@
         up_flow = torch.sum(mask * up_flow, dim=2).permute(0, 1, 4, 2, 5, 3)
         return up_flow.reshape(n, 2, 8 * h, 8 * w)
 
+    def _fuse_upsample(self, pixels: int) -> bool:
+        return bool(self.upsample_fusion) and pixels >= _native.UPSAMPLE_FUSION_MIN_PIXELS
+
     def _lane_cuts(self, b: int):
         n = min(self.pair_lanes, b)
         edges = [(b * i) // n for i in range(n + 1)]
@@ -197,6 +202,12 @@
         lanes = self._lanes_for(dev, b)
         SplitUpdate._weights(self.update_block)
         init_main = getattr(self, "lane_init_on_main", False) or runners is not None
+        hw = cnet_out.shape[2] * cnet_out.shape[3]
+        fuse_up = self._fuse_upsample(b * hw)
+        ups = []
+        if fuse_up:
+            h8, w8 = 8 * cnet_out.shape[2], 8 * cnet_out.shape[3]
+            ups = [torch.empty((b, 2, h8, w8), device=dev, dtype=torch.float32) for _ in range(1 if test_mode else iters)]
         if not init_main:
             for st in lanes[1:]:
                 st.wait_stream(main)
@@ -206,7 +217,6 @@
             for st in lanes[1:]:
                 st.wait_stream(main)
         joined = self.pair_lookup == "joined" and not runners[0].fusable(corr_fn)
-        hw = cnet_out.shape[2] * cnet_out.shape[3]
         if joined:
             rows = torch.empty((b * hw, runners[0].corr_ch), device=dev, dtype=torch.float32)
             h, w = cnet_out.shape[2:]
@@ -217,20 +227,25 @@
         for itr in range(iters):
             last = itr == iters - 1
             need = not test_mode or last
-            mask = torch.empty((b, 576, *cnet_out.shape[2:]), device=dev, dtype=torch.float32) if need else None
+            mask = (torch.empty((b, 576, *cnet_out.shape[2:]), device=dev, dtype=torch.float32)
+                    if need and not fuse_up else None)
+            flow_up = ups[0 if test_mode else itr] if need and fuse_up else None
             if joined:
                 for st in lanes[1:]:
                     main.wait_stream(st)
                 corr_fn.lookup_nhwc(coords1, rows)
-            if joined or need:
+            if joined or mask is not None:
                 for st in lanes[1:]:
                     st.wait_stream(main)
             for i, ((b0, b1), st) in enumerate(zip(cuts, lanes)):
                 with torch.cuda.stream(st):
                     c1 = coords1[b0:b1]
                     corr_in = ins[i] if joined else runners[i].lookup(parts[i], c1)
-                    runners[i].update(corr_in, c1, need, mask_out=mask[b0:b1] if need else None)
-            if need:
+                    runners[i].update(corr_in, c1, need, mask_out=mask[b0:b1] if mask is not None else None,
+                                      up=(coords0[b0:b1], flow_up[b0:b1]) if flow_up is not None else None)
+            if flow_up is not None:
+                outs.append(flow_up)
+            elif need:
                 for st in lanes[1:]:
                     main.wait_stream(st)
                 outs.append(self.upsample_flow(coords1 - coords0, mask))
@@ -317,24 +332,27 @@
             self._range_pending.append(snap)
 
     def _encode(self, image0: Tensor, image1: Tensor, hdim: int, both: bool):
-        if (NATIVE_NORMALIZE and image0.is_cuda and image1.is_cuda and image0.dtype == image1.dtype == torch.float32
-                and image0.shape == image1.shape
-                and not (torch.is_grad_enabled() and (image0.requires_grad or image1.requires_grad))):
-            image0, image1 = _native.normalize_images(image0, image1)
-        else:
-            image0 = (2 * (image0 / 255.0) - 1.0).contiguous()
-            image1 = (2 * (image1 / 255.0) - 1.0).contiguous()
-        first = torch.cat([image0, image1], dim=0) if both else image0
-
-        def sides(a, b):
-            return (torch.cat([a, b], dim=0), torch.cat([b, a], dim=0)) if both else (a, b)
-
         split_enc = (
             image0.is_cuda
             and not torch.is_grad_enabled()
             and self.encoder_impl == "split"
             and (not self.fnet.training or self.fnet.dropout is None)
         )
+        native_norm = (NATIVE_NORMALIZE and image0.is_cuda and image1.is_cuda
+                       and image0.dtype == image1.dtype == torch.float32 and image0.shape == image1.shape
+                       and not (torch.is_grad_enabled() and (image0.requires_grad or image1.requires_grad)))
+        s255 = (native_norm and self.stem_scale_fusion and split_enc and not self.cnet.training and self.stem_from_image)
+        if native_norm:
+            if not s255:
+                image0, image1 = _native.normalize_images(image0, image1)
+        else:
+            image0 = (2 * (image0 / 255.0) - 1.0).contiguous()
+            image1 = (2 * (image1 / 255.0) - 1.0).contiguous()
+        first = torch.cat([image0, image1], dim=0) if both else image0
+
+        def sides(a, b):
+            return (torch.cat([a, b], dim=0), torch.cat([b, a], dim=0)) if both else (a, b)
+
         fnet = SplitEncoder(self.fnet) if split_enc else self.fnet
         cnet = SplitEncoder(self.cnet) if split_enc and not self.cnet.training else self.cnet
         block = AlternateCorrBlock if self.hparams.get("alternate_corr", False) else CorrBlock
@@ -352,7 +370,7 @@
                 side2.wait_stream(main)
                 with torch.cuda.stream(side2):
                     f2s = fnet(image1, patches=None if patches is None else patches[ni:], split_out=True,
-                               stem_from_image=sfi)
+                               stem_from_image=sfi, scale255=s255)
                 if not both:
                     patches = None if sfi else fnet.stem_patches(image0)
             elif not both:
@@ -364,25 +382,25 @@
             if side is not None:
                 side.wait_stream(main)
                 with torch.cuda.stream(side):
-                    cnet_out = cnet(first, patches=cpatches, stem_from_image=sfi)
+                    cnet_out = cnet(first, patches=cpatches, stem_from_image=sfi, scale255=s255)
                     if early:
                         SplitUpdate._weights(self.update_block)
                         pre_runners = self._lane_runners(cnet_out, hdim, lanes, on=side)
             if block is CorrBlock and self.split_corr:
                 if side2 is not None:
                     f1s = fnet(image0, patches=patches[:ni] if both and patches is not None else patches, split_out=True,
-                               stem_from_image=sfi)
+                               stem_from_image=sfi, scale255=s255)
                     main.wait_stream(side2)
                 else:
-                    f1s, f2s = fnet([image0, image1], patches=patches, split_out=True, stem_from_image=sfi)
+                    f1s, f2s = fnet([image0, image1], patches=patches, split_out=True, stem_from_image=sfi, scale255=s255)
                 corr_fn = CorrBlock.from_split_features(*sides(f1s, f2s), radius=self.hparams.corr_radius)
             else:
-                fmap1, fmap2 = fnet([image0, image1], patches=patches, stem_from_image=sfi)
+                fmap1, fmap2 = fnet([image0, image1], patches=patches, stem_from_image=sfi, scale255=s255)
                 corr_fn = block(*sides(fmap1.float(), fmap2.float()), radius=self.hparams.corr_radius)
             if side is not None:
                 main.wait_stream(side)
             else:
-                cnet_out = cnet(first, patches=cpatches, stem_from_image=sfi)
+                cnet_out = cnet(first, patches=cpatches, stem_from_image=sfi, scale255=s255)
         else:
             fmap1, fmap2 = fnet([image0, image1])
             corr_fn = block(*sides(fmap1.float(), fmap2.float()), radius=self.hparams.corr_radius)
@@ -419,12 +437,17 @@
         if impl == "split":
             runner = SplitUpdate(self.update_block, cnet_out, hdim, fuse_c1=self.lookup_fusion)
             coords1 = coords1.contiguous()
+            n, _, h, w = cnet_out.shape
+            fuse_up = self._fuse_upsample(n * h * w)
             for itr in range(iters):
                 last = itr == iters - 1
-                up_mask = runner.step(corr_fn, coords1, need_mask=not test_mode or last)
-                if test_mode and not last:
+                need = not test_mode or last
+                up = ((coords0, torch.empty((n, 2, 8 * h, 8 * w), device=cnet_out.device, dtype=torch.float32))
+                      if need and fuse_up else None)
+                up_mask = runner.step(corr_fn, coords1, need_mask=need, up=up)
+                if not need:
                     continue
-                flow_up = self.upsample_flow(coords1 - coords0, up_mask)
+                flow_up = up[1] if up is not None else self.upsample_flow(coords1 - coords0, up_mask)
                 flow_predictions.append(flow_up)
             if test_mode:
                 return coords1 - coords0, flow_up
diff --git a/torch-optical-flow_amd/methods/raft/model/update.py b/torch-optical-flow_amd/methods/raft/model/update.py
--- a/torch-optical-flow_amd/methods/raft/model/update.py
+++ b/torch-optical-flow_amd/methods/raft/model/update.py
@@ -363,6 +363,7 @@
             "fh2_fused": _native.flow_head_fused_weights(fh.conv2.weight),
             "m1": CW(block.mask[0].weight, block.mask[0].bias, 256),
             "m2": CW(block.mask[2].weight, block.mask[2].bias, 576),
+            "m2u": _native.mask_upsample_weights(block.mask[2]),
         }
         if block.corr_radius in (3, 4):
             w["c1L"] = _native.convc1_level_weights(enc.convc1, block.corr_levels, block.corr_radius)
@@ -375,8 +376,9 @@
                                 torch.cat([cz.bias, cr.bias, cq.bias]), 384)
         return w
 
-    def step(self, corr_fn, coords1: Tensor, need_mask: bool, mask_out: Optional[Tensor] = None) -> Optional[Tensor]:
-        return self.update(self.lookup(corr_fn, coords1), coords1, need_mask, mask_out)
+    def step(self, corr_fn, coords1: Tensor, need_mask: bool, mask_out: Optional[Tensor] = None,
+             up=None) -> Optional[Tensor]:
+        return self.update(self.lookup(corr_fn, coords1), coords1, need_mask, mask_out, up)
 
     def lookup_rows(self, coords1: Tensor) -> Tensor:
         if self.corr_f32 is None:
@@ -400,7 +402,8 @@
         else:
             _native.conv_s32(corr_in, self.w["c1"], 128, "relu", y0=_native.S32Slice(self.c1))
 
-    def update(self, corr_in, coords1: Tensor, need_mask: bool, mask_out: Optional[Tensor] = None) -> Optional[Tensor]:
+    def update(self, corr_in, coords1: Tensor, need_mask: bool, mask_out: Optional[Tensor] = None,
+               up=None) -> Optional[Tensor]:
         V, conv, w = _native.S32Slice, _native.conv_s32, self.w
         main = torch.cuda.current_stream(coords1.device)
         side = self.side_stream if self.streams else None
@@ -438,7 +441,7 @@
             _native.conv_s32_flow_head(net, w["fh1"], bns["fh1"], w["fh2_fused"], self.fhy)
             _native.flow_head_finish(self.fhy, w["fh2_bias"], coords1, (V(self.hx), 254), (V(self.rhx), 254))
             self.flow_for = flow_key
-            return self._mask(net, coords1, mask_out) if need_mask else None
+            return self._mask(net, coords1, mask_out, up) if need_mask else None
         conv(net, w["fh1"], bns["fh1"], "relu", y0=V(self.fh))
         if self.flow_head_fma and coords1.is_contiguous():
             _native.flow_head2(V(self.fh), *w["fh2_f32"], coords1)
@@ -446,11 +449,15 @@
             _native.flow_head2_tiled(V(self.fh), *w["fh2_tiled"], coords1)
         else:
             conv(V(self.fh), w["fh2"], 32, f32=coords1, f32_accumulate=True)
-        return self._mask(net, coords1, mask_out) if need_mask else None
-
-    def _mask(self, net, coords1: Tensor, mask_out: Optional[Tensor]) -> Tensor:
+        return self._mask(net, coords1, mask_out, up) if need_mask else None
+
+    def _mask(self, net, coords1: Tensor, mask_out: Optional[Tensor], up=None) -> Tensor:
         V, conv, w = _native.S32Slice, _native.conv_s32, self.w
         b, h, wd = self.shape
+        if up is not None:
+            conv(net, w["m1"], 128, "relu", y0=V(self.fh))
+            _native.conv_s32_upsample(V(self.fh), w["m2u"], up[0], coords1, up[1], out_scale=0.25)
+            return up[1]
         mask = mask_out if mask_out is not None else torch.empty((b, 576, h, wd), device=coords1.device, dtype=torch.float32)
         conv(net, w["m1"], 128, "relu", y0=V(self.fh))
         conv(V(self.fh), w["m2"], 64, out_scale=0.25, f32=mask)
diff --git a/torch-optical-flow_amd/optical_flow/_native.py b/torch-optical-flow_amd/optical_flow/_native.py
--- a/torch-optical-flow_amd/optical_flow/_native.py
+++ b/torch-optical-flow_amd/optical_flow/_native.py
@@ -34,6 +34,14 @@
         ("d_nhwc", _P), ("d_stats", _P), ("d_res", _P), ("res_pixel_stride", _L),
         ("nhwc_pixel_stride", _I), ("res_activation", _I), ("s2d", _I), ("d_addend", _P), ("addend_pixel_stride", _L),
         ("d_fh_weights", _P), ("d_fh_partial", _P), ("fh_slabs", _I),
+    ]
+
+
+class ConvS32ExtDesc(ctypes.Structure):
+    _fields_ = [
+        ("struct_size", ctypes.c_uint), ("img_scale255", ctypes.c_int),
+        ("d_up_coords0", ctypes.c_void_p), ("d_up_coords1", ctypes.c_void_p), ("d_up_out", ctypes.c_void_p),
+        ("up_batch_stride", ctypes.c_longlong),
     ]
 
 
@@ -128,6 +136,7 @@
         "oflow_ssim_loss_backward_f32": (I, [P, P, P, P, I, P, I, I, I, I, I, FP, F, F, P, P, P]),
         "oflow_charbonnier_loss_f32": (I, [P, P, P, I, I, I, I, I, F, F, F, P, P, P, P]),
         "oflow_charbonnier_loss_backward_f32": (I, [P, P, P, P, I, P, I, I, I, I, F, F, F, P, P, P]),
+        "oflow_conv_s32_ext": (I, [P, P, P]),
     }
 
 
@@ -762,16 +771,16 @@
 
 class ImgIn:
 
-    __slots__ = ("raw", "bhw")
+    __slots__ = ("raw", "bhw", "scale255")
     in_format = 3
 
-    def __init__(self, img: torch.Tensor):
+    def __init__(self, img: torch.Tensor, scale255: bool = False):
         if img.dtype != torch.float32 or img.dim() != 4 or img.shape[1] != 3 or not img.is_contiguous():
             raise RuntimeError("ImgIn: the image must be contiguous fp32 (B, 3, H, W)")
         b, _, hh, ww = img.shape
         if hh % 2 or ww % 2:
             raise RuntimeError("ImgIn: H and W must be even")
-        self.raw, self.bhw = img, (int(b), int(hh) // 2, int(ww) // 2)
+        self.raw, self.bhw, self.scale255 = img, (int(b), int(hh) // 2, int(ww) // 2), bool(scale255)
 
     @property
     def ptr(self) -> int:
@@ -1037,7 +1046,57 @@
         n_exec = -(-cw.n_pad // d.block_n) * d.block_n
         _count(3 * 2 * p_out * n_exec * cw.kg * 32 * taps, 2 * p_out * cw.n * cw.cin * taps)
     with torch.cuda.device(x.device), _Timed(f"conv{cw.kh}x{cw.kw}", x.device):
-        _check(load().oflow_conv_s32(ctypes.byref(d), _stream(x.device)), what)
+        if getattr(x, "scale255", False):
+            ext = ConvS32ExtDesc(struct_size=ctypes.sizeof(ConvS32ExtDesc), img_scale255=1)
+            _check(load().oflow_conv_s32_ext(ctypes.byref(d), ctypes.byref(ext), _stream(x.device)), what)
+        else:
+            _check(load().oflow_conv_s32(ctypes.byref(d), _stream(x.device)), what)
+
+
+UPSAMPLE_BLOCK = 96
+UPSAMPLE_FUSION_MIN_PIXELS = 16384
+
+
+def mask_upsample_weights(conv: torch.nn.Conv2d) -> "ConvWeights":
+    w = conv.weight.detach().float()
+    if tuple(w.shape) != (576, w.shape[1], 1, 1) or conv.bias is None:
+        raise RuntimeError(f"mask_upsample_weights: expected a biased 1x1 conv to 576 channels, got {tuple(w.shape)}")
+    i, k, j = torch.meshgrid(torch.arange(8), torch.arange(9), torch.arange(8), indexing="ij")
+    col = (i * UPSAMPLE_BLOCK + k * 8 + j).reshape(-1).to(w.device)
+    src = (k * 64 + i * 8 + j).reshape(-1).to(w.device)
+    wp = w.new_zeros((8 * UPSAMPLE_BLOCK, w.shape[1], 1, 1))
+    bp = w.new_zeros(8 * UPSAMPLE_BLOCK)
+    wp[col] = w[src]
+    bp[col] = conv.bias.detach().float()[src]
+    cw = ConvWeights(wp, bp, 8 * UPSAMPLE_BLOCK)
+    cw.layout = "mask_upsample"
+    return cw
+
+
+def conv_s32_upsample(x: "S32Slice", cw: "ConvWeights", coords0: torch.Tensor, coords1: torch.Tensor, out: torch.Tensor,
+                      out_scale: float = 0.25) -> None:
+    what = "conv_s32_upsample"
+    if cw.layout != "mask_upsample" or x.ng != cw.kg:
+        raise RuntimeError(f"{what}: weights must be mask_upsample_weights over the input's {x.ng} groups")
+    b, h, w = x.bhw
+    dev = x.device
+    for name, t in (("coords0", coords0), ("coords1", coords1)):
+        if t.dtype != torch.float32 or tuple(t.shape) != (b, 2, h, w) or not t.is_contiguous() or t.device != dev:
+            raise RuntimeError(f"{what}: {name} must be contiguous fp32 ({b}, 2, {h}, {w}) on the input's device")
+    if (out.dtype != torch.float32 or tuple(out.shape) != (b, 2, 8 * h, 8 * w) or out.device != dev
+            or tuple(out.stride()[1:]) != (64 * h * w, 8 * w, 1) or (b > 1 and out.stride(0) < 128 * h * w)):
+        raise RuntimeError(f"{what}: out must be fp32 ({b}, 2, {8 * h}, {8 * w}) with contiguous images")
+    d = _conv_desc(x, cw, UPSAMPLE_BLOCK)
+    d.epilogue, d.activation, d.out_scale = 4, ACT["none"], float(out_scale)
+    ext = ConvS32ExtDesc(struct_size=ctypes.sizeof(ConvS32ExtDesc), d_up_coords0=coords0.data_ptr(),
+                         d_up_coords1=coords1.data_ptr(), d_up_out=out.data_ptr(),
+                         up_batch_stride=out.stride(0) if b > 1 else 128 * h * w)
+    if _flops is not None:
+        _count(3 * 2 * b * h * w * cw.n_pad * cw.kg * 32, 2 * b * h * w * 576 * cw.cin)
+        fl = 2 * b * h * w * 64 * 2 * 9
+        _count(0, fl, fl)
+    with torch.cuda.device(dev), _Timed("conv1x1", dev):
+        _check(load().oflow_conv_s32_ext(ctypes.byref(d), ctypes.byref(ext), _stream(dev)), what)
 
 
 def flow_head2(x: "S32Slice", weight: torch.Tensor, bias: torch.Tensor, coords: torch.Tensor) -> None:
```

Result: no change. 468.9 image-pairs/s, median of 6 (+0.7%).
